# jolibrain/joliGEN

Hardware: AMD Instinct MI355X
Metric: train images/sec at 256x256 (DDPM UNet step) (higher is better)
Workload: dtype bf16; 1 GPU; palette_model DDPM, efficient UNet unet_mha ngf64 mults[1,2,4,8] res_blocks[2,2,2,2] mid-attn 16x32, 256x256, batch 32/GPU, inpainting synthetic masks, AdamW+EMA, iter_size 1 (example_ddpm_noglasses2glasses.json + SURVEY Appendix C overrides); global_batch=32, per_gpu_batch=32, image_size=256, efficient=True, parallelism=dp1, n_ranks_seen=1

## Files before the change

joligen_amd/_lib.py:

```python
from __future__ import annotations

import ctypes as C
import os
import re
import subprocess

_HERE = os.path.dirname(os.path.abspath(__file__))
CSRC = os.path.join(_HERE, "csrc")
LIB_PATH = os.path.join(CSRC, "libjg355.so")
HEADER = os.path.join(os.path.dirname(_HERE), "include", "jg355.h")
SOURCES = ["attention.hip", "gemm_nt.hip", "conv_halo.hip", "conv_kxk.hip", "reflect_border.hip", "conv_p64.hip", "conv1x1.hip", "gemm_tn.hip", "wgrad_halo.hip", "wgrad_sw.hip", "wgrad_kxk.hip", "nce.hip", "segformer.hip", "vit.hip", "projected_d.hip", "effnet.hip", "norm.hip", "gn_fused.hip", "elementwise.hip", "d_aug.hip", "context.hip", "d_diffusion.hip", "dropout.hip", "sem_cls.hip", "resize_aa.hip", "optim.hip", "capi.hip"]
HIPCC_FLAGS = ["--offload-arch=gfx950", "-O3", "-std=c++17", "-fPIC", "-shared", "-munsafe-fp-atomics", "-fno-slp-vectorize"]

FILE_FLAGS = {}

c_i32, c_i64, c_f32, c_p = C.c_int32, C.c_int64, C.c_float, C.c_void_p

_SCALARS = {"int": c_i32, "int32_t": c_i32, "int64_t": c_i64, "uint32_t": C.c_uint32, "uint64_t": C.c_uint64, "float": c_f32, "jg_stream_t": c_p}


def _ctype(decl: str, structs: dict, where: str):
    tok = re.findall(r"\w+|\*", decl)
    if len(tok) > 1 and tok[-1] != "*":
        tok = tok[:-1]
    if not tok or re.sub(r"[\w\s*]", "", decl):
        raise TypeError(f"jg355.h: cannot parse `{decl.strip()}` in `{where}`")
    if "*" not in tok:
        if len(tok) == 1 and tok[0] in _SCALARS:
            return _SCALARS[tok[0]]
        raise TypeError(f"jg355.h: type `{' '.join(tok)}` of `{decl.strip()}` in `{where}` is outside the ABI's type map")
    if tok == ["const", "char", "*"]:
        return C.c_char_p
    if len(tok) == 3 and tok[0] == "const" and tok[1] in structs and tok[2] == "*":
        return C.POINTER(structs[tok[1]])
    return c_p


def parse_header(text: str):
    text = re.sub(r"/\*.*?\*/", " ", text, flags=re.S)
    consts, structs, sigs, restypes = {}, {}, {}, {}
    for name, val in re.findall(r"^[ \t]*#[ \t]*define[ \t]+(JG_\w+)[ \t]+(-?\d+)[ \t]*$", text, flags=re.M):
        consts[name] = int(val)
    text = re.sub(r"^[ \t]*#.*$", " ", text, flags=re.M)
    text = re.sub(r'extern\s+"C"\s*\{(.*)\}', r"\1", text, flags=re.S)
    text = re.sub(r"typedef\s+void\s*\*\s*jg_stream_t\s*;", " ", text)

    def enum(m):
        for item in m.group(1).split(","):
            im = re.fullmatch(r"\s*(JG_\w+)\s*=\s*(-?\d+)\s*", item)
            if not im:
                raise TypeError(f"jg355.h: enumerator `{item.strip()}` needs the form JG_X = n")
            consts[im.group(1)] = int(im.group(2))
        return " "

    def struct(m):
        fields = []
        for decl in filter(str.strip, m.group(1).split(";")):
            first, *more = decl.split(",")
            ct = _ctype(first, structs, m.group(2))
            if ct not in _SCALARS.values() and more:
                raise TypeError(f"jg355.h: one pointer per declaration, `{decl.strip()}` in `{m.group(2)}`")
            fields += [(re.findall(r"\w+", d)[-1], ct) for d in [first] + more]
        structs[m.group(2)] = type(m.group(2), (C.Structure,), {"_fields_": fields})
        return " "

    def proto(m):
        ret, name, params = m.group(1), m.group(2), m.group(3)
        restypes[name] = _ctype(ret + " " + name, structs, name)
        sigs[name] = [] if params.strip() == "void" else [_ctype(p, structs, name) for p in params.split(",")]
        return " "

    text = re.sub(r"enum\s*\{([^}]*)\}\s*;", enum, text)
    text = re.sub(r"typedef\s+struct\s*\w*\s*\{([^}]*)\}\s*(\w+)\s*;", struct, text)
    text = re.sub(r"([\w\s*]+?)\b(jg_\w+)\s*\(([^()]*)\)\s*;", proto, text)
    if text.strip():
        raise TypeError(f"jg355.h: not understood: `{' '.join(text.split())[:200]}`")
    return consts, structs, sigs, restypes


with open(HEADER) as _f:
    CONSTANTS, STRUCTS, SIGNATURES, RESTYPES = parse_header(_f.read())
globals().update(CONSTANTS)
ConvArgs, WgradArgs = STRUCTS["jg_conv_args"], STRUCTS["jg_wgrad_args"]


def build(force: bool = False, verbose: bool = False, jobs: int = 0) -> str:
    import json
    import time
    from concurrent.futures import ThreadPoolExecutor

    hdrs = [os.path.join(CSRC, h) for h in sorted(os.listdir(CSRC)) if h.endswith(".h")] + [HEADER]
    hdr_time = max(os.path.getmtime(h) for h in hdrs)
    bdir = os.path.join(CSRC, "build")
    os.makedirs(bdir, exist_ok=True)
    hipcc = os.environ.get("HIPCC", "/opt/rocm/bin/hipcc")
    if not os.path.exists(hipcc):
        hipcc = "hipcc"
    cflags = [f for f in HIPCC_FLAGS if f != "-shared"]
    todo, objs = [], []
    for src in SOURCES:
        sp, op = os.path.join(CSRC, src), os.path.join(bdir, src.replace(".hip", ".o"))
        objs.append(op)
        if force or not os.path.exists(op) or os.path.getmtime(op) < max(os.path.getmtime(sp), hdr_time):
            todo.append((sp, op))

    def cc(job):
        sp, op = job
        cmd = [hipcc] + cflags + FILE_FLAGS.get(os.path.basename(sp), []) + ["-c", sp, "-o", op]
        if verbose:
            print(" ".join(cmd), flush=True)
        subprocess.run(cmd, check=True, cwd=CSRC)

    t0 = time.time()
    if todo:
        with ThreadPoolExecutor(max_workers=jobs or min(len(todo), os.cpu_count() or 4)) as ex:
            list(ex.map(cc, todo))
    relink = bool(todo) or not os.path.exists(LIB_PATH) or os.path.getmtime(LIB_PATH) < max(os.path.getmtime(o) for o in objs)
    if relink:
        cmd = [hipcc, "--offload-arch=gfx950", "-shared", "-fPIC", "-o", LIB_PATH] + objs
        if verbose:
            print(" ".join(cmd), flush=True)
        subprocess.run(cmd, check=True, cwd=CSRC)
    if todo or relink:
        with open(os.path.join(bdir, "BUILD_INFO.json"), "w") as f:
            json.dump({"compiled": [os.path.basename(s) for s, _ in todo], "linked": relink, "seconds": round(time.time() - t0, 1),
                       "flags": cflags, "hipcc": hipcc}, f)
    return LIB_PATH


_lib = None


def lib():
    global _lib
    if _lib is not None:
        return _lib
    if not os.path.exists(LIB_PATH):
        raise RuntimeError(
            f"{LIB_PATH} is missing: run `python -c 'import __graft_entry__ as g; g.build()'` "
            "(hipcc --offload-arch=gfx950).  joligen_amd has no CPU / eager fallback."
        )
    L = C.CDLL(LIB_PATH)
    for name, argtypes in SIGNATURES.items():
        fn = getattr(L, name)
        fn.argtypes = argtypes
        fn.restype = RESTYPES[name]
    _lib = L
    return L


def set_tuning(name: str, value: int):
    L = lib()
    prev = L.jg_get_tuning(name.encode())
    check(L.jg_set_tuning(name.encode(), int(value)), f"jg_set_tuning({name})")
    return prev


def check(code: int, what: str = ""):
    if code != 0:
        msg = lib().jg_strerror(code).decode()
        raise RuntimeError(f"libjg355 {what} failed: {msg} ({code})")
```

joligen_amd/csrc/common.h:

```cpp
#pragma once
#include <hip/hip_runtime.h>
#include <stdint.h>

#include "../../include/jg355.h"

typedef _Float16 f16_t;
typedef __bf16 bf16_t;
typedef _Float16 f16x8 __attribute__((ext_vector_type(8)));
typedef __bf16 bf16x8 __attribute__((ext_vector_type(8)));
typedef float f32x4 __attribute__((ext_vector_type(4)));
typedef short s16x4_t __attribute__((ext_vector_type(4)));
typedef __attribute__((address_space(3))) s16x4_t* lds_v4;

#define JG_WAVE 64

#define JG_TUNE_LIST(X) \
  X(HALO_CFG, 0) X(WGRAD_HALO_CFG, 0) X(CONV_VARIANT, 6) X(WGRAD_VARIANT, 4) X(SINKHORN_GENERIC, 0) X(CONV1X1, 1) X(GN_REVERSE, 1) \
  X(HALO_DBG, 0) X(PERSIST64, 1) X(HALO_PIPE, 1) X(WGRAD_PIPE, 1) X(CONV_SPLITK, 1) X(CONV_SMALL_TILE, 1) X(GN_FUSED, 1)           \
  X(GN_FUSED_CAP, 256) X(GN_FUSED_DBG, 0) X(GN_FUSED_SLEEP, 4) X(WGRAD_LDS_PAD, 0) X(LN_BWD_CAP, 256) X(DW_BWD_CAP, 512)           \
  X(DW_BWD_PPT, 8) X(CONV_KXK, 1) X(CONV_RING, 1) X(WGRAD_DEEP, 1) X(WGRAD_SW, 0) X(DETERMINISTIC, 0) X(WGRAD_GROUP_BLOCKS, 1024)  \
  X(SGEMM_SPLIT, 0) X(WGRAD_BIG, 1) X(DW_RUN, 1) X(SUBPIXEL_DGRAD_CFG, 0)
#define JG_TUNE_ENUM(name, dflt) JG_TUNE_##name,
enum JgTune { JG_TUNE_LIST(JG_TUNE_ENUM) JG_TUNE_COUNT };
#undef JG_TUNE_ENUM
int jg_tune(int which);
void jg_note_kernel(const char* name);

#define JG_CHECK_LAUNCH()                          \
  do {                                             \
    if (hipGetLastError() != hipSuccess) return JG_ERR_LAUNCH; \
  } while (0)

template <typename T> __device__ __forceinline__ float to_f32(T v) { return (float)v; }
template <typename T> __device__ __forceinline__ T from_f32(float v) { return (T)v; }

template <typename T> __device__ __forceinline__ T bits_to(uint16_t b) { return __builtin_bit_cast(T, b); }
template <typename T> __device__ __forceinline__ uint16_t to_bits(T v) { return __builtin_bit_cast(uint16_t, v); }

template <typename T> __device__ __forceinline__ void unpack8(const uint4& v, float* f) {
  const uint32_t w[4] = {v.x, v.y, v.z, v.w};
#pragma unroll
  for (int i = 0; i < 4; ++i) {
    f[2 * i] = to_f32(bits_to<T>((uint16_t)(w[i] & 0xffffu)));
    f[2 * i + 1] = to_f32(bits_to<T>((uint16_t)(w[i] >> 16)));
  }
}
template <typename T> __device__ __forceinline__ uint4 pack8(const float* f) {
  uint32_t w[4];
#pragma unroll
  for (int i = 0; i < 4; ++i) {
    w[i] = (uint32_t)to_bits<T>(from_f32<T>(f[2 * i])) | ((uint32_t)to_bits<T>(from_f32<T>(f[2 * i + 1])) << 16);
  }
  return make_uint4(w[0], w[1], w[2], w[3]);
}
template <typename T> __device__ __forceinline__ uint2 pack4(float a, float b, float c, float d) {
  uint2 r;
  r.x = (uint32_t)to_bits<T>(from_f32<T>(a)) | ((uint32_t)to_bits<T>(from_f32<T>(b)) << 16);
  r.y = (uint32_t)to_bits<T>(from_f32<T>(c)) | ((uint32_t)to_bits<T>(from_f32<T>(d)) << 16);
  return r;
}
template <typename T> __device__ __forceinline__ void unpack4(const uint2& v, float* f) {
  f[0] = to_f32(bits_to<T>((uint16_t)(v.x & 0xffffu)));
  f[1] = to_f32(bits_to<T>((uint16_t)(v.x >> 16)));
  f[2] = to_f32(bits_to<T>((uint16_t)(v.y & 0xffffu)));
  f[3] = to_f32(bits_to<T>((uint16_t)(v.y >> 16)));
}

template <typename T> struct Mfma;
template <> struct Mfma<f16_t> {
  static __device__ __forceinline__ f32x4 run(const uint4& a, const uint4& b, f32x4 c) {
    return __builtin_amdgcn_mfma_f32_16x16x32_f16(__builtin_bit_cast(f16x8, a), __builtin_bit_cast(f16x8, b), c, 0, 0, 0);
  }
};
template <> struct Mfma<bf16_t> {
  static __device__ __forceinline__ f32x4 run(const uint4& a, const uint4& b, f32x4 c) {
    return __builtin_amdgcn_mfma_f32_16x16x32_bf16(__builtin_bit_cast(bf16x8, a), __builtin_bit_cast(bf16x8, b), c, 0, 0, 0);
  }
};

template <typename T> __device__ __forceinline__ uint4 ldg16(const T* ptr, bool ok) {
  uint4 v = *reinterpret_cast<const uint4*>(ptr);
  v.x = ok ? v.x : 0u;
  v.y = ok ? v.y : 0u;
  v.z = ok ? v.z : 0u;
  v.w = ok ? v.w : 0u;
  return v;
}

__device__ __forceinline__ float sigmoid_fast(float u) { return __builtin_amdgcn_rcpf(1.0f + __expf(-u)); }
__device__ __forceinline__ float silu_f(float u) { return u * sigmoid_fast(u); }
__device__ __forceinline__ float silu_grad_f(float u) {
  const float s = sigmoid_fast(u);
  return s * (1.0f + u * (1.0f - s));
}

template <int ACT> __device__ __forceinline__ float act_f(float u) {
  if (ACT == JG_ACT_SILU) return silu_f(u);
  if (ACT == JG_ACT_RELU) return fmaxf(u, 0.f);
  if (ACT == JG_ACT_LRELU) return u > 0.f ? u : 0.2f * u;
  return u;
}
template <int ACT> __device__ __forceinline__ float act_grad_f(float u) {
  if (ACT == JG_ACT_SILU) return silu_grad_f(u);
  if (ACT == JG_ACT_RELU) return u > 0.f ? 1.f : 0.f;
  if (ACT == JG_ACT_LRELU) return u > 0.f ? 1.f : 0.2f;
  return 1.f;
}
__device__ __forceinline__ float act_grad_rt(float u, int act) {
  return act == JG_ACT_SILU ? silu_grad_f(u) : act == JG_ACT_RELU ? (u > 0.f ? 1.f : 0.f) : act == JG_ACT_LRELU ? (u > 0.f ? 1.f : 0.2f) : 1.f;
}

#define JG_DISPATCH_ACT(act, ...)                          \
  do {                                                     \
    if ((act) == JG_ACT_SILU) { constexpr int ACT = JG_ACT_SILU; __VA_ARGS__ }        \
    else if ((act) == JG_ACT_RELU) { constexpr int ACT = JG_ACT_RELU; __VA_ARGS__ }   \
    else if ((act) == JG_ACT_LRELU) { constexpr int ACT = JG_ACT_LRELU; __VA_ARGS__ } \
    else { constexpr int ACT = JG_ACT_NONE; __VA_ARGS__ }                              \
  } while (0)

__device__ __forceinline__ float wave_sum(float v) {
#pragma unroll
  for (int o = 32; o > 0; o >>= 1) v += __shfl_xor(v, o);
  return v;
}
__device__ __forceinline__ float wave_max(float v) {
#pragma unroll
  for (int o = 32; o > 0; o >>= 1) v = fmaxf(v, __shfl_xor(v, o));
  return v;
}

#define JG_DISPATCH_DTYPE(dtype, ...)                 \
  do {                                                \
    if ((dtype) == JG_F16) {                          \
      typedef f16_t T;                                \
      __VA_ARGS__                                     \
    } else if ((dtype) == JG_BF16) {                  \
      typedef bf16_t T;                               \
      __VA_ARGS__                                     \
    } else {                                          \
      return JG_ERR_BAD_ARG;                          \
    }                                                 \
  } while (0)
```

joligen_amd/csrc/gemm_tn.hip:

```cpp
#include "common.h"
#include "wgrad_params.h"
#include "lds_dma.h"
#include <vector>
#include <cstdlib>

namespace {


__device__ __forceinline__ int swz128(int row) { return (row >> 1) & 7; }

__device__ __forceinline__ void transpose4x8(const uint4* ra, uint2* out) {
  const uint32_t w[4][4] = {{ra[0].x, ra[0].y, ra[0].z, ra[0].w},
                            {ra[1].x, ra[1].y, ra[1].z, ra[1].w},
                            {ra[2].x, ra[2].y, ra[2].z, ra[2].w},
                            {ra[3].x, ra[3].y, ra[3].z, ra[3].w}};
#pragma unroll
  for (int d = 0; d < 4; ++d) {
    out[2 * d].x = (w[0][d] & 0xffffu) | (w[1][d] << 16);
    out[2 * d].y = (w[2][d] & 0xffffu) | (w[3][d] << 16);
    out[2 * d + 1].x = (w[0][d] >> 16) | (w[1][d] & 0xffff0000u);
    out[2 * d + 1].y = (w[2][d] >> 16) | (w[3][d] & 0xffff0000u);
  }
}

template <typename T>
__global__ __launch_bounds__(256) void wgrad_tn_kernel(WgP p) {
  constexpr int BM = 128, BN = 128, BK = 64;
  __shared__ uint4 sm[2][(BM + BN) * 8];

  const int tid = threadIdx.x;
  const int lane = tid & 63;
  const int wave = tid >> 6;
  const int wm = wave >> 1, wn = wave & 1;

  const int tilesN = (p.Ktot + BN - 1) / BN;
  const int n0 = (blockIdx.x % tilesN) * BN;
  const int m0 = (blockIdx.x / tilesN) * BM;

  const int z = blockIdx.z;
  const int batch = z / p.splitk, split = z % p.splitk;
  const int zb = batch / p.nh, zh = batch % p.nh;
  const T* __restrict__ dy = (const T*)p.dy + zb * p.sdyb + zh * p.sdyh;
  const T* __restrict__ x = (const T*)p.x + zb * p.sxb + zh * p.sxh;

  int per = (p.Mpix + p.splitk - 1) / p.splitk;
  per = (per + BK - 1) / BK * BK;
  const int kbeg = split * per;
  const int kend = min(p.Mpix, kbeg + per);
  if (kbeg >= kend) return;
  const int nk = (kend - kbeg + BK - 1) / BK;

  const int pq = tid & 15, co = tid >> 4;
  const int cm = m0 + co * 8;
  const bool a_ok = cm < p.Cout;
  const int nn = n0 + co * 8;
  const bool b_ok = nn < p.Ktot;
  const int rs = nn / p.Cin, ci = nn % p.Cin;
  const int fr = rs / p.S, fs = rs % p.S;
  const bool quad_row = (p.Wo & 3) == 0;

  uint4 ra[4], rb[4];
  float bsum[8];
#pragma unroll
  for (int q = 0; q < 8; ++q) bsum[q] = 0.f;
  const bool do_bias = p.dbias != nullptr && (blockIdx.x % tilesN) == 0;

  auto load_tiles = [&](int kbase) {
    const int p0 = kbase + pq * 4;
#pragma unroll
    for (int i = 0; i < 4; ++i) {
      const int pp = p0 + i;
      const bool ok = a_ok && pp < kend;
      ra[i] = ldg16(dy + (ok ? (long)pp * p.lddy + cm : 0), ok);
    }
    if (quad_row) {
      const int ow0 = p0 % p.Wo;
      const int t = p0 / p.Wo;
      const int oh = t % p.Ho;
      const int b = t / p.Ho;
      const int ih = oh * p.stride + fr - p.pad;
      const bool row_ok = b_ok && (unsigned)ih < (unsigned)p.H;
      const long rowoff = ((long)(b * p.H + ih) * p.W) * p.ldx + ci;
#pragma unroll
      for (int i = 0; i < 4; ++i) {
        const int iw = (ow0 + i) * p.stride + fs - p.pad;
        const bool ok = row_ok && (p0 + i) < kend && (unsigned)iw < (unsigned)p.W;
        rb[i] = ldg16(x + (ok ? rowoff + (long)iw * p.ldx : 0), ok);
      }
    } else {
#pragma unroll
      for (int i = 0; i < 4; ++i) {
        const int pp = p0 + i;
        const int ow = pp % p.Wo;
        const int t = pp / p.Wo;
        const int oh = t % p.Ho;
        const int b = t / p.Ho;
        const int ih = oh * p.stride + fr - p.pad;
        const int iw = ow * p.stride + fs - p.pad;
        const bool ok = b_ok && pp < kend && (unsigned)ih < (unsigned)p.H && (unsigned)iw < (unsigned)p.W;
        rb[i] = ldg16(x + (ok ? ((long)(b * p.H + ih) * p.W + iw) * p.ldx + ci : 0), ok);
      }
    }
  };
  auto store_lds = [&](int buf) {
    uint2 ta[8], tb[8];
    transpose4x8(ra, ta);
    transpose4x8(rb, tb);
    uint2* s2 = reinterpret_cast<uint2*>(&sm[buf][0]);
#pragma unroll
    for (int j = 0; j < 8; ++j) {
      const int row = co * 8 + j;
      const int slot = row * 16 + (((pq >> 1) ^ swz128(row)) << 1) + (pq & 1);
      s2[slot] = ta[j];
      s2[BM * 16 + slot] = tb[j];
    }
    if (do_bias) {
#pragma unroll
      for (int i = 0; i < 4; ++i) {
        float f[8];
        unpack8<T>(ra[i], f);
#pragma unroll
        for (int q = 0; q < 8; ++q) bsum[q] += f[q];
      }
    }
  };

  f32x4 acc[4][4];
#pragma unroll
  for (int i = 0; i < 4; ++i)
#pragma unroll
    for (int j = 0; j < 4; ++j) acc[i][j] = (f32x4){0.f, 0.f, 0.f, 0.f};

  const int frow = lane & 15, fk = lane >> 4;
  auto compute = [&](int buf) {
#pragma unroll
    for (int sub = 0; sub < 2; ++sub) {
      uint4 fa[4], fb[4];
      const int kc = fk + 4 * sub;
#pragma unroll
      for (int i = 0; i < 4; ++i) {
        const int row = wm * 64 + i * 16 + frow;
        fa[i] = sm[buf][row * 8 + (kc ^ swz128(row))];
      }
#pragma unroll
      for (int j = 0; j < 4; ++j) {
        const int row = wn * 64 + j * 16 + frow;
        fb[j] = sm[buf][BM * 8 + row * 8 + (kc ^ swz128(row))];
      }
#pragma unroll
      for (int i = 0; i < 4; ++i)
#pragma unroll
        for (int j = 0; j < 4; ++j) acc[i][j] = Mfma<T>::run(fa[i], fb[j], acc[i][j]);
    }
  };

// ... 419 lines not shown
        const int m = m0 + wm * 128 + i * 16 + (lane >> 4) * 4 + q;
        if (m >= p.Cout_out) continue;
        atomicAdd((float*)p.dw + zoff + (long)m * p.lddw + ocol, p.alpha * acc[i][j][q]);
      }
    }
  }
  if (do_bias) {
    float* s_b = reinterpret_cast<float*>(&sm[0][0]);
#pragma unroll
    for (int q = 0; q < 8; ++q) {
      float v = bsum[q];
      v += __shfl_xor(v, 32);
      if (lane < 32) s_b[wave * 256 + cidx * 8 + q] = v;
    }
    __syncthreads();
    if (tid < BM && (m0 + tid) < p.Cout_out) {
      float v = 0.f;
#pragma unroll
      for (int w8 = 0; w8 < 8; ++w8) v += s_b[w8 * 256 + tid];
      atomicAdd(p.dbias + m0 + tid, p.dbias_scale * v);
    }
  }
}

template <typename T, bool SPREAD = false, int ABL = 0>
__device__ __forceinline__ void wgrad_tn_dma_body(const WgP& p, const int bx, const int bz, uint4 (*sm)[2 * BIG_TILE]) {
  constexpr int BM = 256, BN = 256, BK = 64;
  const int tid = threadIdx.x;
  const int lane = tid & 63;
  const int wave = __builtin_amdgcn_readfirstlane(tid >> 6);
  const int wm = wave >> 2, wn = wave & 3;

  const int tilesN = (p.Ktot + BN - 1) / BN;
  const int n0 = (bx % tilesN) * BN;
  const int m0 = (bx / tilesN) * BM;
  const int batch = bz / p.splitk, split = bz % p.splitk;
  const int zb = batch / p.nh, zh = batch % p.nh;
  const T* __restrict__ dy = (const T*)p.dy + zb * p.sdyb + zh * p.sdyh;
  const T* __restrict__ x = (const T*)p.x + zb * p.sxb + zh * p.sxh;
  const T* zp = reinterpret_cast<const T*>(&jg_zero_page);

  int per = (p.Mpix + p.splitk - 1) / p.splitk;
  per = (per + BK - 1) / BK * BK;
  const int kbeg = split * per;
  const int kend = min(p.Mpix, kbeg + per);
  if (kbeg >= kend) return;
  const int nk = (kend - kbeg + BK - 1) / BK;

  typedef __attribute__((address_space(3))) char* lds_cptr;
  const unsigned lds0 = (unsigned)(size_t)(lds_cptr)(char*)&sm[0][0];

  int a_col[4], b_ci[4], b_fr[4], b_fs[4];
  bool a_ok[4], b_ok[4];
#pragma unroll
  for (int rd = 0; rd < 4; ++rd) {
    const int q = rd * 512 + tid;
    const int row = q >> 5, ps = q & 31;
    const int c = (((ps >> 1) ^ swz_tr(row)) << 1) | (ps & 1);
    a_col[rd] = m0 + c * 8;
    a_ok[rd] = a_col[rd] < p.Cout;
    const int nn = n0 + c * 8;
    b_ok[rd] = nn < p.Ktot;
    const int rs = nn / p.Cin;
    b_ci[rd] = nn % p.Cin;
    b_fr[rd] = rs / p.S;
    b_fs[rd] = rs % p.S;
  }
  auto issue_one = [&](int kbase, int buf, int idx) {
    const unsigned l0 = lds0 + (unsigned)((buf * 2 * BIG_TILE + wave * 64) * 16);
    const int rd = idx & 3;
    const int pp = kbase + ((rd * 512 + tid) >> 5);
    if (idx < 4) {
      const bool ok = a_ok[rd] && pp < kend;
      glds16(ok ? dy + (long)pp * p.lddy + a_col[rd] : zp, l0 + rd * 512 * 16);
    } else {
      const int ow = pp % p.Wo;
      const int t = pp / p.Wo;
      const int oh = t % p.Ho;
      const int b = t / p.Ho;
      const int ih = oh * p.stride + b_fr[rd] - p.pad;
      const int iw = ow * p.stride + b_fs[rd] - p.pad;
      const bool ok = b_ok[rd] && pp < kend && (unsigned)ih < (unsigned)p.H && (unsigned)iw < (unsigned)p.W;
      glds16(ok ? x + ((long)(b * p.H + ih) * p.W + iw) * p.ldx + b_ci[rd] : zp, l0 + (BIG_TILE + rd * 512) * 16);
    }
  };
  auto issue = [&](int kbase, int buf) {
#pragma unroll
    for (int idx = 0; idx < 8; ++idx) issue_one(kbase, buf, idx);
  };

  f32x4 acc[8][4], accb[8];
#pragma unroll
  for (int i = 0; i < 8; ++i) {
    accb[i] = (f32x4){0.f, 0.f, 0.f, 0.f};
#pragma unroll
    for (int j = 0; j < 4; ++j) acc[i][j] = (f32x4){0.f, 0.f, 0.f, 0.f};
  }
  const bool do_bias = p.dbias != nullptr && (bx % tilesN) == 0 && wn == 0;
  const uint32_t one1 = to_bits<T>(from_f32<T>(1.0f));
  const uint32_t one2 = one1 | (one1 << 16);
  const uint4 ones = make_uint4(one2, one2, one2, one2);

  const int i16 = lane & 15, g = lane >> 4;
  auto frag = [&](int buf, int tile, int cb, int sub) -> uint4 {
    if constexpr (ABL == 2) return make_uint4((unsigned)(buf + tile), (unsigned)cb, (unsigned)sub, (unsigned)lane);
    const char* base = reinterpret_cast<const char*>(&sm[buf][tile]);
    uint32_t w[4];
#pragma unroll
    for (int rd = 0; rd < 2; ++rd) {
      const int row = sub * 32 + g * 8 + rd * 4 + (i16 >> 2);
      const int off = (row * BIG_CH + ((cb ^ swz_tr(row)) << 1)) * 16 + (i16 & 3) * 8;
      const s16x4_t v = __builtin_amdgcn_ds_read_tr16_b64_v4i16((lds_v4)(base + off));
      const uint2 u = __builtin_bit_cast(uint2, v);
      w[2 * rd] = u.x;
      w[2 * rd + 1] = u.y;
    }
    return make_uint4(w[0], w[1], w[2], w[3]);
  };

  if constexpr (ABL != 3) issue(kbeg, 0);
  for (int ks = 0; ks < nk; ++ks) {
    const int cur = ks & 1;
    wait_vmcnt<0>();
    __builtin_amdgcn_s_barrier();
    const bool more = ks + 1 < nk;
    if (more && !SPREAD && ABL != 3) issue(kbeg + (ks + 1) * BK, cur ^ 1);
    uint4 fa_n = frag(cur, 0, wm * 8, 0);
#pragma unroll
    for (int sub = 0; sub < 2; ++sub) {
      uint4 fb[4];
#pragma unroll
      for (int j = 0; j < 4; ++j) fb[j] = frag(cur, BIG_TILE, wn * 4 + j, sub);
#pragma unroll
      for (int i = 0; i < 8; ++i) {
        const uint4 fa = fa_n;
        if (i < 7) fa_n = frag(cur, 0, wm * 8 + i + 1, sub);
        else if (sub == 0) fa_n = frag(cur, 0, wm * 8, 1);
        if (SPREAD && more && (i & 1) == 0) {
          __builtin_amdgcn_sched_barrier(0);
          issue_one(kbeg + (ks + 1) * BK, cur ^ 1, sub * 4 + (i >> 1));
          __builtin_amdgcn_sched_barrier(0);
        }
        if (do_bias) accb[i] = Mfma<T>::run(fa, ones, accb[i]);
#pragma unroll
        for (int j = 0; j < 4; ++j) {
          if constexpr (ABL == 1) { acc[i][j][0] += __builtin_bit_cast(float, fa.x ^ fb[j].y); acc[i][j][1] += __builtin_bit_cast(float, fa.z ^ fb[j].w); }
          else acc[i][j] = Mfma<T>::run(fa, fb[j], acc[i][j]);
        }
      }
    }
  }

  const long zoff = zb * p.sdwb + zh * p.sdwh;
#pragma unroll
  for (int j = 0; j < 4; ++j) {
    const int n = n0 + wn * 64 + j * 16 + (lane & 15);
    if (n >= p.Ktot) continue;
    const int ors = n / p.Cin, oci = n % p.Cin;
    if (oci >= p.Cin_out) continue;
    const long ocol = (long)ors * p.Cin_out + oci;
#pragma unroll
    for (int i = 0; i < 8; ++i) {
#pragma unroll
      for (int q = 0; q < 4; ++q) {
        const int m = m0 + wm * 128 + i * 16 + (lane >> 4) * 4 + q;
        if (m >= p.Cout_out) continue;
        atomicAdd((float*)p.dw + zoff + (long)m * p.lddw + ocol, p.alpha * acc[i][j][q]);
      }
    }
  }
  if (do_bias && (lane & 15) == 0) {
#pragma unroll
    for (int i = 0; i < 8; ++i)
#pragma unroll
      for (int q = 0; q < 4; ++q) {
        const int m = m0 + wm * 128 + i * 16 + (lane >> 4) * 4 + q;
        if (m < p.Cout_out) atomicAdd(p.dbias + m, p.dbias_scale * accb[i][q]);
      }
  }
}

template <typename T, bool DMA = true, int ABL = 0>
__global__ __launch_bounds__(512, 1) void wgrad_tn_big_kernel(WgP p) {
  __shared__ uint4 sm[2][2 * BIG_TILE];
  int bx, bz;
  wgrad_xcd_order(bx, bz);
  if constexpr (DMA) wgrad_tn_dma_body<T, ABL == 4, ABL == 4 ? 0 : ABL>(p, bx, bz, sm);
  else wgrad_tn_big_body<T>(p, bx, bz, sm);
}

constexpr int GROUP_MAX = 16;
struct WgGroup {
  WgP p[GROUP_MAX];
  int start[GROUP_MAX + 1];
  int tiles[GROUP_MAX];
  int n;
};
template <typename T, int WAVES_M, bool DEEP = false>
__global__ __launch_bounds__(256, 2) void wgrad_tn_tr_group_kernel(const WgGroup g) {
  __shared__ uint4 sm[2][2 * TR_TILE];
  const int b = blockIdx.x;
  int i = 0;
#pragma unroll
  for (int k = 1; k < GROUP_MAX; ++k) i += (k < g.n && b >= g.start[k]) ? 1 : 0;
  i = __builtin_amdgcn_readfirstlane(i);
  const int local = b - g.start[i];
  wgrad_tn_tr_body<T, WAVES_M, DEEP>(g.p[i], local % g.tiles[i], local / g.tiles[i], sm);
}

template <typename T, bool DMA = true>
__global__ __launch_bounds__(512, 1) void wgrad_tn_big_group_kernel(const WgGroup g) {
  __shared__ uint4 sm[2][2 * BIG_TILE];
  const int b = blockIdx.x;
  int i = 0;
#pragma unroll
  for (int k = 1; k < GROUP_MAX; ++k) i += (k < g.n && b >= g.start[k]) ? 1 : 0;
  i = __builtin_amdgcn_readfirstlane(i);
  const int local = b - g.start[i];
  if constexpr (DMA) wgrad_tn_dma_body<T>(g.p[i], local % g.tiles[i], local / g.tiles[i], sm);
  else wgrad_tn_big_body<T>(g.p[i], local % g.tiles[i], local / g.tiles[i], sm);
}

static inline bool wg_big_ok(const WgP& p) {
  return jg_tune(JG_TUNE_WGRAD_BIG) != 0 && p.out_mode == JG_OUT_ATOMIC_F32 && p.Cout >= 256 && p.Ktot >= 256 && p.Mpix >= 8192;
}

}

static int make_wgp(const jg_wgrad_args* a, WgP& p) {
  if (!a || !a->dy || !a->x || !a->dw) return JG_ERR_BAD_ARG;
  if (a->Cin % 8 || a->Cout % 8 || a->ldx % 8 || a->lddy % 8) return JG_ERR_BAD_ARG;
  if (a->nbatch < 1 || a->nh < 1 || a->splitk < 1) return JG_ERR_BAD_ARG;
  if ((long)a->nbatch * a->splitk > 65535) return JG_ERR_BAD_ARG;
  if (a->out_mode != JG_OUT_ATOMIC_F32 && a->splitk != 1) return JG_ERR_BAD_ARG;
  if (a->dbias && a->out_mode != JG_OUT_ATOMIC_F32) return JG_ERR_BAD_ARG;
  const long Mpix = (long)a->B * a->Ho * a->Wo;
  if (Mpix <= 0 || Mpix > (1L << 30)) return JG_ERR_BAD_ARG;
  p.dy = (const char*)a->dy; p.x = (const char*)a->x; p.dw = (char*)a->dw; p.dbias = a->dbias;
  p.Mpix = (int)Mpix; p.Cout = a->Cout; p.Ktot = a->R * a->S * a->Cin;
  p.H = a->H; p.W = a->W; p.Cin = a->Cin; p.R = a->R; p.S = a->S; p.pad = a->pad; p.stride = a->stride;
  p.Ho = a->Ho; p.Wo = a->Wo;
  p.Cin_out = a->Cin_out > 0 ? a->Cin_out : a->Cin;
  p.Cout_out = a->Cout_out > 0 ? a->Cout_out : a->Cout;
  p.lddy = a->lddy; p.ldx = a->ldx; p.lddw = a->lddw;
  p.nh = a->nh; p.splitk = a->splitk;
  if (jg_tune(JG_TUNE_DETERMINISTIC) != 0 && a->out_mode == JG_OUT_ATOMIC_F32) p.splitk = 1;
  p.sdyb = a->sdyb; p.sdyh = a->sdyh; p.sxb = a->sxb; p.sxh = a->sxh; p.sdwb = a->sdwb; p.sdwh = a->sdwh;
  p.alpha = a->alpha; p.out_mode = a->out_mode; p.B = a->B;
  p.dbias_scale = a->dbias_scale != 0.f ? a->dbias_scale : 1.f;
  if (a->pad_mode != 0 && a->pad_mode != 1) return JG_ERR_BAD_ARG;
  p.reflect = a->pad_mode == 1;
  if (a->x_mode < 0 || a->x_mode > 2) return JG_ERR_BAD_ARG;
  p.x_up = a->x_mode;
  if (p.x_up && (p.reflect || (a->H & 1) || (a->W & 1) || a->nbatch != 1)) return JG_ERR_BAD_ARG;
  return JG_OK;
}

extern "C" int jg_conv2d_wgrad_tn_group(int dtype, const jg_wgrad_args* a, int n, jg_stream_t stream) {
  if (!a || n < 1 || n > 4096) return JG_ERR_BAD_ARG;
  const int variant = jg_tune(JG_TUNE_WGRAD_VARIANT);
  if (variant < 2) return JG_ERR_UNSUPPORTED;
  std::vector<WgP> ps((size_t)n);
  std::vector<char> special((size_t)n, 0);
  for (int i = 0; i < n; ++i) {
    const int rc = make_wgp(a + i, ps[i]);
    if (rc != JG_OK) return rc;
    if (a[i].nbatch != 1 || a[i].out_mode != JG_OUT_ATOMIC_F32 || ps[i].reflect || ps[i].x_up) return JG_ERR_UNSUPPORTED;
    special[i] = variant >= 4 && (a[i].R > 1 || a[i].S > 1) &&
                 (jg_wgrad_halo_try(dtype, ps[i], 1, (hipStream_t)stream, true) || jg_wgrad_kxk_try(dtype, ps[i], 1, (hipStream_t)stream, true));
  }
  for (int i = 0; i < n; ++i)
    if (special[i] && !jg_wgrad_halo_try(dtype, ps[i], 1, (hipStream_t)stream)) jg_wgrad_kxk_try(dtype, ps[i], 1, (hipStream_t)stream);
  const int group_blocks = jg_tune(JG_TUNE_WGRAD_GROUP_BLOCKS);
  const size_t gpad = (size_t)jg_tune(JG_TUNE_WGRAD_LDS_PAD);
  for (int wavesm = 1; wavesm <= 3; ++wavesm) {
    WgGroup g;
    g.n = 0;
    g.start[0] = 0;
    auto flush = [&]() -> int {
      if (!g.n) return JG_OK;
      if (group_blocks > 0) {
        long total = 0;
        for (int i = 0; i < g.n; ++i) total += (long)g.tiles[i] * ((g.p[i].Mpix + 63) / 64);
        const long len = std::max<long>(4, (total + group_blocks - 1) / group_blocks);
        for (int i = 0; i < g.n; ++i) {
          const long ks = (g.p[i].Mpix + 63) / 64;
          g.p[i].splitk = (int)std::max<long>(1, std::min<long>(g.p[i].splitk, (ks + len - 1) / len));
          g.start[i + 1] = g.start[i] + g.tiles[i] * g.p[i].splitk;
        }
      }
      const dim3 grid(g.start[g.n]);
      const int deep = jg_tune(JG_TUNE_WGRAD_DEEP);
      if (wavesm == 3) {
        if (jg_tune(JG_TUNE_WGRAD_BIG) == 2) { JG_DISPATCH_DTYPE(dtype, hipLaunchKernelGGL((wgrad_tn_big_group_kernel<T, false>), grid, dim3(512), 0, (hipStream_t)stream, g);); }
        else { JG_DISPATCH_DTYPE(dtype, hipLaunchKernelGGL((wgrad_tn_big_group_kernel<T, true>), grid, dim3(512), 0, (hipStream_t)stream, g);); }
      } else if (wavesm == 1) {
        if (deep & 1) { JG_DISPATCH_DTYPE(dtype, hipLaunchKernelGGL((wgrad_tn_tr_group_kernel<T, 1, true>), grid, dim3(256), gpad, (hipStream_t)stream, g);); }
        else { JG_DISPATCH_DTYPE(dtype, hipLaunchKernelGGL((wgrad_tn_tr_group_kernel<T, 1>), grid, dim3(256), gpad, (hipStream_t)stream, g);); }
      } else {
        if (deep & 2) { JG_DISPATCH_DTYPE(dtype, hipLaunchKernelGGL((wgrad_tn_tr_group_kernel<T, 2, true>), grid, dim3(256), gpad, (hipStream_t)stream, g);); }
        else { JG_DISPATCH_DTYPE(dtype, hipLaunchKernelGGL((wgrad_tn_tr_group_kernel<T, 2>), grid, dim3(256), gpad, (hipStream_t)stream, g);); }
      }
      g.n = 0;
      return JG_OK;
    };
    for (int i = 0; i < n; ++i) {
      const WgP& p = ps[i];
      if (special[i] || (wg_big_ok(p) ? 3 : p.Cout <= 64 ? 1 : 2) != wavesm) continue;
      const int tiles = wavesm == 3 ? ((p.Cout + 255) / 256) * ((p.Ktot + 255) / 256) : ((p.Cout + 64 * wavesm - 1) / (64 * wavesm)) * ((p.Ktot + 127) / 128);
      g.p[g.n] = p;
      g.tiles[g.n] = tiles;
      g.start[g.n + 1] = g.start[g.n] + tiles * p.splitk;
      if (++g.n == GROUP_MAX) {
        const int rc2 = flush();
        if (rc2 != JG_OK) return rc2;
      }
    }
    const int rc3 = flush();
    if (rc3 != JG_OK) return rc3;
  }
  JG_CHECK_LAUNCH();
  return JG_OK;
}

extern "C" int jg_conv2d_wgrad_tn(int dtype, const jg_wgrad_args* a, jg_stream_t stream) {
  jg_note_kernel("");
  WgP p;
  {
    const int rc = make_wgp(a, p);
    if (rc != JG_OK) return rc;
  }
  const int variant = jg_tune(JG_TUNE_WGRAD_VARIANT);
  if (p.x_up == 2) {
    if (variant < 4 || !jg_wgrad_halo_try(dtype, p, a->nbatch, (hipStream_t)stream)) return JG_ERR_UNSUPPORTED;
    JG_CHECK_LAUNCH();
    return JG_OK;
  }
  if (variant >= 4 && (jg_wgrad_halo_try(dtype, p, a->nbatch, (hipStream_t)stream) || jg_wgrad_kxk_try(dtype, p, a->nbatch, (hipStream_t)stream))) {
    JG_CHECK_LAUNCH();
    return JG_OK;
  }
  if (p.reflect || p.x_up) return JG_ERR_UNSUPPORTED;
  if (variant >= 2 && wg_big_ok(p)) {
    const int tiles = ((p.Cout + 255) / 256) * ((p.Ktot + 255) / 256);
    dim3 grid(tiles, 1, a->nbatch * p.splitk);
    jg_note_kernel("wgrad_tn_big_kernel");
    const int bigmode = jg_tune(JG_TUNE_WGRAD_BIG);
    if (bigmode == 11) { JG_DISPATCH_DTYPE(dtype, hipLaunchKernelGGL((wgrad_tn_big_kernel<T, true, 1>), grid, dim3(512), 0, (hipStream_t)stream, p);); }
    else if (bigmode == 12) { JG_DISPATCH_DTYPE(dtype, hipLaunchKernelGGL((wgrad_tn_big_kernel<T, true, 2>), grid, dim3(512), 0, (hipStream_t)stream, p);); }
    else if (bigmode == 14) { JG_DISPATCH_DTYPE(dtype, hipLaunchKernelGGL((wgrad_tn_big_kernel<T, true, 4>), grid, dim3(512), 0, (hipStream_t)stream, p);); }
    else if (bigmode == 13) { JG_DISPATCH_DTYPE(dtype, hipLaunchKernelGGL((wgrad_tn_big_kernel<T, true, 3>), grid, dim3(512), 0, (hipStream_t)stream, p);); }
    else if (bigmode == 2) { JG_DISPATCH_DTYPE(dtype, hipLaunchKernelGGL((wgrad_tn_big_kernel<T, false>), grid, dim3(512), 0, (hipStream_t)stream, p);); }
    else { JG_DISPATCH_DTYPE(dtype, hipLaunchKernelGGL((wgrad_tn_big_kernel<T, true>), grid, dim3(512), 0, (hipStream_t)stream, p);); }
    JG_CHECK_LAUNCH();
    return JG_OK;
  }
  const int tilesN = (p.Ktot + 127) / 128;
  if (variant == 1) {
    dim3 grid(((p.Cout + 127) / 128) * tilesN, 1, a->nbatch * p.splitk);
    JG_DISPATCH_DTYPE(dtype, hipLaunchKernelGGL((wgrad_tn_kernel<T>), grid, dim3(256), 0, (hipStream_t)stream, p););
  } else if (p.Cout <= 64 && variant != 3) {
    dim3 grid(tilesN, 1, a->nbatch * p.splitk);
    jg_note_kernel("wgrad_tn_tr_kernel<1>");
    if (jg_tune(JG_TUNE_WGRAD_DEEP) & 1) { JG_DISPATCH_DTYPE(dtype, hipLaunchKernelGGL((wgrad_tn_tr_kernel<T, 1, true>), grid, dim3(256), 0, (hipStream_t)stream, p);); }
    else { JG_DISPATCH_DTYPE(dtype, hipLaunchKernelGGL((wgrad_tn_tr_kernel<T, 1>), grid, dim3(256), 0, (hipStream_t)stream, p);); }
  } else {
    dim3 grid(((p.Cout + 127) / 128) * tilesN, 1, a->nbatch * p.splitk);
    jg_note_kernel("wgrad_tn_tr_kernel<2>");
    if (jg_tune(JG_TUNE_WGRAD_DEEP) & 2) { JG_DISPATCH_DTYPE(dtype, hipLaunchKernelGGL((wgrad_tn_tr_kernel<T, 2, true>), grid, dim3(256), 0, (hipStream_t)stream, p);); }
    else { JG_DISPATCH_DTYPE(dtype, hipLaunchKernelGGL((wgrad_tn_tr_kernel<T, 2>), grid, dim3(256), 0, (hipStream_t)stream, p);); }
  }
  JG_CHECK_LAUNCH();
  return JG_OK;
}
```

joligen_amd/modules/projected_d.py:

```python
from __future__ import annotations

import os

import torch
import torch.nn as nn

from .._autograd import JGFunction
from .. import _lib, launch, ops
from .._lib import check
from ..ops import JG_ACT_LRELU, _dt, _p, _st, conv_nt, wgrad_tn
from .layers import JGConv2d, JGConvNd

TF_EFFICIENTNET_LITE0_WIDTHS = (24, 40, 112, 320)


class _Bilinear2Fn(JGFunction):

    @staticmethod
    def forward(ctx, x, Ho, Wo, align):
        ctx.geo = (x.shape[1], x.shape[2], align)
        return launch.bilinear2_fwd(x.contiguous(), Ho, Wo, align)

    @staticmethod
    @torch.autograd.function.once_differentiable
# ... 47 lines not shown
        dev = mods[0].weight_orig.device
        ws = snap = w16 = dw = 0
        rec = []
        for mod in mods:
            m = mod.meta
            K, RS = m.R * m.S * m.Cin_real, m.R * m.S
            rec.append(dict(ws=ws, snap=0, w16=w16, dw=dw, Cout=m.Cout_real, RS=RS, Cin=m.Cin_real, CoutP=m.Cout, CinP=m.Cin, K=K))
            ws += K + m.Cout_real + 2
            w16 += 2 * m.Cout * RS * m.Cin
            dw += m.Cout_real * K
        self.zero_floats = ws
        for r in rec:
            r["snap"] = ws + snap
            snap += 1 + r["Cout"] + r["K"]
        self.fbuf_floats, self.hbuf_elems, self.dbuf_floats = ws + snap, w16, dw + self.L
        self.dots_off = dw
        self.rec = rec
        self.max_K = max(r["K"] for r in rec)
        self.max_Cout = max(r["Cout"] for r in rec)
        self.max_w = max(r["CoutP"] * r["RS"] * r["CinP"] for r in rec)
        self.max_n = max(r["Cout"] * r["K"] for r in rec)
        tab = np.zeros((self.L, 11), dtype=np.int64)
        ints = tab.view(np.int32).reshape(self.L, 22)
        self.ptrs = []
        for i, (mod, r) in enumerate(zip(mods, rec)):
            g = mod.weight_orig.grad
            if g is None:
                raise RuntimeError("spectral conv weight has no arena-backed .grad")
            p = (mod.weight_orig.data_ptr(), mod.weight_u.data_ptr(), mod.weight_v.data_ptr(), g.data_ptr())
            self.ptrs.append(p)
            tab[i, 0:4] = p
            tab[i, 4:8] = (r["ws"], r["snap"], r["w16"], r["dw"])
            ints[i, 16:22] = (r["Cout"], r["RS"], r["Cin"], r["CoutP"], r["CinP"], 0)
        self.table = torch.from_numpy(tab).to(dev)

    def still_valid(self):
        return all(p == (m.weight_orig.data_ptr(), m.weight_u.data_ptr(), m.weight_v.data_ptr(), m.weight_orig.grad.data_ptr())
                   for p, m in zip(self.ptrs, self.mods))


class _SnPass:

    def __init__(self, group):
        L = _lib.lib()
        self.g = g = group
        dev = g.table.device
        self.fbuf = torch.empty(g.fbuf_floats, device=dev, dtype=torch.float32)
        self.hbuf = torch.empty(g.hbuf_elems, device=dev, dtype=g.dtype)
        check(L.jg_spectral_group_forward(_lib.JG_F16 if g.dtype == torch.float16 else _lib.JG_BF16, g.table.data_ptr(), g.L, self.fbuf.data_ptr(),
                                          g.zero_floats, self.hbuf.data_ptr(), g.max_K, g.max_Cout, g.max_w, 1e-12, _st()), "jg_spectral_group_forward")
        self.dbuf, self.mask, self.flushed = None, 0, False

    def views(self, i):
        r = self.g.rec[i]
        n = r["CoutP"] * r["RS"] * r["CinP"]
        w16 = self.hbuf[r["w16"]:r["w16"] + n].view(r["CoutP"], -1, r["CinP"])
        w16T = self.hbuf[r["w16"] + n:r["w16"] + 2 * n].view(r["CinP"], -1, r["CoutP"])
        return w16, w16T

    def dwsn(self, i):
        if self.dbuf is None:
            self.dbuf = torch.zeros(self.g.dbuf_floats, device=self.fbuf.device, dtype=torch.float32)
        r = self.g.rec[i]
        return self.dbuf[r["dw"]:r["dw"] + r["Cout"] * r["K"]].view(r["Cout"], r["K"])

    def delivered(self, i):
        self.mask |= 1 << i
        if self.mask == (1 << self.g.L) - 1:
            self.flush()

    def flush(self):
        if self.flushed or not self.mask:
            return
        g = self.g
        if ops.WGRAD_DEFER:
            ops.flush_deferred_wgrads()
        check(_lib.lib().jg_spectral_group_wgrad_fix(g.table.data_ptr(), g.L, self.fbuf.data_ptr(), self.dbuf.data_ptr(),
                                                     self.dbuf.data_ptr() + 4 * g.dots_off, self.mask, g.max_n, _st()), "jg_spectral_group_wgrad_fix")
        self.flushed = True


class _SpectralConvFn(JGFunction):

    @staticmethod
    def forward(ctx, x, weight_orig, bias, mod):
        L = _lib.lib()
        m = mod.meta
        x = x.contiguous()
        B, H, W_, Cin = x.shape
        assert Cin == m.Cin, (Cin, m.Cin)
        dev = x.device
        prepared = getattr(mod, "_sn_pass", None)
        if prepared is not None:
            mod._sn_pass = None
            sn, idx = prepared
            w16, w16T = sn.views(idx)
            Ho, Wo = m.out_hw(H, W_)
            y = torch.empty((B, Ho, Wo, m.Cout), device=dev, dtype=x.dtype)
            conv_nt(x, w16, y, B=B, H=H, W=W_, Cin=Cin, Cout=m.Cout, R=m.R, S=m.S, pad=m.pad, stride=m.stride, Ho=Ho, Wo=Wo, ldx=Cin,
                    ldw=m.R * m.S * Cin, ldy=m.Cout, bias=m.bias_pad if m.bias_pad is not None else bias)
            ctx.save_for_backward(x, w16T)
            ctx.mod, ctx.sn = mod, (sn, idx)
            return y
        ctx.sn = None
        sigma = torch.empty(1, device=dev, dtype=torch.float32)
        Wp = weight_orig.data_ptr()
        if mod.training:
            launch.spectral_power_iter(weight_orig, mod.weight_u, mod.weight_v, sigma, m.Cout_real, m.R * m.S, m.Cin_real)
        else:
            Wl = weight_orig.detach().reshape(m.Cout_real, -1)
            sigma.copy_(torch.dot(mod.weight_u, Wl @ mod.weight_v).reshape(1))
        w16 = torch.empty((m.Cout, m.R, m.S, m.Cin), device=dev, dtype=x.dtype)
        w16T = torch.empty((m.Cin, m.R, m.S, m.Cout), device=dev, dtype=x.dtype) if ctx.needs_input_grad[0] else None
        check(L.jg_spectral_weights(_dt(x), Wp, sigma.data_ptr(), w16.data_ptr(), _p(w16T), m.Cout_real, m.R * m.S, m.Cin_real, m.Cout, m.Cin,
                                    _st()), "jg_spectral_weights")
        Ho, Wo = m.out_hw(H, W_)
        y = torch.empty((B, Ho, Wo, m.Cout), device=dev, dtype=x.dtype)
        conv_nt(x, w16, y, B=B, H=H, W=W_, Cin=Cin, Cout=m.Cout, R=m.R, S=m.S, pad=m.pad, stride=m.stride, Ho=Ho, Wo=Wo, ldx=Cin,
                ldw=m.R * m.S * Cin, ldy=m.Cout, bias=m.bias_pad if m.bias_pad is not None else bias)
        ctx.save_for_backward(x, w16T, sigma, mod.weight_u.clone(), mod.weight_v.clone())
        ctx.mod = mod
        return y

    @staticmethod
    @torch.autograd.function.once_differentiable
    def backward(ctx, dy):
        if ctx.sn is not None:
            x, w16T = ctx.saved_tensors
            sigma = u = v = None
        else:
            x, w16T, sigma, u, v = ctx.saved_tensors
        mod = ctx.mod
        m = mod.meta
        dy = dy.contiguous()
        B, H, W_, Cin = x.shape
        _, Ho, Wo, Cout = dy.shape
        dx = None
        if ctx.needs_input_grad[0]:
            dx = torch.empty_like(x)
            if m.stride != 1:
                Hd, Wd = H + 2 * m.pad - m.R + 1, W_ + 2 * m.pad - m.S + 1
                dyd = ops.dilate2d(dy, Hd, Wd, m.stride)
                conv_nt(dyd, w16T, dx, B=B, H=Hd, W=Wd, Cin=Cout, Cout=Cin, R=m.R, S=m.S, pad=m.R - 1 - m.pad, stride=1, Ho=H, Wo=W_,
                        ldx=Cout, ldw=m.R * m.S * Cout, ldy=Cin)
            else:
                conv_nt(dy, w16T, dx, B=B, H=Ho, W=Wo, Cin=Cout, Cout=Cin, R=m.R, S=m.S, pad=m.R - 1 - m.pad, stride=1, Ho=H, Wo=W_,
                        ldx=Cout, ldw=m.R * m.S * Cout, ldy=Cin)
        if ctx.needs_input_grad[1]:
            wg = mod.weight_orig.grad
            if wg is None:
                raise RuntimeError("spectral conv weight has no arena-backed .grad")
            K = m.R * m.S * m.Cin_real
            dwsn = ctx.sn[0].dwsn(ctx.sn[1]) if ctx.sn is not None else torch.zeros((m.Cout_real, K), device=dy.device, dtype=torch.float32)
            ktot = m.R * m.S * Cin
            splitk = ops._wgrad_splitk(((Cout + 127) // 128) * ((ktot + 127) // 128), B * Ho * Wo)
            wgrad_tn(dy, x, dwsn, B=B, H=H, W=W_, Cin=Cin, Cout=Cout, R=m.R, S=m.S, pad=m.pad, stride=m.stride, Ho=Ho, Wo=Wo, lddy=Cout, ldx=Cin,
                     lddw=K, dbias=mod.bias.grad if mod.bias is not None else None, Cin_out=m.Cin_real, Cout_out=m.Cout_real, splitk=splitk,
                     defer=ctx.sn is not None)
            if ctx.sn is not None:
                ctx.sn[0].delivered(ctx.sn[1])
                return dx, None, None, None
            launch.spectral_wgrad_fix(dwsn, mod.weight_orig, u, v, sigma, wg, m.Cout_real, m.R * m.S, m.Cin_real)
        return dx, None, None, None


class SpectralConv2d(nn.Module, JGConvNd):

    jg_wname = "weight_orig"

    def __init__(self, cin, cout, k, stride, padding, bias=True):
        super().__init__()
        ref = nn.Conv2d(cin, cout, k, stride, padding, bias=bias)
        if bias:
            self.bias = nn.Parameter(ref.bias.detach().clone())
        else:
            self.register_parameter("bias", None)
        self.weight_orig = nn.Parameter(ref.weight.detach().clone())
        u = nn.functional.normalize(torch.randn(cout), dim=0, eps=1e-12)
        v = nn.functional.normalize(torch.randn(cin * k * k), dim=0, eps=1e-12)
        self.register_buffer("weight_u", u)
        self.register_buffer("weight_v", v)
        self.needs_dgrad = True
        self.jg_padding, self.jg_stride = padding, stride

    def forward(self, x):
        if self.meta is None:
            raise RuntimeError("SpectralConv2d used before ParamArena finalisation")
        return _SpectralConvFn.apply(x, self.weight_orig, self.bias, self)


class DownBlock(nn.Module):

    def __init__(self, cin, cout):
        super().__init__()
        self.main = nn.Sequential(SpectralConv2d(cin, cout, 4, 2, 1), nn.GroupNorm(cout // 2, cout), nn.LeakyReLU(0.2, inplace=True))

    def forward(self, x):
        conv, gn = self.main[0], self.main[1]
        return ops.group_norm(conv(x), gn.num_groups, gn.weight, gn.bias, None, JG_ACT_LRELU, gn.eps)


CHANNEL_DICT = {4: 512, 8: 512, 16: 256, 32: 128, 64: 64, 128: 64, 256: 32, 512: 16, 1024: 8}


class SingleDisc(nn.Module):

    def __init__(self, nc, start_sz=256, end_sz=8):
        super().__init__()
        nfc = dict(CHANNEL_DICT)
        if start_sz not in nfc:
            start_sz = min(nfc, key=lambda s: abs(s - start_sz))
        self.start_sz = start_sz
        nfc[start_sz] = nc
        layers = []
        while start_sz > end_sz:
            layers.append(DownBlock(nfc[start_sz], nfc[start_sz // 2]))
            start_sz //= 2
        layers.append(SpectralConv2d(nfc[end_sz], 1, 4, 1, 0, bias=False))
        self.main = nn.Sequential(*layers)

    def forward(self, x):
        for layer in self.main:
            x = layer(x)
        return x


class MultiScaleD(nn.Module):

    def __init__(self, channels, resolutions, num_discs=4):
        super().__init__()
        self.mini_discs = nn.ModuleDict({str(i): SingleDisc(nc=c, start_sz=r, end_sz=8)
                                         for i, (c, r) in enumerate(zip(channels[:num_discs], resolutions[:num_discs]))})

    def forward(self, features):
        outs = []
        for k, disc in self.mini_discs.items():
            lg = disc(features[k])
            outs.append(lg[..., 0].reshape(lg.shape[0], -1))
        return torch.cat(outs, dim=1)


class StandInEfficientNet(nn.Module):

    def __init__(self):
        super().__init__()
        w = TF_EFFICIENTNET_LITE0_WIDTHS

        def stage(cin, cout):
            return nn.Sequential(nn.Conv2d(cin, cout, 4, 2, 1), nn.LeakyReLU(0.2))

        self.conv_stem = nn.Conv2d(3, 16, 4, 2, 1)
        self.bn1 = nn.LeakyReLU(0.2)
        self.blocks = nn.Sequential(nn.Identity(), stage(16, w[0]), stage(w[0], w[1]), nn.Identity(), stage(w[1], w[2]), nn.Identity(),
                                    nn.Identity(), nn.Identity(), stage(w[2], w[3]))


class _Stage(nn.Module):

    def __init__(self, items):
        super().__init__()
        for i, it in enumerate(items):
            self.add_module(str(i), it)

    def forward(self, x):
        for mod in self.children():
            x = _run_plain(mod, x)
        return x


def _run_plain(mod, x):
    if isinstance(mod, JGConv2d):
        return mod(x)
    if isinstance(mod, nn.LeakyReLU):
        return ops.activation(x, JG_ACT_LRELU)
    if isinstance(mod, nn.Identity):
        return x
    if isinstance(mod, (nn.Sequential, _Stage)):
        for sub in mod.children():
            x = _run_plain(sub, x)
        return x
    raise NotImplementedError(type(mod))


def _hip_stage(cin, cout):
    return nn.Sequential(JGConv2d(cin, cout, 4, padding=1, stride=2), nn.LeakyReLU(0.2))


LITE0_STEM = 32
LITE0_ARCH = (("ds", 1, 3, 1, 1, 16), ("ir", 2, 3, 2, 6, 24), ("ir", 2, 5, 2, 6, 40), ("ir", 3, 3, 2, 6, 80), ("ir", 3, 5, 1, 6, 112),
              ("ir", 4, 5, 2, 6, 192), ("ir", 1, 3, 1, 6, 320))
LITE0_BN_EPS = 1e-3


def tf_same_pad(size, k, stride):
    out = -(-size // stride)
    total = max((out - 1) * stride + k - size, 0)
    return total // 2, total - total // 2


class _FrozenBN(nn.Module):

    def __init__(self, c, eps=LITE0_BN_EPS):
        super().__init__()
        self.weight, self.bias = nn.Parameter(torch.ones(c)), nn.Parameter(torch.zeros(c))
        self.register_buffer("running_mean", torch.zeros(c))
        self.register_buffer("running_var", torch.ones(c))
        self.register_buffer("num_batches_tracked", torch.tensor(0, dtype=torch.long))
        self.eps = eps
        self._key, self._affine = None, None

# ... 430 lines not shown
```

joligen_amd/modules/unet_exec.py:

```python
from __future__ import annotations

import contextlib
import math
import os
import weakref
from typing import Tuple

import torch
import torch.nn as nn

from .._autograd import JGFunction
from .. import _lib, launch, ops, parallel
from .._lib import JG_ACT_NONE, JG_ACT_SILU, check
from ..ops import _dt, _p, _st, attn_core_bwd, attn_core_fwd, conv_nt, wgrad_tn


class Act:

    __slots__ = ("t", "st", "hw", "pid", "hs_j")

    def __init__(self, t, st, hw, pid, hs_j=None):
        self.t, self.st, self.hw, self.pid, self.hs_j = t, st, hw, pid, hs_j


# ... 9 lines not shown
NSLOT = 16
NORM_BEFORE_UP = os.environ.get("JG_NORM_BEFORE_UP", "1") != "0"
FUSE_DOWN_POOL = os.environ.get("JG_FUSE_DOWN_POOL", "1") != "0"
SUBPIXEL_CONV = os.environ.get("JG_SUBPIXEL_CONV", "1") != "0"
POOL_IN_DGRAD = os.environ.get("JG_POOL_IN_DGRAD", "1") != "0"
SUBPIXEL_DGRAD = os.environ.get("JG_SUBPIXEL_DGRAD", "1") != "0"
SUBPIXEL_WGRAD = os.environ.get("JG_SUBPIXEL_WGRAD", "1") != "0"
X_UP_ON_READ = os.environ.get("JG_X_UP_ON_READ", "1") != "0"
RES_UP_ON_READ = os.environ.get("JG_RES_UP_ON_READ", "1") != "0"
FUSE_GN_REDUCE = os.environ.get("JG_FUSE_GN_REDUCE", "0") != "0"
WGRAD_STREAM = os.environ.get("JG_WGRAD_STREAM", "1") != "0"
WGRAD_CU_MASK = os.environ.get("JG_WGRAD_CU_MASK", "")


def cu_masked_stream(device, first, count, total=256):
    import ctypes as C

    hip = C.CDLL("libamdhip64.so")
    words = (total + 31) // 32
    mask = (C.c_uint32 * words)()
    for i in range(first, min(total, first + count)):
        mask[i // 32] |= 1 << (i % 32)
    st = C.c_void_p()
    with torch.cuda.device(device):
        rc = hip.hipExtStreamCreateWithCUMask(C.byref(st), C.c_uint32(words), mask)
    if rc != 0:
        raise RuntimeError(f"hipExtStreamCreateWithCUMask failed with {rc}")
    return torch.cuda.ExternalStream(st.value, device=device)


def _side_stream(device):
    if WGRAD_CU_MASK:
        first, count = (int(v) for v in WGRAD_CU_MASK.split(":"))
        return cu_masked_stream(device, first, count)
    return torch.cuda.Stream(device=device)
WGRAD_FIRST = os.environ.get("JG_WGRAD_FIRST", "1") != "0"
FUSE_GN_COEF = os.environ.get("JG_FUSE_GN_COEF", "0") != "0"
GN_FUSED = os.environ.get("JG_GN_FUSED", "0") != "0"
FUSE_SKIP_APPLY = os.environ.get("JG_FUSE_SKIP_APPLY", "1") != "0"
FUSE_SKIP_BWD = os.environ.get("JG_FUSE_SKIP_BWD", "1") != "0"


class _Pool:

    def __init__(self, n, device):
        self.buf = torch.zeros(n, device=device, dtype=torch.float32)
        self.off = 0

    def take(self, B, C):
        n = B * NSLOT * C * 2
        if self.off + n > self.buf.numel():
            raise RuntimeError("statistics pool exhausted")
        v = self.buf[self.off:self.off + n].view(B, NSLOT, C, 2)
        self.off += n
        return v

    def take_rows(self, B, C):
        n = B * C * 2
        if self.off + n > self.buf.numel():
            return None
        v = self.buf[self.off:self.off + n].view(B, C, 2)
        self.off += n
        return v


def halo_ok(m, H, W):
    return m.R == 3 and m.S == 3 and m.pad == 1 and m.stride == 1 and m.Cin % 64 == 0 and m.Cout % 64 == 0 and H % 16 == 0 and W % 16 == 0


def subpixel_ok(m, H, W):
    return halo_ok(m, H, W) and H % 32 == 0 and W % 32 == 0 and m.Cin_real == m.Cin and m.Cout_real == m.Cout


def subpixel_fold(m, dtype):
    out = torch.empty((4, m.Cout, 2, 2, m.Cin), device=m.weight.device, dtype=dtype)
    check(_lib.lib().jg_subpixel_fold(_lib.JG_F16 if dtype == torch.float16 else _lib.JG_BF16, m.weight.data_ptr(), out.data_ptr(), m.Cout,
                                      m.Cin, _st()), "jg_subpixel_fold")
    return out


def subpixel_fold_pair(m, dtype):
    out = torch.empty((4, m.Cout, 2, 2, m.Cin), device=m.weight.device, dtype=dtype)
    outT = torch.empty((4, m.Cin, 2, 2, m.Cout), device=m.weight.device, dtype=dtype)
    check(_lib.lib().jg_subpixel_fold_pair(_lib.JG_F16 if dtype == torch.float16 else _lib.JG_BF16, m.weight.data_ptr(), out.data_ptr(),
                                           outT.data_ptr(), m.Cout, m.Cin, _st()), "jg_subpixel_fold_pair")
    return out, outT


def conv_fwd(x, m, out=None, res=None, res_scale=1.0, alpha=1.0, stats=None, res_up=False, x_up=False, wfold=None):
    B, H, W, Cin = x.shape
    if x_up:
        H, W = 2 * H, 2 * W
    Ho, Wo = m.out_hw(H, W)
    if out is None:
        out = torch.empty((B, Ho, Wo, m.Cout), device=x.device, dtype=x.dtype)
    fuse = stats is not None and _stats_fusable(B, Ho, Wo, m.Cout)
    conv_nt(x, m.w16 if wfold is None else wfold, out, B=B, H=H, W=W, Cin=Cin, Cout=m.Cout, R=m.R, S=m.S, pad=m.pad, stride=m.stride,
            Ho=Ho, Wo=Wo, ldx=_ld(x), ldw=m.R * m.S * Cin if wfold is None else 4 * Cin, ldy=_ld(out),
            bias=m.bias_pad if m.bias_pad is not None else m.bias, res=res,
            ldres=_ld(res) if res is not None else 0, alpha=alpha, res_scale=res_scale,
            stats=stats if fuse else None, ldstats=stats.stride(1) // 2 if fuse else 0, stats_slots=NSLOT,
            res_mode=1 if res_up else 0, x_mode=(2 if wfold is not None else 1) if x_up else 0)
    if stats is not None and not fuse:
        check(_lib.lib().jg_gn_stats_ld(_dt(out), out.data_ptr(), _ld(out), stats.data_ptr(), stats.stride(0) // 2, B, Ho * Wo,
                                        m.Cout, _st()), "jg_gn_stats_ld")
    return out


def conv1x1_gn_apply(x, m, ab, act):
    B, H, W, Cin = x.shape
    if m.R != 1 or m.S != 1 or m.stride != 1 or m.pad != 0:
        return None
    y = torch.empty((B, H, W, m.Cout), device=x.device, dtype=x.dtype)
    yn = torch.empty((B, H, W, Cin), device=x.device, dtype=x.dtype)
    ok = conv_nt(x, m.w16, y, B=B, H=H, W=W, Cin=Cin, Cout=m.Cout, R=1, S=1, pad=0, stride=1, Ho=H, Wo=W, ldx=_ld(x), ldw=Cin, ldy=m.Cout,
                 bias=m.bias_pad if m.bias_pad is not None else m.bias, apply=(ab, yn, Cin, act))
    return (yn, y) if ok is not False else None


def conv_dgrad(dy, m, x_shape, out=None, res=None, alpha=1.0, gn=None, pool=None, pool_out=False, wfoldT=None):
    if m.stride != 1:
        raise NotImplementedError("input-gradient of strided convolutions is not implemented")
    B, H, W, Cin = x_shape
    _, Ho, Wo, Cout = dy.shape
    if pool_out:
        assert out is None and res is None and gn is None
        out = torch.empty((B, H // 2, W // 2, Cin), device=dy.device, dtype=dy.dtype)
        if wfoldT is not None:
            conv_nt(dy, wfoldT, out, B=B, H=Ho, W=Wo, Cin=Cout, Cout=Cin, R=3, S=3, pad=1, stride=1, Ho=H, Wo=W, ldx=_ld(dy), ldw=4 * Cout,
                    ldy=_ld(out), alpha=alpha, y_mode=2)
            return out
    if out is None:
        out = torch.empty(x_shape, device=dy.device, dtype=dy.dtype)
    red = None
    kw = {}
    if gn is not None and pool is not None and res is None and _stats_fusable(B, H, W, Cin) and FUSE_GN_REDUCE:
        gx, gab, gact = gn
        red = pool.take(B, Cin)
        kw = dict(stats=red, ldstats=Cin, stats_slots=NSLOT, gn_reduce=(gx, _ld(gx), gab, gact))
    conv_nt(dy, m.w16T, out, B=B, H=Ho, W=Wo, Cin=Cout, Cout=Cin, R=m.R, S=m.S, pad=m.R - 1 - m.pad, stride=1, Ho=H, Wo=W,
            ldx=_ld(dy), ldw=m.R * m.S * Cout, ldy=_ld(out), alpha=alpha, res=res, ldres=_ld(res) if res is not None else 0,
            res_scale=1.0, y_mode=1 if pool_out else 0, **kw)
    return (out, red) if gn is not None else out


def conv_wgrad(dy, x, m, alpha=1.0, dbias_scale=0.0, x_up=False, subpixel=False):
    B, H, W, Cin = x.shape
    if x_up:
        H, W = 2 * H, 2 * W
    _, Ho, Wo, Cout = dy.shape
    wg = m.weight.grad
    if wg is None:
        raise RuntimeError("conv weight has no arena-backed .grad")
    ktot = m.R * m.S * Cin
    tiles = ((Cout + 127) // 128) * ((ktot + 127) // 128)
    splitk = ops._wgrad_splitk(tiles, B * Ho * Wo)
    wgrad_tn(dy, x, wg, B=B, H=H, W=W, Cin=Cin, Cout=Cout, R=m.R, S=m.S, pad=m.pad, stride=m.stride, Ho=Ho, Wo=Wo,
             lddy=_ld(dy), ldx=_ld(x), lddw=m.R * m.S * m.Cin_real, dbias=m.bias.grad if m.bias is not None else None,
             Cin_out=m.Cin_real, Cout_out=m.Cout_real, splitk=splitk, alpha=alpha, dbias_scale=dbias_scale, x_mode=(2 if subpixel else 1) if x_up else 0)


def gn_coef(st, hw, gamma, beta, film, G, eps):
    B, ns, C, _ = st.shape
    ab = torch.empty((B, C, 2), device=st.device, dtype=torch.float32)
    mr = torch.empty((B, G, 2), device=st.device, dtype=torch.float32)
    check(_lib.lib().jg_gn_coef_ld(st.data_ptr(), st.stride(1) // 2, ns, _p(gamma), _p(beta), _p(film),
                                   film.stride(0) if film is not None else 0, ab.data_ptr(), mr.data_ptr(), B, hw, C, G, eps,
                                   _st()), "jg_gn_coef_ld")
    return ab, mr


def gn_apply(x, ab, act):
    B, H, W, C = x.shape
    y = torch.empty((B, H, W, C), device=x.device, dtype=x.dtype)
    check(_lib.lib().jg_gn_apply_ld(_dt(x), x.data_ptr(), _ld(x), ab.data_ptr(), y.data_ptr(), C, B, H * W, C, act, _st()),
          "jg_gn_apply_ld")
    return y


def gn_bwd_coef(red, nslots, gamma, beta, film, mr, dgamma, dbeta, dfilm, B, HW, C, G):
    pqr = torch.empty((B, C, 3), device=red.device, dtype=torch.float32)
    check(_lib.lib().jg_gn_bwd_coef_slots(red.data_ptr(), nslots, _p(gamma), _p(beta), _p(film),
                                          film.stride(0) if film is not None else 0, mr.data_ptr(), pqr.data_ptr(), _p(dgamma),
                                          _p(dbeta), _p(dfilm), dfilm.stride(0) if dfilm is not None else 0, B, HW, C, G, _st()),
          "jg_gn_bwd_coef_slots")
    return pqr


def gn_bwd(x, dy, ab, mr, gamma, beta, film, G, act, dfilm=None, out=None, adds=(), red=None, pooled=None, pool=None, skip=None):
    L = _lib.lib()
    B, H, W, C = x.shape
    HW = H * W
    dev, dt = x.device, _dt(x)
    nslots = NSLOT
    if red is None and GN_FUSED and skip is None and pool is not None and G <= 2048 and C <= 2048:
        rows, cnt = pool.take_rows(B, C), pool.take_rows(B, 1)
        if rows is not None and cnt is not None:
            dgamma = gamma.grad if gamma is not None else None
            dbeta = beta.grad if beta is not None else None
            if gamma is not None and dgamma is None:
                raise RuntimeError("norm weight has no arena-backed .grad")
            if out is None:
                out = torch.empty((B, H, W, C), device=dev, dtype=x.dtype)
            adds = list(adds)
            if pooled is not None:
                if len(adds) > 1:
                    raise RuntimeError("at most one full-resolution addend next to the pooled one")
                a1, s1 = pooled[1] if pooled[1] is not None else (None, 0.0)
                a2, s2 = adds[0] if adds else (None, 0.0)
            else:
                if len(adds) > 2:
                    raise RuntimeError("at most two fused gradient addends")
                a1, s1 = adds[0] if len(adds) > 0 else (None, 0.0)
                a2, s2 = adds[1] if len(adds) > 1 else (None, 0.0)
            check(L.jg_gn_bwd_fused(dt, int(pooled is not None), x.data_ptr(), _ld(x), dy.data_ptr(), _ld(dy),
                                    pooled[0] if pooled is not None else 1.0, ab.data_ptr(), rows.data_ptr(), cnt.data_ptr(),
                                    ops.gn_status(dev).data_ptr(), _p(gamma), _p(beta), _p(film), film.stride(0) if film is not None else 0,
                                    mr.data_ptr(), _p(dgamma), _p(dbeta), _p(dfilm), dfilm.stride(0) if dfilm is not None else 0, G,
                                    out.data_ptr(), _ld(out), _p(a1), _ld(a1) if a1 is not None else 0, s1, _p(a2),
                                    _ld(a2) if a2 is not None else 0, s2, B, H, W, C, act, _st()), "jg_gn_bwd_fused")
            return out
    if red is None:
        nslots = 1
        red = pool.take_rows(B, C) if pool is not None else None
        up, ld = (L.jg_gn_bwd_reduce_up_acc, L.jg_gn_bwd_reduce_ld_acc) if red is not None else (L.jg_gn_bwd_reduce_up, L.jg_gn_bwd_reduce_ld)
        if red is None:
            red = torch.empty((B, C, 2), device=dev, dtype=torch.float32)
        if pooled is not None:
            check(up(dt, x.data_ptr(), _ld(x), dy.data_ptr(), _ld(dy), pooled[0], ab.data_ptr(), red.data_ptr(), B, H, W, C, act, _st()),
                  "jg_gn_bwd_reduce_up")
        else:
            check(ld(dt, x.data_ptr(), _ld(x), dy.data_ptr(), _ld(dy), ab.data_ptr(), red.data_ptr(), B, HW, C, act, _st()),
                  "jg_gn_bwd_reduce_ld")
    dgamma = gamma.grad if gamma is not None else None
    dbeta = beta.grad if beta is not None else None
    if gamma is not None and dgamma is None:
        raise RuntimeError("norm weight has no arena-backed .grad")
    if FUSE_GN_COEF and skip is None and nslots == 1 and G <= 256:
        if out is None:
            out = torch.empty((B, H, W, C), device=dev, dtype=x.dtype)
        adds = list(adds)
        if pooled is not None:
            if len(adds) > 1:
                raise RuntimeError("at most one full-resolution addend next to the pooled one")
            a1, s1 = pooled[1] if pooled[1] is not None else (None, 0.0)
            a2, s2 = adds[0] if adds else (None, 0.0)
        else:
            if len(adds) > 2:
                raise RuntimeError("at most two fused gradient addends")
            a1, s1 = adds[0] if len(adds) > 0 else (None, 0.0)
            a2, s2 = adds[1] if len(adds) > 1 else (None, 0.0)
        check(L.jg_gn_bwd_apply_fc(dt, int(pooled is not None), x.data_ptr(), _ld(x), dy.data_ptr(), _ld(dy),
                                   pooled[0] if pooled is not None else 1.0, ab.data_ptr(), red.data_ptr(), _p(gamma), _p(beta), _p(film),
                                   film.stride(0) if film is not None else 0, mr.data_ptr(), _p(dgamma), _p(dbeta), _p(dfilm),
                                   dfilm.stride(0) if dfilm is not None else 0, G, out.data_ptr(), _ld(out), _p(a1),
                                   _ld(a1) if a1 is not None else 0, s1, _p(a2), _ld(a2) if a2 is not None else 0, s2, B, H, W, C, act, _st()),
              "jg_gn_bwd_apply_fc")
        return out
    pqr = gn_bwd_coef(red, nslots, gamma, beta, film, mr, dgamma, dbeta, dfilm, B, HW, C, G)
    if out is None:
        out = torch.empty((B, H, W, C), device=dev, dtype=x.dtype)
    adds = list(adds)
    if pooled is not None:
        if len(adds) > 1:
            raise RuntimeError("at most one full-resolution addend next to the pooled one")
        a1, s1 = pooled[1] if pooled[1] is not None else (None, 0.0)
        a2, s2 = adds[0] if adds else (None, 0.0)
        check(L.jg_gn_bwd_apply_up(dt, x.data_ptr(), _ld(x), dy.data_ptr(), _ld(dy), pooled[0], ab.data_ptr(), pqr.data_ptr(),
                                   out.data_ptr(), _ld(out), _p(a1), _ld(a1) if a1 is not None else 0, s1, _p(a2),
                                   _ld(a2) if a2 is not None else 0, s2, B, H, W, C, act, _st()), "jg_gn_bwd_apply_up")
        return out
    if len(adds) > 2:
        raise RuntimeError("at most two fused gradient addends")
    a1, s1 = adds[0] if len(adds) > 0 else (None, 0.0)
    a2, s2 = adds[1] if len(adds) > 1 else (None, 0.0)
    if skip is not None:
        dO, m, alpha = skip
        if FUSE_SKIP_BWD and m.R == 1 and m.S == 1 and m.stride == 1 and m.pad == 0:
            ok = conv_nt(dO, m.w16T, out, B=B, H=H, W=W, Cin=m.Cout, Cout=C, R=1, S=1, pad=0, stride=1, Ho=H, Wo=W, ldx=_ld(dO), ldw=m.Cout,
                         ldy=_ld(out), alpha=alpha, gn_bwd_apply=(x, dy, ab, pqr, a1, s1, a2, s2, act))
            if ok is not False:
                return out
    check(L.jg_gn_bwd_apply_ld(dt, x.data_ptr(), _ld(x), dy.data_ptr(), _ld(dy), ab.data_ptr(), pqr.data_ptr(), out.data_ptr(),
                               _ld(out), _p(a1), _ld(a1) if a1 is not None else 0, s1, _p(a2),
                               _ld(a2) if a2 is not None else 0, s2, B, HW, C, act, _st()), "jg_gn_bwd_apply_ld")
    if skip is not None:
        dO, m, alpha = skip
        return conv_dgrad(dO, m, x.shape, res=out, alpha=alpha)
    return out


def gn_bwd_drop(x, dy, ab, mr, gamma, beta, film, G, act, drop, dfilm=None, pool=None):
    B, H, W, C = x.shape
    red = pool.take_rows(B, C) if pool is not None else None
    if red is None:
        red = torch.zeros((B, C, 2), device=x.device, dtype=torch.float32)
    dgamma = gamma.grad if gamma is not None else None
    dbeta = beta.grad if beta is not None else None
    if gamma is not None and dgamma is None:
        raise RuntimeError("norm weight has no arena-backed .grad")
    launch.gn_bwd_reduce_drop(x, dy, ab, red, act, *drop)
    pqr = gn_bwd_coef(red, 1, gamma, beta, film, mr, dgamma, dbeta, dfilm, B, H * W, C, G)
    return launch.gn_bwd_apply_drop(x, dy, ab, pqr, act, *drop)


def gn_apply_pool(x, ab, act, scale):
    B, H, W, C = x.shape
    y = torch.empty((B, H // 2, W // 2, C), device=x.device, dtype=x.dtype)
    check(_lib.lib().jg_gn_apply_pool(_dt(x), x.data_ptr(), _ld(x), ab.data_ptr(), y.data_ptr(), C, B, H, W, C, act, scale, _st()),
          "jg_gn_apply_pool")
    return y

# ... 576 lines not shown
```

joligen_amd/ops.py:

```python
from __future__ import annotations

import ctypes as C
import math
import os

from typing import Optional, Tuple

import torch

from ._autograd import JGFunction
from . import _lib
from ._lib import (JG_ACT_LRELU, JG_ACT_NONE, JG_ACT_RELU, JG_ACT_SILU, JG_ACT_TANH, JG_OUT_ATOMIC_F32, JG_OUT_STORE_T, ConvArgs,
                   WgradArgs, check)
from . import launch
from .launch import SINKHORN_ITERS, _DT, _dt, _p, _raw_stream, _st, sgemm


def _require_cuda(*ts):
    for t in ts:
        if t is not None and not t.is_cuda:
            raise RuntimeError("joligen_amd ops run on the GPU only (no CPU fallback); got a CPU tensor")


KERNEL_TIMING = None
# ... 149 lines not shown
        return 0
    by_dt = {}
    for dt, a, keep in todo:
        by_dt.setdefault(dt, []).append(a)
    if os.environ.get("JG_WGRAD_DUMP"):
        with open(os.environ["JG_WGRAD_DUMP"], "a") as f:
            f.write("flush %d\n" % len(todo))
            for dt, a, keep in todo:
                f.write("%d %d %d %d %d %d %d %d %d %d %d %d %d\n" % (a.B, a.H, a.W, a.Cin, a.Cout, a.R, a.S, a.pad, a.stride, a.Ho, a.Wo, a.splitk, int(bool(a.dbias))))
    side = _WGRAD_SIDE[0] if _WGRAD_SIDE is not None else None
    if side is not None:
        side.wait_stream(torch.cuda.current_stream())
        for dt, a, keep in todo:
            for t in keep[:2]:
                t.record_stream(side)
        ctx = torch.cuda.stream(side)
    else:
        import contextlib

        ctx = contextlib.nullcontext()
    with ctx:
        for dt, args in by_dt.items():
            arr = (WgradArgs * len(args))(*args)
            check(_lib.lib().jg_conv2d_wgrad_tn_group(dt, arr, len(args), _st()), "jg_conv2d_wgrad_tn_group")
    return len(todo)


class deferred_wgrads:

    def __init__(self, stream=None, every=48):
        self.stream, self.every = stream, every

    def __enter__(self):
        global WGRAD_DEFER, _WGRAD_SIDE
        self.prev = WGRAD_DEFER
        if WGRAD_GROUP and WGRAD_DEFER is None:
            WGRAD_DEFER = []
            _WGRAD_SIDE = (self.stream, self.every) if self.stream is not None else None
        return self

    def __exit__(self, *exc):
        global WGRAD_DEFER, _WGRAD_SIDE
        if self.prev is None and WGRAD_DEFER is not None:
            try:
                if exc[0] is None:
                    flush_deferred_wgrads()
                    if _WGRAD_SIDE is not None:
                        torch.cuda.current_stream().wait_stream(_WGRAD_SIDE[0])
            finally:
                WGRAD_DEFER = None
                _WGRAD_SIDE = None


def axpby(a, alpha=1.0, b=None, beta=0.0, alpha_dev=None, out=None):
    y = torch.empty_like(a) if out is None else out
    check(_lib.lib().jg_axpby(_dt(a), a.data_ptr(), alpha, _p(alpha_dev), _p(b), beta, y.data_ptr(), a.numel(), _st()),
          "jg_axpby")
    return y


class ConvMeta:

    __slots__ = ("Cin", "Cout", "Cin_real", "Cout_real", "R", "S", "pad", "stride", "w16", "w16T", "weight", "bias",
                 "bias_pad")

    def out_hw(self, H, W):
        return ((H + 2 * self.pad - self.R) // self.stride + 1, (W + 2 * self.pad - self.S) // self.stride + 1)


WGRAD_TARGET_BLOCKS = int(os.environ.get("JG_WGRAD_TARGET_BLOCKS", "1536"))
WGRAD_MAX_SPLITK = 512
WGRAD_SPLIT_PIX = int(os.environ.get("JG_WGRAD_SPLIT_PIX", "256"))


def _wgrad_splitk(tiles, mpix, nbatch=1):
    want = max(1, (WGRAD_TARGET_BLOCKS + tiles - 1) // tiles)
    cap = max(1, mpix // WGRAD_SPLIT_PIX)
    return max(1, min(want, cap, WGRAD_MAX_SPLITK, 65535 // max(1, nbatch)))


def conv2d_forward(x, m: ConvMeta, res=None, res_scale=1.0, alpha=1.0, stats=None):
    _require_cuda(x)
    B, H, W, Cin = x.shape
    assert Cin == m.Cin, (Cin, m.Cin)
    Ho, Wo = m.out_hw(H, W)
    y = torch.empty((B, Ho, Wo, m.Cout), device=x.device, dtype=x.dtype)
    conv_nt(x, m.w16, y, B=B, H=H, W=W, Cin=Cin, Cout=m.Cout, R=m.R, S=m.S, pad=m.pad, stride=m.stride, Ho=Ho, Wo=Wo,
            ldx=Cin, ldw=m.R * m.S * Cin, ldy=m.Cout, bias=m.bias_pad if m.bias_pad is not None else m.bias, res=res,
            ldres=m.Cout, alpha=alpha, res_scale=res_scale, stats=stats)
    return y


def dilate2d(x, Ho, Wo, stride):
    B, H, W, Cc = x.shape
    y = torch.empty((B, Ho, Wo, Cc), device=x.device, dtype=x.dtype)
    check(_lib.lib().jg_dilate2d(_dt(x), x.contiguous().data_ptr(), y.data_ptr(), B, H, W, Cc, Ho, Wo, stride, _st()), "jg_dilate2d")
    return y


PHASE_TCONV = os.environ.get("JG_PHASE_TCONV", "1") != "0"
PATCH_DGRAD = os.environ.get("JG_PATCH_DGRAD", "1") != "0"


def phase_tconv_ok(m: ConvMeta, Hout, Wout, C, N):
    return (PHASE_TCONV and m.stride == 2 and m.R == m.S and m.R in (3, 4) and m.pad == 1 and C % 64 == 0 and N % 64 == 0 and Hout % 32 == 0
            and Wout % 32 == 0)


def phase_tconv(x, m: ConvMeta, y, bias=None, alpha=1.0):
    B, h, w, C = x.shape
    N = y.shape[-1]
    wf = torch.empty((4, N, 2, 2, C), device=x.device, dtype=x.dtype)
    check(_lib.lib().jg_transposed_fold(_dt(x), m.w16T.data_ptr(), wf.data_ptr(), N, C, m.R, m.S, m.pad, _st()), "jg_transposed_fold")
    conv_nt(x, wf, y, B=B, H=2 * h, W=2 * w, Cin=C, Cout=N, R=3, S=3, pad=1, stride=1, Ho=2 * h, Wo=2 * w, ldx=C, ldw=4 * C, ldy=N, bias=bias,
            alpha=alpha, x_mode=2)
    return y


def conv2d_dgrad(dy, m: ConvMeta, x_shape, alpha=1.0):
    B, H, W, Cin = x_shape
    _, Ho, Wo, Cout = dy.shape
    dx = torch.empty(x_shape, device=dy.device, dtype=dy.dtype)
    if m.stride != 1:
        if H == 2 * Ho and W == 2 * Wo and phase_tconv_ok(m, H, W, Cout, Cin):
            return phase_tconv(dy, m, dx, alpha=alpha)
        if (PATCH_DGRAD and Cin == 8 and m.Cin_real <= 4 and Cout % 8 == 0 and m.R * m.S * Cout * 16 <= 65536
                and Ho == (H + 2 * m.pad - m.R) // m.stride + 1 and Wo == (W + 2 * m.pad - m.S) // m.stride + 1):
            check(_lib.lib().jg_conv_dgrad_gather(_dt(dy), dy.contiguous().data_ptr(), m.w16.data_ptr(), dx.data_ptr(), B, H, W, Ho, Wo, Cout, m.R, m.S,
                                                  m.stride, m.pad, alpha, _st()), "jg_conv_dgrad_gather")
            return dx
        if PATCH_DGRAD and m.stride == m.R == m.S and m.pad == 0 and H == Ho * m.R and W == Wo * m.S:
            N = m.R * m.S * Cin
            wt = m.w16.view(Cout, N).t().contiguous()
            tmp = torch.empty((B, Ho, Wo, N), device=dy.device, dtype=dy.dtype)
            conv_nt(dy, wt, tmp, B=B, H=Ho, W=Wo, Cin=Cout, Cout=N, R=1, S=1, pad=0, stride=1, Ho=Ho, Wo=Wo, ldx=Cout, ldw=Cout, ldy=N, alpha=alpha)
            dx.view(B, Ho, m.R, Wo, m.S, Cin).copy_(tmp.view(B, Ho, Wo, m.R, m.S, Cin).permute(0, 1, 3, 2, 4, 5))
            return dx
        Hd, Wd = H + 2 * m.pad - m.R + 1, W + 2 * m.pad - m.S + 1
        dyd = dilate2d(dy, Hd, Wd, m.stride)
        conv_nt(dyd, m.w16T, dx, B=B, H=Hd, W=Wd, Cin=Cout, Cout=Cin, R=m.R, S=m.S, pad=m.R - 1 - m.pad, stride=1, Ho=H, Wo=W,
                ldx=Cout, ldw=m.R * m.S * Cout, ldy=Cin, alpha=alpha)
        return dx
    conv_nt(dy, m.w16T, dx, B=B, H=Ho, W=Wo, Cin=Cout, Cout=Cin, R=m.R, S=m.S, pad=m.R - 1 - m.pad, stride=1, Ho=H, Wo=W,
            ldx=Cout, ldw=m.R * m.S * Cout, ldy=Cin, alpha=alpha)
    return dx


def conv2d_wgrad(dy, x, m: ConvMeta, alpha=1.0, want_w=True, want_b=True):
    B, H, W, Cin = x.shape
    _, Ho, Wo, Cout = dy.shape
    wg = m.weight.grad
    if wg is None:
        raise RuntimeError("conv weight has no arena-backed .grad (module not finalised by ParamArena)")
    ktot = m.R * m.S * Cin
    tiles = ((Cout + 127) // 128) * ((ktot + 127) // 128)
    splitk = _wgrad_splitk(tiles, B * Ho * Wo)
    dbias = m.bias.grad if (want_b and m.bias is not None) else None
    wgrad_tn(dy, x, wg, B=B, H=H, W=W, Cin=Cin, Cout=Cout, R=m.R, S=m.S, pad=m.pad, stride=m.stride, Ho=Ho, Wo=Wo,
             lddy=Cout, ldx=Cin, lddw=m.R * m.S * m.Cin_real, dbias=dbias, Cin_out=m.Cin_real, Cout_out=m.Cout_real,
             splitk=splitk, alpha=alpha)


HEAD7_PACKED = os.environ.get("JG_HEAD7_PACKED", "1") != "0"
_HEAD7_BUFS = {}


def head7_ok(x_pad, m: ConvMeta):
    if not HEAD7_PACKED or TORCH_OPS_BOUNDARY or KERNEL_TIMING is not None or not x_pad.is_cuda:
        return False
    B, Hp, Wp, Cin = x_pad.shape
    return (m.R == 7 and m.S == 7 and m.stride == 1 and m.pad == 0 and Cin == m.Cin and Cin % 64 == 0 and m.Cout_real <= 4 and (Wp - 6) % 16 == 0
            and Hp > 6 and B * (Hp - 6) * (Wp - 6) >= 65536 and x_pad.dtype in (torch.float16, torch.bfloat16))


class _Head7x7Fn(JGFunction):

    @staticmethod
    def forward(ctx, x_pad, weight, bias, meta, act):
        m = meta
        x_pad = x_pad.contiguous()
        B, Hp, Wp, Cin = x_pad.shape
        H, W = Hp - 6, Wp - 6
        dev, dt = x_pad.device, x_pad.dtype
        key = (m.w16.data_ptr(), dt, Cin)
        bufs = _HEAD7_BUFS.get(key)
        if bufs is None:
            bufs = _HEAD7_BUFS[key] = (torch.zeros((8, 4, 7, Cin), device=dev, dtype=dt), torch.zeros((Cin, 7, 8, 4), device=dev, dtype=dt))
        wz, wzT = bufs
        wz[:7].copy_(m.w16[:4].permute(1, 0, 2, 3))
        wzT[:, :, :7].copy_(m.w16[:4].permute(3, 2, 1, 0).flip(1))
        z = torch.empty((B, Hp, W, 32), device=dev, dtype=dt)
        conv_nt(x_pad, wz, z, B=B, H=Hp, W=Wp, Cin=Cin, Cout=32, R=1, S=7, pad=0, stride=1, Ho=Hp, Wo=W, ldx=Cin, ldw=7 * Cin, ldy=32)
        out = torch.empty((B, H, W, 8), device=dev, dtype=dt)
        b4 = m.bias_pad
        if b4 is None and m.bias is not None:
            b4 = torch.zeros(4, device=dev, dtype=torch.float32)
            b4[:m.Cout_real].copy_(m.bias.detach()[:m.Cout_real])
        check(_lib.lib().jg_tapsum7(_dt(x_pad), z.data_ptr(), _p(b4), out.data_ptr(), B, H, W, act, _st()), "jg_tapsum7")
        ctx.save_for_backward(x_pad, out, wzT)
        ctx.cfg = (m, act)
        return out

    @staticmethod
    @torch.autograd.function.once_differentiable
    def backward(ctx, dout):
        x_pad, out, wzT = ctx.saved_tensors
        m, act = ctx.cfg
        dout = dout.contiguous()
        B, Hp, Wp, Cin = x_pad.shape
        H, W = Hp - 6, Wp - 6
        dev, dt = x_pad.device, x_pad.dtype
        Hz = (Hp + 7) // 8 * 8
        dz = torch.empty((B, Hz, W, 32), device=dev, dtype=dt)
        dzm = torch.empty((B, Hp, W + 12, 32), device=dev, dtype=dt)
        check(_lib.lib().jg_tapspread7(_dt(dout), dout.data_ptr(), out.data_ptr(), dz.data_ptr(), dzm.data_ptr(), B, H, W, Hz, act, _st()), "jg_tapspread7")
        dx = None
        if ctx.needs_input_grad[0]:
            dx = torch.empty_like(x_pad)
            conv_nt(dzm, wzT, dx, B=B, H=Hp, W=W + 12, Cin=32, Cout=Cin, R=1, S=7, pad=0, stride=1, Ho=Hp, Wo=Wp, ldx=32, ldw=7 * 32, ldy=Cin)
        if ctx.needs_input_grad[1] or ctx.needs_input_grad[2]:
            wg = m.weight.grad
            if wg is None:
                raise RuntimeError("conv weight has no arena-backed .grad (module not finalised by ParamArena)")
            acc = torch.zeros(32 * 7 * Cin + 32, device=dev, dtype=torch.float32)
            dwz, db = acc[:32 * 7 * Cin].view(8, 4, 7, Cin), acc[32 * 7 * Cin:]
            wgrad_tn(dz, x_pad, dwz, B=B, H=Hp, W=Wp, Cin=Cin, Cout=32, R=1, S=7, pad=0, stride=1, Ho=Hz, Wo=W, lddy=32, ldx=Cin, lddw=7 * Cin, dbias=db,
                     Cin_out=Cin, Cout_out=32, splitk=1, defer=False)
            cr = m.Cout_real
            wg.permute(0, 2, 3, 1)[:cr].add_(dwz[:7, :cr].permute(1, 0, 2, 3)[..., :m.Cin_real])
            if m.bias is not None and ctx.needs_input_grad[2]:
                m.bias.grad[:cr].add_(db[:cr])
        return dx, None, None, None, None


def head_conv7(x_pad, m: ConvMeta, act=0):
    return _Head7x7Fn.apply(x_pad, m.weight, m.bias, m, act)


class _Conv2dFn(JGFunction):
    @staticmethod
    def forward(ctx, x, weight, bias, res, meta, res_scale, alpha, stats=None):
        y = conv2d_forward(x, meta, res, res_scale, alpha, stats)
        ctx.save_for_backward(x)
        ctx.meta, ctx.res_scale, ctx.alpha, ctx.has_res = meta, res_scale, alpha, res is not None
        return y

    @staticmethod
    @torch.autograd.function.once_differentiable
    def backward(ctx, dy):
        (x,) = ctx.saved_tensors
        m = ctx.meta
        dy = dy.contiguous()
        dx = dres = None
        if ctx.needs_input_grad[0]:
            dx = conv2d_dgrad(dy, m, x.shape, ctx.alpha)
        if ctx.needs_input_grad[1] or ctx.needs_input_grad[2]:
            conv2d_wgrad(dy, x, m, ctx.alpha, ctx.needs_input_grad[1], ctx.needs_input_grad[2])
        if ctx.has_res and ctx.needs_input_grad[3]:
            dres = dy if ctx.res_scale == 1.0 else axpby(dy, ctx.res_scale)
        return dx, None, None, dres, None, None, None, None


TORCH_OPS_BOUNDARY = False


class torch_ops_boundary:
    def __enter__(self):
        global TORCH_OPS_BOUNDARY
        self.prev, TORCH_OPS_BOUNDARY = TORCH_OPS_BOUNDARY, True

    def __exit__(self, *a):
        global TORCH_OPS_BOUNDARY
        TORCH_OPS_BOUNDARY = self.prev


def _conv2d_via_torch_ops(x, m: ConvMeta, res, res_scale, alpha):
    import torch.nn.functional as F

    w = m.weight.reshape(m.Cout_real, m.Cin_real, m.R, m.S).permute(0, 2, 3, 1)
    b = m.bias
    if m.Cin != m.Cin_real or m.Cout != m.Cout_real:
        w = F.pad(w, (0, m.Cin - m.Cin_real, 0, 0, 0, 0, 0, m.Cout - m.Cout_real))
        if b is not None:
            b = F.pad(b, (0, m.Cout - m.Cout_real))
    return torch.ops.jg355.conv2d_nt(x, w, b, res, m.pad, m.stride, alpha, res_scale if res is not None else 0.0)


CONV_STATS = os.environ.get("JG_CONV_STATS", "0") != "0"


def conv2d_stats(x, meta: ConvMeta):
    B, H, W, _ = x.shape
    Ho, Wo = meta.out_hw(H, W)
    if (not CONV_STATS or TORCH_OPS_BOUNDARY or KERNEL_TIMING is not None or (Ho * Wo) % 256 or meta.Cout % 64 or meta.R != meta.S or meta.R not in (1, 3)
            or meta.stride != 1 or _lib.lib().jg_get_tuning(b"JG_DETERMINISTIC") != 0):
        return conv2d(x, meta), None
    sums = torch.zeros((B, meta.Cout, 2), device=x.device, dtype=torch.float32)
    return _Conv2dFn.apply(x, meta.weight, meta.bias, None, meta, 1.0, 1.0, sums), sums


def conv2d(x, meta: ConvMeta, res=None, res_scale=1.0, alpha=1.0):
    if TORCH_OPS_BOUNDARY:
        return _conv2d_via_torch_ops(x, meta, res, res_scale, alpha)
    return _Conv2dFn.apply(x, meta.weight, meta.bias, res, meta, res_scale, alpha)


REFLECT_DGRAD_HALO = os.environ.get("JG_REFLECT_DGRAD_HALO", "1") != "0"


def reflect_conv_ok(x, m: ConvMeta):
    B, H, W, Cin = x.shape
    return (m.R == 3 and m.S == 3 and m.stride == 1 and m.pad == 0 and Cin % 64 == 0 and m.Cout % 64 == 0 and H % 16 == 0
            and W % 16 == 0 and H >= 16 and W >= 16 and B * H * W * max(Cin, m.Cout) < (1 << 31))


class _ReflectConv2dFn(JGFunction):

    @staticmethod
    def forward(ctx, x, weight, bias, meta, with_identity=False):
        _require_cuda(x)
        x = x.contiguous()
        B, H, W, Cin = x.shape
        m = meta
        y = torch.empty((B, H, W, m.Cout), device=x.device, dtype=x.dtype)
        conv_nt(x, m.w16, y, B=B, H=H, W=W, Cin=Cin, Cout=m.Cout, R=3, S=3, pad=1, stride=1, Ho=H, Wo=W, ldx=Cin, ldw=9 * Cin,
                ldy=m.Cout, bias=m.bias_pad if m.bias_pad is not None else m.bias, pad_mode=1)
        ctx.save_for_backward(x)
        ctx.meta = m
        ctx.with_identity = with_identity
        if with_identity:
            return x.view_as(x), y
        return y

    @staticmethod
    @torch.autograd.function.once_differentiable
    def backward(ctx, *grads):
        (x,) = ctx.saved_tensors
        m = ctx.meta
        did, dy = grads if ctx.with_identity else (None, grads[0])
        if dy is None:
            return did, None, None, None, None
        dy = dy.contiguous()
        B, H, W, Cin = x.shape
        dx = None
        if ctx.needs_input_grad[0]:
            if REFLECT_DGRAD_HALO and m.Cout % 64 == 0 and Cin % 64 == 0:
                dx = torch.empty_like(x)
                res = did.contiguous() if did is not None else None
                did = None
                conv_nt(dy, m.w16T, dx, B=B, H=H, W=W, Cin=m.Cout, Cout=Cin, R=3, S=3, pad=1, stride=1, Ho=H, Wo=W, ldx=m.Cout, ldw=9 * m.Cout,
                        ldy=Cin, res=res, ldres=Cin)
                ws = torch.empty(_lib.lib().jg_reflect_dgrad_border_ws_floats(B, H, W, Cin), device=x.device, dtype=torch.float32)
                check(_lib.lib().jg_reflect_dgrad_border(_dt(dy), dy.data_ptr(), m.Cout, m.w16T.data_ptr(), dx.data_ptr(), Cin, ws.data_ptr(), B, H, W,
                                                         m.Cout, Cin, 1.0, _st()), "jg_reflect_dgrad_border")
            else:
                dx = launch.reflect_pad2d_bwd(conv2d_dgrad(dy, m, (B, H + 2, W + 2, Cin)), 1)
        if ctx.needs_input_grad[1] or ctx.needs_input_grad[2]:
            wg = m.weight.grad
            if wg is None:
                raise RuntimeError("conv weight has no arena-backed .grad (module not finalised by ParamArena)")
            dbias = m.bias.grad if (ctx.needs_input_grad[2] and m.bias is not None) else None
            wgrad_tn(dy, x, wg, B=B, H=H, W=W, Cin=Cin, Cout=m.Cout, R=3, S=3, pad=1, stride=1, Ho=H, Wo=W, lddy=m.Cout, ldx=Cin,
                     lddw=9 * m.Cin_real, dbias=dbias, Cin_out=m.Cin_real, Cout_out=m.Cout_real,
                     splitk=_wgrad_splitk(((m.Cout + 127) // 128) * ((9 * Cin + 127) // 128), B * H * W), pad_mode=1)
        if did is not None and dx is not None:
            dx = axpby(dx, 1.0, did.contiguous(), 1.0)
        elif did is not None:
            dx = did
        return dx, None, None, None, None


def reflect_conv2d_id(x, meta: ConvMeta):
    return _ReflectConv2dFn.apply(x, meta.weight, meta.bias, meta, True)


def reflect_conv2d(x, meta: ConvMeta):
    if TORCH_OPS_BOUNDARY:
        return torch.ops.jg355.reflect_conv2d(x, meta.weight.permute(0, 2, 3, 1), meta.bias)
    return _ReflectConv2dFn.apply(x, meta.weight, meta.bias, meta)


ZERO_POOL = os.environ.get("JG_ZERO_POOL", "1") != "0"
_ZERO_CHUNK = {}


def zero_pool_reset(device=None, allocate=False):
    for k in [k for k in _ZERO_CHUNK if device is None or k[0] == device]:
        del _ZERO_CHUNK[k]
    if allocate and ZERO_POOL and device is not None:
        _ZERO_CHUNK[(device, torch.cuda.current_stream(device).cuda_stream)] = [torch.zeros(1 << 20, device=device, dtype=torch.float32), 0,
                                                                               torch.cuda.is_current_stream_capturing()]


def zeros_f32(n, device):
    n = (int(n) + 63) // 64 * 64
    if not ZERO_POOL or n > (1 << 18) or device.type != "cuda":
        return torch.zeros(n, device=device, dtype=torch.float32)
    cap = torch.cuda.is_current_stream_capturing()
    key = (device, torch.cuda.current_stream(device).cuda_stream)
    st = _ZERO_CHUNK.get(key)
    if st is not None and st[2] != cap:
        st = None
    if st is None and cap and not any(v[2] for v in _ZERO_CHUNK.values()):
        return torch.zeros(n, device=device, dtype=torch.float32)
    if st is None or st[1] + n > st[0].numel():
        st = _ZERO_CHUNK[key] = [torch.zeros(1 << 20, device=device, dtype=torch.float32), 0, cap]
    out = st[0][st[1]:st[1] + n]
    st[1] += n
    return out


def _drop_args(x, keep, u, key, stream, call, shape=None):
    keep, stream, call = float(keep), int(stream), int(call)
    if x.dim() != 4 or not 0.0 < keep <= 1.0 or not 0 <= stream < 65536 or not 0 <= call < 2 ** 32:
        raise ValueError(f"dropout: x [B, H, W, C], keep in (0, 1], stream < 65536 (got {tuple(x.shape)}, keep={keep}, stream={stream}, call={call})")
    B, H, W, C = x.shape if shape is None else shape
    if u is not None:
        if u.dtype != torch.float32 or tuple(u.shape) != (B, C, H, W):
            raise ValueError(f"dropout: u must be fp32 [B, C, H, W] = {(B, C, H, W)}, got {u.dtype} {tuple(u.shape)}")
        u, key = u.contiguous(), None
    elif key is None or key.numel() != 2 or key.element_size() != 4:
        raise ValueError("dropout: a draw needs the two-word Philox key (ops.d_aug_key)")
    _require_cuda(x, u, key)
    return keep, u, key, stream, call


def _group_norm_launch(x, gamma, beta, film, G, act, eps, sums=None, add=None, drop=None):
    _require_cuda(x)
    L = _lib.lib()
    B, C = x.shape[0], x.shape[-1]
    HW = x.numel() // (B * C)
    dev, st, dt = x.device, _st(), _dt(x)
    ab = torch.empty((B, C, 2), device=dev, dtype=torch.float32)
    mr = torch.empty((B, G, 2), device=dev, dtype=torch.float32)
    ldfilm = film.stride(0) if film is not None else 0
    if sums is None:
        sums = zeros_f32(B * C * 2, dev)[:B * C * 2].view(B, C, 2)
        check(L.jg_gn_stats_ld(dt, x.data_ptr(), C, sums.data_ptr(), C, B, HW, C, st), "jg_gn_stats_ld")
    check(L.jg_gn_coef(sums.data_ptr(), _p(gamma), _p(beta), _p(film), ldfilm, ab.data_ptr(), mr.data_ptr(), B, HW, C,
                       G, eps, st), "jg_gn_coef")
    if drop is not None:
        return launch.gn_apply_drop(x, ab, act, *drop), ab, mr
    y = torch.empty_like(x)
    if add is not None:
        add = add.contiguous()
        check(L.jg_gn_apply_add(dt, x.data_ptr(), C, ab.data_ptr(), add.data_ptr(), C, y.data_ptr(), C, B, HW, C, act, st), "jg_gn_apply_add")
    else:
        check(L.jg_gn_apply(dt, x.data_ptr(), ab.data_ptr(), y.data_ptr(), B, HW, C, act, st), "jg_gn_apply")
    return y, ab, mr


class _GroupNormFn(JGFunction):
    @staticmethod
    def forward(ctx, x, gamma, beta, film, G, act, eps, sums=None, add=None):
        y, ab, mr = _group_norm_launch(x, gamma, beta, film, G, act, eps, sums, add)
        ctx.save_for_backward(x, ab, mr, gamma, beta, film)
        ctx.G, ctx.act = G, act
        return y

    @staticmethod
    @torch.autograd.function.once_differentiable
    def backward(ctx, dy):
        x, ab, mr, gamma, beta, film = ctx.saved_tensors
        L = _lib.lib()
        dy = dy.contiguous()
        B, C = x.shape[0], x.shape[-1]
        HW = x.numel() // (B * C)
        dev, st, dt = x.device, _st(), _dt(x)
        red = zeros_f32(B * C * 2, dev)[:B * C * 2].view(B, C, 2)
        pqr = torch.empty((B, C, 3), device=dev, dtype=torch.float32)
        want_film = film is not None and ctx.needs_input_grad[3]
        dfilm = torch.empty((B, 2 * C), device=dev, dtype=torch.float32) if want_film else None
        dgamma = gamma.grad if (gamma is not None and ctx.needs_input_grad[1]) else None
        dbeta = beta.grad if (beta is not None and ctx.needs_input_grad[2]) else None
        if (gamma is not None and ctx.needs_input_grad[1] and dgamma is None):
            raise RuntimeError("norm weight has no arena-backed .grad")
        ldfilm = film.stride(0) if film is not None else 0
        check(L.jg_gn_bwd_reduce_ld_acc(dt, x.data_ptr(), C, dy.data_ptr(), C, ab.data_ptr(), red.data_ptr(), B, HW, C, ctx.act, st),
              "jg_gn_bwd_reduce_ld_acc")
        check(L.jg_gn_bwd_coef(red.data_ptr(), _p(gamma), _p(beta), _p(film), ldfilm, mr.data_ptr(), pqr.data_ptr(),
                               _p(dgamma), _p(dbeta), _p(dfilm), 2 * C, B, HW, C, ctx.G, st), "jg_gn_bwd_coef")
        dx = None
        if ctx.needs_input_grad[0]:
            dx = torch.empty_like(x)
            check(L.jg_gn_bwd_apply(dt, x.data_ptr(), dy.data_ptr(), ab.data_ptr(), pqr.data_ptr(), dx.data_ptr(), B, HW,
                                    C, ctx.act, st), "jg_gn_bwd_apply")
        return dx, None, None, dfilm, None, None, None, None, (dy if ctx.needs_input_grad[8] else None)


def _gn_drop_bwd_launch(x, dy, ab, mr, gamma, beta, film, G, act, drop, red, dgamma, dbeta, dfilm, want_dx=True):
    B, C = x.shape[0], x.shape[-1]
    HW = x.numel() // (B * C)
    pqr = torch.empty((B, C, 3), device=x.device, dtype=torch.float32)
    ldfilm = film.stride(0) if film is not None else 0
    launch.gn_bwd_reduce_drop(x, dy, ab, red, act, *drop)
    check(_lib.lib().jg_gn_bwd_coef(red.data_ptr(), _p(gamma), _p(beta), _p(film), ldfilm, mr.data_ptr(), pqr.data_ptr(), _p(dgamma), _p(dbeta),
                                    _p(dfilm), 2 * C, B, HW, C, G, _st()), "jg_gn_bwd_coef")
    return launch.gn_bwd_apply_drop(x, dy, ab, pqr, act, *drop) if want_dx else None


class _GroupNormDropFn(JGFunction):

    @staticmethod
    def forward(ctx, x, gamma, beta, film, G, act, eps, sums, keep, u, key, stream, call):
        x = x.contiguous()
        drop = _drop_args(x, keep, u, key, stream, call)
        y, ab, mr = _group_norm_launch(x, gamma, beta, film, G, act, eps, sums, None, drop)
        ctx.save_for_backward(x, ab, mr, gamma, beta, film, drop[1], drop[2])
        ctx.G, ctx.act, ctx.drop = G, act, (drop[0], drop[3], drop[4])
        return y

    @staticmethod
    @torch.autograd.function.once_differentiable
    def backward(ctx, dy):
        x, ab, mr, gamma, beta, film, u, key = ctx.saved_tensors
        keep, stream, call = ctx.drop
        B, C = x.shape[0], x.shape[-1]
        red = zeros_f32(B * C * 2, x.device)[:B * C * 2].view(B, C, 2)
        want_film = film is not None and ctx.needs_input_grad[3]
        dfilm = torch.empty((B, 2 * C), device=x.device, dtype=torch.float32) if want_film else None
        dgamma = gamma.grad if (gamma is not None and ctx.needs_input_grad[1]) else None
        dbeta = beta.grad if (beta is not None and ctx.needs_input_grad[2]) else None
        if (gamma is not None and ctx.needs_input_grad[1] and dgamma is None):
            raise RuntimeError("norm weight has no arena-backed .grad")
        dx = _gn_drop_bwd_launch(x, dy.contiguous(), ab, mr, gamma, beta, film, ctx.G, ctx.act, (keep, u, key, stream, call), red, dgamma, dbeta,
                                 dfilm, ctx.needs_input_grad[0])
        return (dx, None, None, dfilm) + (None,) * 9


class _ActDropFn(JGFunction):

    @staticmethod
    def forward(ctx, x, act, keep, u, key, stream, call):
        x = x.contiguous()
        drop = _drop_args(x, keep, u, key, stream, call)
        ctx.save_for_backward(x, drop[1], drop[2])
        ctx.act, ctx.drop = act, (drop[0], drop[3], drop[4])
        return launch.gn_apply_drop(x, None, act, *drop)

    @staticmethod
    @torch.autograd.function.once_differentiable
    def backward(ctx, dy):
        x, u, key = ctx.saved_tensors
        keep, stream, call = ctx.drop
        return (launch.gn_bwd_apply_drop(x, dy.contiguous(), None, None, ctx.act, keep, u, key, stream, call),) + (None,) * 6


def activation_dropout(x, act, keep, u=None, key=None, stream=0, call=0):
    if TORCH_OPS_BOUNDARY:
        return torch.ops.jg355.act_drop(x, act, float(keep), u, key, int(stream), int(call))
    return _ActDropFn.apply(x, act, keep, u, key, stream, call)


_GN_STATUS = {}


def gn_status(device):
    key = torch.device(device).index or 0
    t = _GN_STATUS.get(key)
    if t is None:
        t = _GN_STATUS[key] = torch.zeros(4, device=device, dtype=torch.int32)
    return t


def check_gn_status():
    for k, t in _GN_STATUS.items():
        if int(t[0]) != 0:
            raise RuntimeError(f"jg_gn_bwd_fused: an inter-workgroup wait expired on cuda:{k} (results of that launch are invalid)")


def group_norm(x, G, gamma=None, beta=None, film=None, act=JG_ACT_NONE, eps=1e-5, sums=None, add=None, keep=None, u=None, key=None, stream=0,
               call=0):
    if keep is not None:
        if add is not None:
            raise ValueError("group_norm: dropout and a residual addend do not occur behind one normalisation")
        if TORCH_OPS_BOUNDARY:
            return torch.ops.jg355.group_norm_act_drop(x, gamma, beta, film, G, act, eps, float(keep), u, key, int(stream), int(call))
        return _GroupNormDropFn.apply(x, gamma, beta, film, G, act, eps, sums, keep, u, key, stream, call)
    if TORCH_OPS_BOUNDARY:
        y = torch.ops.jg355.group_norm_act(x, gamma, beta, film, G, act, eps)
        return y if add is None else y + add
    return _GroupNormFn.apply(x, gamma, beta, film, G, act, eps, sums, add)


def conv_transpose2d_forward(x, m: ConvMeta, output_padding=0):
    B, H, W, Cin_t = x.shape
    assert Cin_t == m.Cout, (Cin_t, m.Cout)
    Ho = (H - 1) * m.stride - 2 * m.pad + m.R + output_padding
    Wo = (W - 1) * m.stride - 2 * m.pad + m.S + output_padding
    y = torch.empty((B, Ho, Wo, m.Cin), device=x.device, dtype=x.dtype)
    if Ho == 2 * H and Wo == 2 * W and phase_tconv_ok(m, Ho, Wo, Cin_t, m.Cin):
        return phase_tconv(x.contiguous(), m, y, bias=m.bias)
    Hd, Wd = Ho + 2 * m.pad - m.R + 1, Wo + 2 * m.pad - m.S + 1
    xd = dilate2d(x, Hd, Wd, m.stride)
    conv_nt(xd, m.w16T, y, B=B, H=Hd, W=Wd, Cin=Cin_t, Cout=m.Cin, R=m.R, S=m.S, pad=m.R - 1 - m.pad, stride=1, Ho=Ho, Wo=Wo,
            ldx=Cin_t, ldw=m.R * m.S * Cin_t, ldy=m.Cin, bias=m.bias)
    return y


class _ConvTranspose2dFn(JGFunction):
    @staticmethod
    def forward(ctx, x, weight, bias, meta, output_padding):
        _require_cuda(x)
        y = conv_transpose2d_forward(x, meta, output_padding)
        ctx.save_for_backward(x)
        ctx.meta = meta
        return y

    @staticmethod
    @torch.autograd.function.once_differentiable
    def backward(ctx, dy):
        (x,) = ctx.saved_tensors
        m = ctx.meta
        dy = dy.contiguous()
        B, H, W, Cin_t = x.shape
        _, Ho, Wo, Cout_t = dy.shape
        dx = None
        if ctx.needs_input_grad[0]:
            dx = torch.empty_like(x)
            conv_nt(dy, m.w16, dx, B=B, H=Ho, W=Wo, Cin=Cout_t, Cout=Cin_t, R=m.R, S=m.S, pad=m.pad, stride=m.stride, Ho=H, Wo=W,
                    ldx=Cout_t, ldw=m.R * m.S * Cout_t, ldy=Cin_t)
        if ctx.needs_input_grad[1]:
            wg = m.weight.grad
            if wg is None:
                raise RuntimeError("conv-transpose weight has no arena-backed .grad")
            ktot = m.R * m.S * Cout_t
            tiles = ((Cin_t + 127) // 128) * ((ktot + 127) // 128)
            wgrad_tn(x, dy, wg, B=B, H=Ho, W=Wo, Cin=Cout_t, Cout=Cin_t, R=m.R, S=m.S, pad=m.pad, stride=m.stride, Ho=H, Wo=W,
                     lddy=Cin_t, ldx=Cout_t, lddw=ktot, splitk=_wgrad_splitk(tiles, B * H * W))
        if ctx.needs_input_grad[2] and m.bias is not None:
            check(_lib.lib().jg_channel_sum(_dt(dy), dy.data_ptr(), Cout_t, m.bias.grad.data_ptr(), B * Ho * Wo, Cout_t, 1.0, _st()),
                  "jg_channel_sum")
        return dx, None, None, None, None


def conv_transpose2d(x, meta: ConvMeta, output_padding=0):
    if TORCH_OPS_BOUNDARY:
        from .ops_library_cut import conv_transpose2d_via_ops

        return conv_transpose2d_via_ops(x, meta, output_padding)
    return _ConvTranspose2dFn.apply(x, meta.weight, meta.bias, meta, output_padding)


class _ReflectPadFn(JGFunction):
    @staticmethod
    def forward(ctx, x, pad):
        _require_cuda(x)
        ctx.pad = pad
        return launch.reflect_pad2d(x.contiguous(), pad)

    @staticmethod
    @torch.autograd.function.once_differentiable
    def backward(ctx, dy):
        return launch.reflect_pad2d_bwd(dy.contiguous(), ctx.pad), None


def reflect_pad2d(x, pad):
    if TORCH_OPS_BOUNDARY:
        return torch.ops.jg355.reflect_pad2d(x, pad)
    return _ReflectPadFn.apply(x, pad)


def _crop_window(x, top, left, Ho, Wo):
    B, H, W, Cc = x.shape
    y = torch.empty(B, Ho, Wo, Cc, device=x.device, dtype=x.dtype)
    check(_lib.lib().jg_crop2d(_dt(x), x.data_ptr(), y.data_ptr(), B, H, W, Cc, top, left, Ho, Wo, 0, _st()), "jg_crop2d")
    return y


class _CropFn(JGFunction):
    @staticmethod
    def forward(ctx, x, top, left, Ho, Wo):
        _require_cuda(x)
        x = x.contiguous()
        ctx.cfg = (x.shape[1], x.shape[2], top, left)
        return _crop_window(x, top, left, Ho, Wo)

    @staticmethod
    @torch.autograd.function.once_differentiable
    def backward(ctx, dy):
        H, W, top, left = ctx.cfg
        dy = dy.contiguous()
        B, Ho, Wo, Cc = dy.shape
        dx = torch.empty(B, H, W, Cc, device=dy.device, dtype=dy.dtype)
        check(_lib.lib().jg_crop2d(_dt(dy), dy.data_ptr(), dx.data_ptr(), B, H, W, Cc, top, left, Ho, Wo, 1, _st()), "jg_crop2d")
        return dx, None, None, None, None


def crop2d(x, top, left, Ho, Wo):
    return _CropFn.apply(x, top, left, Ho, Wo)


class _ActFn(JGFunction):
    @staticmethod
    def forward(ctx, x, act):
        _require_cuda(x)
        y = launch.act_fwd(x.contiguous(), act)
        ctx.save_for_backward(y)
        ctx.act = act
        return y

    @staticmethod
    @torch.autograd.function.once_differentiable
    def backward(ctx, dy):
        (y,) = ctx.saved_tensors
        return launch.act_bwd(y, dy.contiguous(), ctx.act), None


def activation(x, act):
    if TORCH_OPS_BOUNDARY:
        return torch.ops.jg355.act(x, act)
    return _ActFn.apply(x, act)


def _pool(x, scale):
    B, H, W, Cc = x.shape
    y = torch.empty((B, H // 2, W // 2, Cc), device=x.device, dtype=x.dtype)
    check(_lib.lib().jg_pool2x2(_dt(x), x.data_ptr(), y.data_ptr(), B, H, W, Cc, scale, _st()), "jg_pool2x2")
    return y


def _up(x, scale):
    B, H, W, Cc = x.shape
    y = torch.empty((B, H * 2, W * 2, Cc), device=x.device, dtype=x.dtype)
    check(_lib.lib().jg_upsample2x(_dt(x), x.data_ptr(), y.data_ptr(), B, H, W, Cc, scale, _st()), "jg_upsample2x")
    return y


class _AvgPool2Fn(JGFunction):
    @staticmethod
    def forward(ctx, x):
        return _pool(x, 0.25)

    @staticmethod
    @torch.autograd.function.once_differentiable
    def backward(ctx, dy):
        return _up(dy.contiguous(), 0.25)


class _Upsample2Fn(JGFunction):
    @staticmethod
    def forward(ctx, x):
        return _up(x, 1.0)

    @staticmethod
    @torch.autograd.function.once_differentiable
    def backward(ctx, dy):
        return _pool(dy.contiguous(), 1.0)


def avg_pool2(x):
    return torch.ops.jg355.resample2(x, False, 0.25)


def upsample_nearest2(x):
    return torch.ops.jg355.resample2(x, True, 1.0)


def copy_channels(src, soff, dst, doff, n):
    P = src.numel() // src.shape[-1]
    check(_lib.lib().jg_copy_channels(_dt(src), src.data_ptr(), src.shape[-1], soff, dst.data_ptr(), dst.shape[-1], doff, P,
                                      n, _st()), "jg_copy_channels")


class _CatFn(JGFunction):
    @staticmethod
    def forward(ctx, a, b):
        Ca, Cb = a.shape[-1], b.shape[-1]
        y = torch.empty(a.shape[:-1] + (Ca + Cb,), device=a.device, dtype=a.dtype)
        copy_channels(a, 0, y, 0, Ca)
        copy_channels(b, 0, y, Ca, Cb)
        ctx.Ca, ctx.Cb = Ca, Cb
        return y

    @staticmethod
    @torch.autograd.function.once_differentiable
    def backward(ctx, dy):
        dy = dy.contiguous()
        da = db = None
        if ctx.needs_input_grad[0]:
            da = torch.empty(dy.shape[:-1] + (ctx.Ca,), device=dy.device, dtype=dy.dtype)
            copy_channels(dy, 0, da, 0, ctx.Ca)
# ... 964 lines not shown
        return out, noisy
    return _ContextFrameFn.apply(inner, ctx, c, C, sigma, z, key, int(noise_stream), int(call), None if outs is None else tuple(outs), want_noisy)


def _d_diffusion_launch(xs, a, b, t_epl, noise_std, key, call, ts, zs, outs, t_outs):
    n, B = _dd_check_maps(xs, "d_diffusion")
    for grp, what in ((ts, "ts"), (zs, "zs")):
        if grp is not None and len(grp) != n:
            raise ValueError(f"d_diffusion: {what} needs one entry per map (None: drawn)")
    for l, x in enumerate(xs):
        C = x.shape[3]
        t = None if ts is None else ts[l]
        z = None if zs is None else zs[l]
        if t is not None and (t.dtype != torch.int32 or tuple(t.shape) != (B, C) or not t.is_contiguous()):
            raise TypeError(f"d_diffusion: t of level {l} must be contiguous int32 {(B, C)}, got {tuple(t.shape)} {t.dtype}")
        if z is not None and (z.dtype != torch.float32 or tuple(z.shape) != (B, C, x.shape[1], x.shape[2]) or not z.is_contiguous()):
            raise TypeError(f"d_diffusion: z of level {l} must be contiguous fp32 {(B, C, x.shape[1], x.shape[2])}, got {tuple(z.shape)} {z.dtype}")
        _require_cuda(t, z)
    if key is not None and (key.dtype != torch.int32 or key.numel() != 2):
        raise TypeError("d_diffusion: key must hold two int32 words")
    _require_cuda(key)
    H, W, C = _dd_arrays(xs)
    check(_lib.lib().jg_d_diffusion(_dt(xs[0]), n, _dd_ptrs(xs, n), _dd_ptrs(outs, n), _dd_ptrs(t_outs, n), _dd_ptrs(ts, n), _dd_ptrs(zs, n), H, W, C, B,
                                    a.data_ptr(), b.data_ptr(), t_epl.data_ptr(), float(noise_std), _p(key), int(call), _st()), "jg_d_diffusion")


def _d_diffusion_bwd_launch(dys, t_saved, a):
    n, B = _dd_check_maps(dys, "d_diffusion_bwd")
    dxs = [torch.empty_like(d) for d in dys]
    H, W, C = _dd_arrays(dys)
    check(_lib.lib().jg_d_diffusion_bwd(_dt(dys[0]), n, _dd_ptrs(dys, n), _dd_ptrs(dxs, n), _dd_ptrs(t_saved, n), H, W, C, B, a.data_ptr(), _st()),
          "jg_d_diffusion_bwd")
    return dxs


class _DDiffusionFn(JGFunction):

    @staticmethod
    def forward(ctx, state, noise_std, key, call, ts, zs, *xs):
        xs = [x.contiguous() for x in xs]
        outs = [torch.empty_like(x) for x in xs]
        t_outs = [torch.empty((x.shape[0], x.shape[3]), device=x.device, dtype=torch.int32) for x in xs]
        _d_diffusion_launch(xs, state.a, state.b, state.t_epl, noise_std, key, call, ts, zs, outs, t_outs)
        ctx.a = state.a
        ctx.save_for_backward(*t_outs)
        ctx.mark_non_differentiable(*t_outs)
        return (*outs, *t_outs)

    @staticmethod
    @torch.autograd.function.once_differentiable
    def backward(ctx, *g):
        n = len(ctx.saved_tensors)
        dxs = _d_diffusion_bwd_launch([d.contiguous() for d in g[:n]], list(ctx.saved_tensors), ctx.a)
        return (None,) * 6 + tuple(dxs)


def d_diffusion(xs, state, noise_std, key=None, ts=None, zs=None, call=0):
    xs = list(xs)
    state.check()
    n = len(xs)
    if TORCH_OPS_BOUNDARY:
        if (ts is not None and any(t is None for t in ts)) or (zs is not None and any(z is None for z in zs)):
            raise ValueError("d_diffusion through torch.ops: ts / zs are given for every level or not at all")
        res = torch.ops.jg355.d_diffusion(xs, state.a, state.b, state.t_epl, float(noise_std), key, list(ts or ()), list(zs or ()), int(call))
        return list(res[:n]), list(res[n:])
    res = _DDiffusionFn.apply(state, float(noise_std), key, int(call), None if ts is None else list(ts), None if zs is None else list(zs), *xs)
    return list(res[:n]), list(res[n:])


def _d_diffusion_update_launch(p, Tn, a, b, t_epl, loss, num, den, u, key, call):
    _require_cuda(loss, u, key)
    if loss.dtype != torch.float32 or loss.numel() != 1:
        raise TypeError(f"d_diffusion_update: loss_real must be an fp32 scalar on the device, got {tuple(loss.shape)} {loss.dtype}")
    if u is not None and (u.dtype != torch.float32 or u.numel() != D_DIFFUSION_EPL or not u.is_contiguous()):
        raise TypeError(f"d_diffusion_update: u must be contiguous fp32 [{D_DIFFUSION_EPL}]")
    if key is not None and (key.dtype != torch.int32 or key.numel() != 2):
        raise TypeError("d_diffusion_update: key must hold two int32 words")
    check(_lib.lib().jg_d_diffusion_update(p.data_ptr(), Tn.data_ptr(), a.data_ptr(), b.data_ptr(), t_epl.data_ptr(), loss.data_ptr(), float(num),
                                           float(den), _p(u), _p(key), int(call), _st()), "jg_d_diffusion_update")


def d_diffusion_update(state, loss_real, batch_times_every, u=None, key=None, call=0):
    state.check()
    loss = loss_real.detach().reshape(1)
    if u is None and key is None:
        key = d_aug_key(loss.device)
    if TORCH_OPS_BOUNDARY:
        torch.ops.jg355.d_diffusion_update(*state.tensors(), loss, float(batch_times_every), 100.0 * 1000.0, u, key, int(call))
    else:
        _d_diffusion_update_launch(*state.tensors(), loss, float(batch_times_every), 100.0 * 1000.0, u, key, int(call))
    return state


class _ToNCHWFn(JGFunction):
    @staticmethod
    def forward(ctx, x, Cc):
        B, H, W, cpad = x.shape
        y = torch.empty((B, Cc, H, W), device=x.device, dtype=torch.float32)
        check(_lib.lib().jg_nhwc_to_nchw_f32(_dt(x), x.data_ptr(), y.data_ptr(), B, Cc, H, W, cpad, _st()), "nhwc_to_nchw")
        ctx.cpad, ctx.dtype = cpad, x.dtype
        return y

    @staticmethod
    @torch.autograd.function.once_differentiable
    def backward(ctx, dy):
        return to_nhwc(dy.contiguous().float(), ctx.dtype, ctx.cpad), None


def to_nchw_f32(x, Cc):
    return _ToNCHWFn.apply(x, Cc)


def to_nhwc(x, act_dtype, cpad=None):
    B, Cc, H, W = x.shape
    cpad = cpad or (Cc + 7) // 8 * 8
    y = torch.empty((B, H, W, cpad), device=x.device, dtype=act_dtype)
    check(_lib.lib().jg_nchw_f32_to_nhwc(_DT[act_dtype], x.contiguous().data_ptr(), y.data_ptr(), B, Cc, H, W, cpad, _st()),
          "nchw_to_nhwc")
    return y


def _conv_out_hw(H, W, R, S, pad, stride):
    return (H + 2 * pad - R) // stride + 1, (W + 2 * pad - S) // stride + 1


@torch.library.custom_op("jg355::conv2d_nt", mutates_args=())
def _op_conv2d_nt(x: torch.Tensor, w: torch.Tensor, bias: Optional[torch.Tensor], res: Optional[torch.Tensor], pad: int, stride: int,
                  alpha: float, res_scale: float) -> torch.Tensor:
    B, H, W, Cin = x.shape
    Cout, R, S, _ = w.shape
    Ho, Wo = _conv_out_hw(H, W, R, S, pad, stride)
    y = torch.empty((B, Ho, Wo, Cout), device=x.device, dtype=x.dtype)
    x, w = x.contiguous(), w.to(x.dtype).contiguous()
    conv_nt(x, w, y, B=B, H=H, W=W, Cin=Cin, Cout=Cout, R=R, S=S, pad=pad, stride=stride, Ho=Ho, Wo=Wo, ldx=Cin,
            ldw=R * S * Cin, ldy=Cout, bias=bias, res=None if res is None else res.contiguous(), ldres=Cout, alpha=alpha, res_scale=res_scale)
    return y


@_op_conv2d_nt.register_fake
def _(x, w, bias, res, pad, stride, alpha, res_scale):
    B, H, W, _ = x.shape
    Cout, R, S, _ = w.shape
    Ho, Wo = _conv_out_hw(H, W, R, S, pad, stride)
    return x.new_empty((B, Ho, Wo, Cout))


@torch.library.custom_op("jg355::conv2d_wgrad", mutates_args=())
def _op_conv2d_wgrad(dy: torch.Tensor, x: torch.Tensor, R: int, S: int, pad: int, stride: int, alpha: float) -> Tuple[torch.Tensor, torch.Tensor]:
    B, H, W, Cin = x.shape
    _, Ho, Wo, Cout = dy.shape
    dw = torch.zeros((Cout, R, S, Cin), device=x.device, dtype=torch.float32)
    db = torch.zeros((Cout,), device=x.device, dtype=torch.float32)
    ktot = R * S * Cin
    splitk = _wgrad_splitk(((Cout + 127) // 128) * ((ktot + 127) // 128), B * Ho * Wo)
    wgrad_tn(dy.contiguous(), x.contiguous(), dw, B=B, H=H, W=W, Cin=Cin, Cout=Cout, R=R, S=S, pad=pad, stride=stride, Ho=Ho, Wo=Wo,
             lddy=Cout, ldx=Cin, lddw=ktot, dbias=db, splitk=splitk, alpha=alpha)
    return dw, db


@_op_conv2d_wgrad.register_fake
def _(dy, x, R, S, pad, stride, alpha):
    return x.new_empty((dy.shape[-1], R, S, x.shape[-1]), dtype=torch.float32), x.new_empty((dy.shape[-1],), dtype=torch.float32)


def _conv2d_nt_setup(ctx, inputs, output):
    x, w, bias, res, pad, stride, alpha, res_scale = inputs
    ctx.save_for_backward(x, w)
    ctx.geo = (pad, stride, alpha, res_scale, bias is not None, res is not None)


def _conv2d_nt_backward(ctx, dy):
    x, w = ctx.saved_tensors
    pad, stride, alpha, res_scale, has_bias, has_res = ctx.geo
    Cout, R, S, Cin = w.shape
    dy = dy.contiguous()
    dx = dw = db = dres = None
    if ctx.needs_input_grad[0]:
        wT = w.to(dy.dtype).permute(3, 1, 2, 0).flip(1, 2).contiguous()
        dyd = dy
        if stride != 1:
            H, W_ = x.shape[1], x.shape[2]
            dyd = torch.ops.jg355.dilate2d(dy, H + 2 * pad - R + 1, W_ + 2 * pad - S + 1, stride)
        dx = torch.ops.jg355.conv2d_nt(dyd, wT, None, None, R - 1 - pad, 1, alpha, 0.0)
    if ctx.needs_input_grad[1] or (has_bias and ctx.needs_input_grad[2]):
        dwf, dbf = torch.ops.jg355.conv2d_wgrad(dy, x, R, S, pad, stride, alpha)
        dw = dwf.to(w.dtype) if ctx.needs_input_grad[1] else None
        db = dbf if (has_bias and ctx.needs_input_grad[2]) else None
    if has_res and ctx.needs_input_grad[3]:
        dres = dy if res_scale == 1.0 else (dy.float() * res_scale).to(dy.dtype)
    return dx, dw, db, dres, None, None, None, None


_op_conv2d_nt.register_autograd(_conv2d_nt_backward, setup_context=_conv2d_nt_setup)


@torch.library.custom_op("jg355::group_norm_act", mutates_args=())
def _op_group_norm_act(x: torch.Tensor, gamma: Optional[torch.Tensor], beta: Optional[torch.Tensor], film: Optional[torch.Tensor],
                       groups: int, act: int, eps: float) -> torch.Tensor:
    return _group_norm_launch(x.contiguous(), gamma, beta, None if film is None else film.contiguous(), groups, act, eps)[0]


@_op_group_norm_act.register_fake
def _(x, gamma, beta, film, groups, act, eps):
    return torch.empty_like(x)


@torch.library.custom_op("jg355::group_norm_act_bwd", mutates_args=())
def _op_group_norm_act_bwd(x: torch.Tensor, dy: torch.Tensor, gamma: Optional[torch.Tensor], beta: Optional[torch.Tensor],
                           film: Optional[torch.Tensor], groups: int, act: int, eps: float) -> Tuple[torch.Tensor, torch.Tensor, torch.Tensor, torch.Tensor]:
    L = _lib.lib()
    x, dy = x.contiguous(), dy.contiguous()
    B, C = x.shape[0], x.shape[-1]
    HW = x.numel() // (B * C)
    dev, st, dt = x.device, _st(), _dt(x)
    f32 = dict(device=dev, dtype=torch.float32)
    sums, ab, mr = torch.empty((B, C, 2), **f32), torch.empty((B, C, 2), **f32), torch.empty((B, groups, 2), **f32)
    film = None if film is None else film.contiguous()
    ldfilm = film.stride(0) if film is not None else 0
    check(L.jg_gn_stats(dt, x.data_ptr(), sums.data_ptr(), B, HW, C, st), "jg_gn_stats")
    check(L.jg_gn_coef(sums.data_ptr(), _p(gamma), _p(beta), _p(film), ldfilm, ab.data_ptr(), mr.data_ptr(), B, HW, C, groups, eps, st), "jg_gn_coef")
    red, pqr = torch.empty((B, C, 2), **f32), torch.empty((B, C, 3), **f32)
    dgamma, dbeta, dfilm = torch.zeros((C,), **f32), torch.zeros((C,), **f32), torch.zeros((B, 2 * C), **f32)
    check(L.jg_gn_bwd_reduce(dt, x.data_ptr(), dy.data_ptr(), ab.data_ptr(), red.data_ptr(), B, HW, C, act, st), "jg_gn_bwd_reduce")
    check(L.jg_gn_bwd_coef(red.data_ptr(), _p(gamma), _p(beta), _p(film), ldfilm, mr.data_ptr(), pqr.data_ptr(),
                           dgamma.data_ptr() if gamma is not None else None, dbeta.data_ptr() if beta is not None else None,
                           dfilm.data_ptr() if film is not None else None, 2 * C, B, HW, C, groups, st), "jg_gn_bwd_coef")
    dx = torch.empty_like(x)
    check(L.jg_gn_bwd_apply(dt, x.data_ptr(), dy.data_ptr(), ab.data_ptr(), pqr.data_ptr(), dx.data_ptr(), B, HW, C, act, st), "jg_gn_bwd_apply")
    return dx, dgamma, dbeta, dfilm


@_op_group_norm_act_bwd.register_fake
def _(x, dy, gamma, beta, film, groups, act, eps):
    B, C = x.shape[0], x.shape[-1]
    f = lambda *sh: x.new_empty(sh, dtype=torch.float32)
    return torch.empty_like(x), f(C), f(C), f(B, 2 * C)


def _gn_setup(ctx, inputs, output):
    x, gamma, beta, film, groups, act, eps = inputs
    ctx.save_for_backward(x, gamma, beta, film)
    ctx.cfg = (groups, act, eps)


def _gn_backward(ctx, dy):
    x, gamma, beta, film = ctx.saved_tensors
    groups, act, eps = ctx.cfg
    dx, dgamma, dbeta, dfilm = torch.ops.jg355.group_norm_act_bwd(x, dy, gamma, beta, film, groups, act, eps)
    return (dx if ctx.needs_input_grad[0] else None, dgamma if (gamma is not None and ctx.needs_input_grad[1]) else None,
            dbeta if (beta is not None and ctx.needs_input_grad[2]) else None,
            dfilm if (film is not None and ctx.needs_input_grad[3]) else None, None, None, None)


_op_group_norm_act.register_autograd(_gn_backward, setup_context=_gn_setup)


@torch.library.custom_op("jg355::group_norm_act_drop", mutates_args=())
def _op_group_norm_act_drop(x: torch.Tensor, gamma: Optional[torch.Tensor], beta: Optional[torch.Tensor], film: Optional[torch.Tensor],
                            groups: int, act: int, eps: float, keep: float, u: Optional[torch.Tensor], key: Optional[torch.Tensor], stream: int,
                            call: int) -> torch.Tensor:
    x = x.contiguous()
    return _group_norm_launch(x, gamma, beta, None if film is None else film.contiguous(), groups, act, eps, None, None,
                              _drop_args(x, keep, u, key, stream, call))[0]


@_op_group_norm_act_drop.register_fake
def _(x, gamma, beta, film, groups, act, eps, keep, u, key, stream, call):
    return torch.empty_like(x, memory_format=torch.contiguous_format)


@torch.library.custom_op("jg355::group_norm_act_drop_bwd", mutates_args=())
def _op_group_norm_act_drop_bwd(x: torch.Tensor, dy: torch.Tensor, gamma: Optional[torch.Tensor], beta: Optional[torch.Tensor],
                                film: Optional[torch.Tensor], groups: int, act: int, eps: float, keep: float, u: Optional[torch.Tensor],
                                key: Optional[torch.Tensor], stream: int, call: int) -> Tuple[torch.Tensor, torch.Tensor, torch.Tensor, torch.Tensor]:
    L = _lib.lib()
    x, dy = x.contiguous(), dy.contiguous()
    drop = _drop_args(x, keep, u, key, stream, call)
    B, C = x.shape[0], x.shape[-1]
    HW = x.numel() // (B * C)
    f32 = dict(device=x.device, dtype=torch.float32)
    sums, ab, mr = torch.empty((B, C, 2), **f32), torch.empty((B, C, 2), **f32), torch.empty((B, groups, 2), **f32)
    film = None if film is None else film.contiguous()
    ldfilm = film.stride(0) if film is not None else 0
    check(L.jg_gn_stats(_dt(x), x.data_ptr(), sums.data_ptr(), B, HW, C, _st()), "jg_gn_stats")
    check(L.jg_gn_coef(sums.data_ptr(), _p(gamma), _p(beta), _p(film), ldfilm, ab.data_ptr(), mr.data_ptr(), B, HW, C, groups, eps, _st()), "jg_gn_coef")
    dgamma, dbeta, dfilm = torch.zeros((C,), **f32), torch.zeros((C,), **f32), torch.zeros((B, 2 * C), **f32)
    dx = _gn_drop_bwd_launch(x, dy, ab, mr, gamma, beta, film, groups, act, drop, torch.zeros((B, C, 2), **f32), dgamma if gamma is not None else None,
                             dbeta if beta is not None else None, dfilm if film is not None else None)
    return dx, dgamma, dbeta, dfilm


@_op_group_norm_act_drop_bwd.register_fake
def _(x, dy, gamma, beta, film, groups, act, eps, keep, u, key, stream, call):
    B, C = x.shape[0], x.shape[-1]
    f = lambda *sh: x.new_empty(sh, dtype=torch.float32)
    return torch.empty_like(x, memory_format=torch.contiguous_format), f(C), f(C), f(B, 2 * C)


def _gnd_setup(ctx, inputs, output):
    x, gamma, beta, film, groups, act, eps, keep, u, key, stream, call = inputs
    ctx.save_for_backward(x, gamma, beta, film, u, key)
    ctx.cfg = (groups, act, eps, keep, stream, call)


def _gnd_backward(ctx, dy):
    x, gamma, beta, film, u, key = ctx.saved_tensors
    groups, act, eps, keep, stream, call = ctx.cfg
    dx, dgamma, dbeta, dfilm = torch.ops.jg355.group_norm_act_drop_bwd(x, dy, gamma, beta, film, groups, act, eps, keep, u, key, stream, call)
    return (dx if ctx.needs_input_grad[0] else None, dgamma if (gamma is not None and ctx.needs_input_grad[1]) else None,
# ... 319 lines not shown
```

joligen_amd/ops_library_cut.py:

```python
from __future__ import annotations

from typing import List, Optional, Tuple

import torch

from . import _lib, launch, ops
from ._lib import check
from .launch import SINKHORN_ITERS, _DT, _dt, _st
from .ops import conv_nt, wgrad_tn

T = torch.Tensor
op = torch.library.custom_op


def _z(like, dtype=torch.float32):
    return torch.zeros(0, device=like.device, dtype=dtype)


@op("jg355::layer_norm", mutates_args=())
def layer_norm(x: T, weight: T, bias: T, eps: float) -> Tuple[T, T]:
    return launch.layernorm_fwd(x.contiguous(), weight, bias, eps)


@layer_norm.register_fake
# ... 113 lines not shown
    B, Tn, C3 = qkv.shape
    return qkv.new_empty((B, Tn, C3 // 3)), qkv.new_empty((B * heads, Tn), dtype=torch.float32)


@op("jg355::vit_attention_bwd", mutates_args=())
def vit_attention_bwd(qkv: T, a: T, lse: T, da: T, heads: int) -> T:
    return launch.vit_attention_bwd(qkv.contiguous(), a, lse, da.contiguous(), heads)


@vit_attention_bwd.register_fake
def _(qkv, a, lse, da, heads):
    return torch.empty_like(qkv)


def _va_setup(ctx, inputs, output):
    ctx.save_for_backward(inputs[0], output[0], output[1])
    ctx.heads = inputs[1]


def _va_backward(ctx, da, dl):
    qkv, a, lse = ctx.saved_tensors
    return torch.ops.jg355.vit_attention_bwd(qkv, a, lse, da, ctx.heads), None


vit_attention.register_autograd(_va_backward, setup_context=_va_setup)


@op("jg355::gelu", mutates_args=())
def gelu(x: T) -> T:
    return launch.gelu_fwd(x.contiguous())


@gelu.register_fake
def _(x):
    return torch.empty_like(x)


@op("jg355::gelu_bwd", mutates_args=())
def gelu_bwd(x: T, dy: T) -> T:
    return launch.gelu_bwd(x.contiguous(), dy.contiguous())


@gelu_bwd.register_fake
def _(x, dy):
    return torch.empty_like(x)


gelu.register_autograd(lambda ctx, dy: torch.ops.jg355.gelu_bwd(ctx.saved_tensors[0], dy),
                       setup_context=lambda ctx, inputs, output: ctx.save_for_backward(inputs[0]))


@op("jg355::reflect_pad2d", mutates_args=())
def reflect_pad2d(x: T, pad: int) -> T:
    return launch.reflect_pad2d(x.contiguous(), pad)


@reflect_pad2d.register_fake
def _(x, pad):
    B, H, W, C = x.shape
    return x.new_empty((B, H + 2 * pad, W + 2 * pad, C))


@op("jg355::reflect_pad2d_bwd", mutates_args=())
def reflect_pad2d_bwd(dy: T, pad: int) -> T:
    return launch.reflect_pad2d_bwd(dy.contiguous(), pad)


@reflect_pad2d_bwd.register_fake
def _(dy, pad):
    B, Hp, Wp, C = dy.shape
    return dy.new_empty((B, Hp - 2 * pad, Wp - 2 * pad, C))


reflect_pad2d.register_autograd(lambda ctx, dy: (torch.ops.jg355.reflect_pad2d_bwd(dy, ctx.pad), None),
                                setup_context=lambda ctx, inputs, output: setattr(ctx, "pad", inputs[1]))
reflect_pad2d_bwd.register_autograd(lambda ctx, g: (torch.ops.jg355.reflect_pad2d(g, ctx.pad), None),
                                    setup_context=lambda ctx, inputs, output: setattr(ctx, "pad", inputs[1]))


@op("jg355::dilate2d", mutates_args=())
def dilate2d(x: T, Ho: int, Wo: int, stride: int) -> T:
    return ops.dilate2d(x.contiguous(), Ho, Wo, stride)


@dilate2d.register_fake
def _(x, Ho, Wo, stride):
    return x.new_empty((x.shape[0], Ho, Wo, x.shape[-1]))


def _dil_setup(ctx, inputs, output):
    ctx.geo = (inputs[0].shape[1], inputs[0].shape[2], inputs[3])


def _dil_backward(ctx, dy):
    H, W, s = ctx.geo
    return dy[:, ::s, ::s][:, :H, :W].contiguous(), None, None, None


dilate2d.register_autograd(_dil_backward, setup_context=_dil_setup)


@op("jg355::act", mutates_args=())
def act(x: T, kind: int) -> T:
    return launch.act_fwd(x.contiguous(), kind)


@act.register_fake
def _(x, kind):
    return torch.empty_like(x)


@op("jg355::act_bwd", mutates_args=())
def act_bwd(y: T, dy: T, kind: int) -> T:
    return launch.act_bwd(y.contiguous(), dy.contiguous(), kind)


@act_bwd.register_fake
def _(y, dy, kind):
    return torch.empty_like(y)


def _act_setup(ctx, inputs, output):
    ctx.save_for_backward(output)
    ctx.kind = inputs[1]


act.register_autograd(lambda ctx, dy: (torch.ops.jg355.act_bwd(ctx.saved_tensors[0], dy, ctx.kind), None), setup_context=_act_setup)


@op("jg355::reflect_conv2d", mutates_args=())
def reflect_conv2d(x: T, w: T, bias: Optional[T]) -> T:
    x = x.contiguous()
    B, H, W, Cin = x.shape
    Cout = w.shape[0]
    y = torch.empty((B, H, W, Cout), device=x.device, dtype=x.dtype)
    conv_nt(x, w.to(x.dtype).contiguous(), y, B=B, H=H, W=W, Cin=Cin, Cout=Cout, R=3, S=3, pad=1, stride=1, Ho=H, Wo=W, ldx=Cin, ldw=9 * Cin,
            ldy=Cout, bias=bias, pad_mode=1)
    return y


@reflect_conv2d.register_fake
def _(x, w, bias):
    return x.new_empty((*x.shape[:3], w.shape[0]))


@op("jg355::reflect_conv2d_wgrad", mutates_args=())
def reflect_conv2d_wgrad(dy: T, x: T) -> Tuple[T, T]:
    dy, x = dy.contiguous(), x.contiguous()
    B, H, W, Cin = x.shape
    Cout = dy.shape[-1]
    dw = torch.zeros((Cout, 3, 3, Cin), device=x.device, dtype=torch.float32)
    db = torch.zeros((Cout,), device=x.device, dtype=torch.float32)
    wgrad_tn(dy, x, dw, B=B, H=H, W=W, Cin=Cin, Cout=Cout, R=3, S=3, pad=1, stride=1, Ho=H, Wo=W, lddy=Cout, ldx=Cin, lddw=9 * Cin, dbias=db,
             splitk=ops._wgrad_splitk(((Cout + 127) // 128) * ((9 * Cin + 127) // 128), B * H * W), pad_mode=1)
    return dw, db


@reflect_conv2d_wgrad.register_fake
def _(dy, x):
    return x.new_empty((dy.shape[-1], 3, 3, x.shape[-1]), dtype=torch.float32), x.new_empty((dy.shape[-1],), dtype=torch.float32)


def _rc_setup(ctx, inputs, output):
    x, w, bias = inputs
    ctx.save_for_backward(x, w)
    ctx.has_bias = bias is not None


def _rc_backward(ctx, dy):
    x, w = ctx.saved_tensors
    dy = dy.contiguous()
    dx = dw = db = None
    if ctx.needs_input_grad[0]:
        wT = w.to(dy.dtype).permute(3, 1, 2, 0).flip(1, 2).contiguous()
        dx = torch.ops.jg355.reflect_pad2d_bwd(torch.ops.jg355.conv2d_nt(dy, wT, None, None, 2, 1, 1.0, 0.0), 1)
    if ctx.needs_input_grad[1] or (ctx.has_bias and ctx.needs_input_grad[2]):
        dwf, dbf = torch.ops.jg355.reflect_conv2d_wgrad(dy, x)
        dw = dwf.to(w.dtype) if ctx.needs_input_grad[1] else None
        db = dbf if (ctx.has_bias and ctx.needs_input_grad[2]) else None
    return dx, dw, db


reflect_conv2d.register_autograd(_rc_backward, setup_context=_rc_setup)


@op("jg355::gather_patches", mutates_args=())
def gather_patches(feat: T, ids: T, C: int) -> T:
    feat, ids = feat.contiguous(), ids.contiguous()
    B, H, W, ld = feat.shape
    P = ids.numel()
    out = torch.empty((B * P, C), device=feat.device, dtype=torch.float32)
    check(_lib.lib().jg_gather_rows(_dt(feat), feat.data_ptr(), ld, ids.data_ptr(), out.data_ptr(), B, H * W, C, P, _st()), "jg_gather_rows")
    return out


@gather_patches.register_fake
def _(feat, ids, C):
    return feat.new_empty((feat.shape[0] * ids.numel(), C), dtype=torch.float32)


@op("jg355::scatter_patches", mutates_args=())
def scatter_patches(dout: T, ids: T, B: int, H: int, W: int, ld: int, fp16: bool) -> T:
    dout, ids = dout.contiguous(), ids.contiguous()
    dt = torch.float16 if fp16 else torch.bfloat16
    dfeat = torch.zeros((B, H, W, ld), device=dout.device, dtype=dt)
    check(_lib.lib().jg_scatter_rows(_DT[dt], dfeat.data_ptr(), ld, ids.data_ptr(), dout.data_ptr(), B, H * W, dout.shape[1], ids.numel(), _st()),
          "jg_scatter_rows")
    return dfeat


@scatter_patches.register_fake
def _(dout, ids, B, H, W, ld, fp16):
    return dout.new_empty((B, H, W, ld), dtype=torch.float16 if fp16 else torch.bfloat16)


def _gp_setup(ctx, inputs, output):
    feat, ids, C = inputs
    ctx.save_for_backward(ids)
    ctx.geo = (*feat.shape, feat.dtype == torch.float16)


def _gp_backward(ctx, dout):
    (ids,) = ctx.saved_tensors
    B, H, W, ld, fp16 = ctx.geo
    return torch.ops.jg355.scatter_patches(dout, ids, B, H, W, ld, fp16), None, None


gather_patches.register_autograd(_gp_backward, setup_context=_gp_setup)


@op("jg355::l2_normalize", mutates_args=())
def l2_normalize(x: T, eps: float) -> Tuple[T, T]:
    return launch.l2norm_fwd(x.contiguous(), eps)


@l2_normalize.register_fake
def _(x, eps):
    return torch.empty_like(x), x.new_empty((x.shape[0],))


@op("jg355::l2_normalize_bwd", mutates_args=())
def l2_normalize_bwd(y: T, nrm: T, dy: T, eps: float) -> T:
    return launch.l2norm_bwd(y, nrm, dy.contiguous(), eps)


@l2_normalize_bwd.register_fake
def _(y, nrm, dy, eps):
    return torch.empty_like(y)


def _l2_setup(ctx, inputs, output):
    ctx.save_for_backward(output[0], output[1])
    ctx.eps = inputs[1]


l2_normalize.register_autograd(lambda ctx, dy, dn: (torch.ops.jg355.l2_normalize_bwd(ctx.saved_tensors[0], ctx.saved_tensors[1], dy, ctx.eps), None),
                               setup_context=_l2_setup)


@op("jg355::patch_nce", mutates_args=())
def patch_nce(q: T, k: T, nimg: int, temp: float, pm1: float, monce: bool) -> Tuple[T, T, T, T, T]:
    loss, S, K, uh, vh = launch.nce_fwd(q.contiguous(), k.contiguous(), nimg, temp, pm1, monce)
    return (loss, S, K, uh, vh) if monce else (loss, S, _z(q), _z(q), _z(q))


@patch_nce.register_fake
def _(q, k, nimg, temp, pm1, monce):
    R = q.shape[0]
    P = R // nimg
    e = q.new_empty((0,))
    if monce:
        return q.new_empty((R,)), q.new_empty((nimg, P, P)), q.new_empty((nimg, P, P)), q.new_empty((nimg, SINKHORN_ITERS, P)), q.new_empty((nimg, SINKHORN_ITERS + 1, P))
    return q.new_empty((R,)), q.new_empty((nimg, P, P)), e, q.new_empty((0,)), q.new_empty((0,))


@op("jg355::patch_nce_bwd", mutates_args=())
def patch_nce_bwd(q: T, k: T, S: T, K: T, uh: T, vh: T, dloss: T, nimg: int, temp: float, pm1: float, monce: bool) -> Tuple[T, T]:
    return launch.nce_bwd(q, k, S, K, uh, vh, dloss.contiguous().float(), nimg, temp, pm1, monce)


@patch_nce_bwd.register_fake
def _(q, k, S, K, uh, vh, dloss, nimg, temp, pm1, monce):
    return torch.empty_like(q), torch.empty_like(k)


def _nce_setup(ctx, inputs, output):
    q, k, nimg, temp, pm1, monce = inputs
    ctx.save_for_backward(q, k, *output[1:])
    ctx.cfg = (nimg, temp, pm1, monce)


def _nce_backward(ctx, dloss, *unused):
    q, k, S, K, uh, vh = ctx.saved_tensors
    dq, dk = torch.ops.jg355.patch_nce_bwd(q, k, S, K, uh, vh, dloss, *ctx.cfg)
    return dq, dk, None, None, None, None


patch_nce.register_autograd(_nce_backward, setup_context=_nce_setup)


@op("jg355::patch_hdce", mutates_args=())
def patch_hdce(q: T, k: T, nimg: int, temp: float, gamma: float, wperiod: int, wcount: int) -> Tuple[T, T, T, T]:
    loss, S, G, stats = launch.hdce_fwd(q.contiguous(), k.contiguous(), nimg, temp, gamma, wperiod, wcount)
    return loss, S, (_z(q) if G is None else G), stats


def _hdce_ng(nimg, wperiod, wcount):
# ... 336 lines not shown
```

joligen_amd/ops_segformer.py:

```python
from __future__ import annotations

import os

import torch

from ._autograd import JGFunction
from . import _lib, launch
from ._lib import JG_ACT_NONE, JG_ACT_RELU, check
from .ops import _DT, _dt, _p, _require_cuda, _st, copy_channels

DW_TWO_PHASE = os.environ.get("JG_DW_TWO_PHASE", "1") != "0"
RESIZE_BWD_SEPARABLE = os.environ.get("JG_RESIZE_BWD_SEPARABLE", "1") != "0"


class _LayerNormFn(JGFunction):
    @staticmethod
    def forward(ctx, x, weight, bias, eps):
        _require_cuda(x)
        x = x.contiguous()
        y, mr = launch.layernorm_fwd(x, weight, bias, eps)
        ctx.save_for_backward(x, mr, weight)
        ctx.gw, ctx.gb = weight.grad, bias.grad
        return y

# ... 236 lines not shown
        ab = torch.empty((B, C, 2), device=dev, dtype=torch.float32)
        mr = torch.empty((C, 2), device=dev, dtype=torch.float32)
        sums = None
        sync = _sync_active(training)
        world = 1
        if training:
            sums = torch.empty((B, C, 2), device=dev, dtype=torch.float32)
            check(L.jg_gn_stats(dt, x.data_ptr(), sums.data_ptr(), B, HW, C, st), "jg_gn_stats")
        if sync:
            tot = sums.sum(0, keepdim=True).contiguous()
            world = _all_reduce_sum(tot)
            ab1 = torch.empty((1, C, 2), device=dev, dtype=torch.float32)
            check(L.jg_bn_coef(tot.data_ptr(), weight.data_ptr(), bias.data_ptr(), _p(running_mean), _p(running_var), ab1.data_ptr(), mr.data_ptr(), 1,
                               world * B * HW, C, eps, momentum, 1, st), "jg_bn_coef")
            ab.copy_(ab1.expand(B, C, 2))
        else:
            check(L.jg_bn_coef(_p(sums), weight.data_ptr(), bias.data_ptr(), _p(running_mean), _p(running_var), ab.data_ptr(), mr.data_ptr(), B, HW, C,
                               eps, momentum, int(training), st), "jg_bn_coef")
        y = torch.empty_like(x)
        check(L.jg_gn_apply(dt, x.data_ptr(), ab.data_ptr(), y.data_ptr(), B, HW, C, act, st), "jg_gn_apply")
        ctx.save_for_backward(x, ab, mr, weight)
        ctx.cfg = (training, act, weight.grad, bias.grad, sync, world)
        return y

    @staticmethod
    @torch.autograd.function.once_differentiable
    def backward(ctx, dy):
        x, ab, mr, weight = ctx.saved_tensors
        training, act, gw, gb, sync, world = ctx.cfg
        L = _lib.lib()
        dy = dy.contiguous()
        B, C = x.shape[0], x.shape[-1]
        HW = x.numel() // (B * C)
        dev, st, dt = x.device, _st(), _dt(x)
        red = torch.empty((B, C, 2), device=dev, dtype=torch.float32)
        pqr = torch.empty((B, C, 3), device=dev, dtype=torch.float32)
        want_p = ctx.needs_input_grad[1] or ctx.needs_input_grad[2]
        if want_p and (gw is None or gb is None):
            raise RuntimeError("BatchNorm parameters have no arena-backed .grad")
        check(L.jg_gn_bwd_reduce(dt, x.data_ptr(), dy.data_ptr(), ab.data_ptr(), red.data_ptr(), B, HW, C, act, st), "jg_gn_bwd_reduce")
        if sync:
            if want_p:
                scratch = torch.empty((B, C, 3), device=dev, dtype=torch.float32)
                check(L.jg_bn_bwd_coef(red.data_ptr(), weight.data_ptr(), mr.data_ptr(), scratch.data_ptr(), _p(gw), _p(gb), B, HW, C, 1, st),
                      "jg_bn_bwd_coef")
            tot = red.sum(0, keepdim=True).contiguous()
            _all_reduce_sum(tot)
            pqr1 = torch.empty((1, C, 3), device=dev, dtype=torch.float32)
            check(L.jg_bn_bwd_coef(tot.data_ptr(), weight.data_ptr(), mr.data_ptr(), pqr1.data_ptr(), None, None, 1, world * B * HW, C, 1, st),
                  "jg_bn_bwd_coef")
            pqr.copy_(pqr1.expand(B, C, 3))
        else:
            check(L.jg_bn_bwd_coef(red.data_ptr(), weight.data_ptr(), mr.data_ptr(), pqr.data_ptr(), _p(gw) if want_p else None,
                                   _p(gb) if want_p else None, B, HW, C, int(training), st), "jg_bn_bwd_coef")
        dx = None
        if ctx.needs_input_grad[0]:
            dx = torch.empty_like(x)
            check(L.jg_gn_bwd_apply(dt, x.data_ptr(), dy.data_ptr(), ab.data_ptr(), pqr.data_ptr(), dx.data_ptr(), B, HW, C, act, st), "jg_gn_bwd_apply")
        return (dx,) + (None,) * 8


def batch_norm(x, bn, act=JG_ACT_NONE):
    training = bn.training
    if training and bn.num_batches_tracked is not None:
        bn.num_batches_tracked += 1
    return _BatchNormFn.apply(x, bn.weight, bn.bias, bn.running_mean, bn.running_var, training, float(bn.momentum), float(bn.eps), act)


class _AttnComposeFn(JGFunction):
    @staticmethod
    def forward(ctx, img, logits, xin, na, ni, nc):
        _require_cuda(img, logits, xin)
        img, logits, xin = img.contiguous(), logits.contiguous(), xin.contiguous()
        B, S = img.shape[0], img.shape[1]
        f = S // logits.shape[1]
        out = torch.empty_like(xin)
        check(_lib.lib().jg_attn_compose_fwd(_dt(img), img.data_ptr(), logits.data_ptr(), xin.data_ptr(), out.data_ptr(), B, S, f, na, ni, nc,
                                             img.shape[-1], logits.shape[-1], xin.shape[-1], out.shape[-1], _st()), "jg_attn_compose_fwd")
        ctx.save_for_backward(img, logits, xin)
        ctx.cfg = (f, na, ni, nc)
        return out

    @staticmethod
    @torch.autograd.function.once_differentiable
    def backward(ctx, dout):
        img, logits, xin = ctx.saved_tensors
        f, na, ni, nc = ctx.cfg
        dout = dout.contiguous()
        B, S = img.shape[0], img.shape[1]
        dimg, dlog = torch.empty_like(img), torch.empty_like(logits)
        dxin = torch.empty_like(xin) if ctx.needs_input_grad[2] else None
        check(_lib.lib().jg_attn_compose_bwd(_dt(img), img.data_ptr(), logits.data_ptr(), xin.data_ptr(), dout.data_ptr(), dimg.data_ptr(),
                                             dlog.data_ptr(), _p(dxin), B, S, f, na, ni, nc, img.shape[-1], logits.shape[-1], xin.shape[-1],
                                             dout.shape[-1], _st()), "jg_attn_compose_bwd")
        return dimg, dlog, dxin, None, None, None


def attention_compose(img, logits, xin, na, ni, nc):
    return _AttnComposeFn.apply(img, logits, xin, na, ni, nc)


class _ScaleFn(JGFunction):
    @staticmethod
    def forward(ctx, x, s, res, per_channel):
        _require_cuda(x)
        x = x.contiguous()
        B, C = x.shape[0], x.shape[-1]
        HW = x.numel() // (B * C)
        y = torch.empty_like(x)
        r = None if res is None else res.contiguous()
        check(_lib.lib().jg_scale(_dt(x), x.data_ptr(), s.data_ptr(), _p(r), y.data_ptr(), B, HW, C, int(per_channel), _st()), "jg_scale")
        ctx.save_for_backward(s)
        ctx.per_channel, ctx.has_res = per_channel, res is not None
        return y

    @staticmethod
    @torch.autograd.function.once_differentiable
    def backward(ctx, dy):
        (s,) = ctx.saved_tensors
        dy = dy.contiguous()
        B, C = dy.shape[0], dy.shape[-1]
        HW = dy.numel() // (B * C)
        dx = None
        if ctx.needs_input_grad[0]:
            dx = torch.empty_like(dy)
            check(_lib.lib().jg_scale(_dt(dy), dy.data_ptr(), s.data_ptr(), None, dx.data_ptr(), B, HW, C, int(ctx.per_channel), _st()), "jg_scale")
        return dx, None, (dy if ctx.has_res and ctx.needs_input_grad[2] else None), None


def scale_add(x, s, res=None, per_channel=False):
    return _ScaleFn.apply(x, s.contiguous().float(), res, per_channel)


class _SlicedLinearFn(JGFunction):

    @staticmethod
    def forward(ctx, x, weight, bias, meta, row0, n):
        from .ops import conv_nt

        _require_cuda(x)
        x = x.contiguous()
        B, N, Cin = x.shape
        m = meta
        y = torch.empty((B, N, n), device=x.device, dtype=x.dtype)
        conv_nt(x, m.w16, y, B=B, H=1, W=N, Cin=Cin, Cout=n, R=1, S=1, pad=0, stride=1, Ho=1, Wo=N, ldx=Cin, ldw=Cin, ldy=n,
                bias=None if m.bias is None else m.bias[row0:row0 + n], w_off=row0 * Cin)
        ctx.save_for_backward(x)
        ctx.cfg = (m, row0, n)
        return y

    @staticmethod
    @torch.autograd.function.once_differentiable
    def backward(ctx, dy):
        from .ops import _wgrad_splitk, conv_nt, wgrad_tn

        (x,) = ctx.saved_tensors
        m, row0, n = ctx.cfg
        dy = dy.contiguous()
        B, N, Cin = x.shape
        rows = m.Cout
        dx = None
        if ctx.needs_input_grad[0]:
            dx = torch.empty_like(x)
            conv_nt(dy, m.w16T, dx, B=B, H=1, W=N, Cin=n, Cout=Cin, R=1, S=1, pad=0, stride=1, Ho=1, Wo=N, ldx=n, ldw=rows, ldy=Cin, w_off=row0)
        if ctx.needs_input_grad[1] or ctx.needs_input_grad[2]:
            wg = m.weight.grad
            if wg is None:
                raise RuntimeError("projection weight has no arena-backed .grad")
            dbias = m.bias.grad[row0:row0 + n] if (m.bias is not None and ctx.needs_input_grad[2]) else None
            tiles = ((n + 127) // 128) * ((Cin + 127) // 128)
            wgrad_tn(dy, x, wg, B=B, H=1, W=N, Cin=Cin, Cout=n, R=1, S=1, pad=0, stride=1, Ho=1, Wo=N, lddy=n, ldx=Cin, lddw=Cin, dbias=dbias,
                     Cin_out=Cin, Cout_out=n, splitk=_wgrad_splitk(tiles, B * N), dw_off=row0 * Cin)
        return dx, None, None, None, None, None


class _SlicedInConvFn(JGFunction):

    @staticmethod
    def forward(ctx, x, weight, bias, meta, col0, with_bias):
        from .ops import conv_nt

        _require_cuda(x)
        x = x.contiguous()
        B, H, W, k = x.shape
        m = meta
        y = torch.empty((B, H, W, m.Cout), device=x.device, dtype=x.dtype)
        conv_nt(x, m.w16, y, B=B, H=H, W=W, Cin=k, Cout=m.Cout, R=1, S=1, pad=0, stride=1, Ho=H, Wo=W, ldx=k, ldw=m.Cin, ldy=m.Cout,
                bias=(m.bias_pad if m.bias_pad is not None else m.bias) if with_bias else None, w_off=col0)
        ctx.save_for_backward(x)
        ctx.cfg = (m, col0, with_bias)
        return y

    @staticmethod
    @torch.autograd.function.once_differentiable
    def backward(ctx, dy):
        from .ops import _wgrad_splitk, conv_nt, wgrad_tn

        (x,) = ctx.saved_tensors
        m, col0, with_bias = ctx.cfg
        dy = dy.contiguous()
        B, H, W, k = x.shape
        dx = None
        if ctx.needs_input_grad[0]:
            dx = torch.empty_like(x)
            conv_nt(dy, m.w16T, dx, B=B, H=H, W=W, Cin=m.Cout, Cout=k, R=1, S=1, pad=0, stride=1, Ho=H, Wo=W, ldx=m.Cout, ldw=m.Cout, ldy=k,
                    w_off=col0 * m.Cout)
        if ctx.needs_input_grad[1] or ctx.needs_input_grad[2]:
            wg = m.weight.grad
            if wg is None:
                raise RuntimeError("convolution weight has no arena-backed .grad")
            dbias = m.bias.grad if (with_bias and m.bias is not None and ctx.needs_input_grad[2]) else None
            tiles = ((m.Cout + 127) // 128) * ((k + 127) // 128)
            wgrad_tn(dy, x, wg, B=B, H=H, W=W, Cin=k, Cout=m.Cout, R=1, S=1, pad=0, stride=1, Ho=H, Wo=W, lddy=m.Cout, ldx=k, lddw=m.Cin_real,
                     dbias=dbias, Cin_out=k, Cout_out=m.Cout_real, splitk=_wgrad_splitk(tiles, B * H * W), dw_off=col0)
        return dx, None, None, None, None, None


def sliced_in_conv(x, meta, col0, with_bias=False):
    if meta.R != 1 or meta.S != 1 or meta.Cin != meta.Cin_real or col0 % 8 or x.shape[-1] % 8:
        raise ValueError("sliced_in_conv: 1x1 convolution with unpadded input channels, slices on multiples of 8")
    return _SlicedInConvFn.apply(x, meta.weight, meta.bias, meta, col0, with_bias)


class _ResizeSumFn(JGFunction):

    @staticmethod
    def forward(ctx, act, chscale, x0, *xs):
        _require_cuda(x0, *xs)
        x0 = x0.contiguous()
        xs = [x.contiguous() for x in xs]
        if len(xs) > 3:
            raise ValueError("resize_sum: at most three resized terms")
        B, Ho, Wo, C = x0.shape
        y = torch.empty_like(x0)
        a = []
        for i in range(3):
            a += [xs[i].data_ptr(), xs[i].shape[1], xs[i].shape[2]] if i < len(xs) else [None, 1, 1]
        if chscale is not None:
            chscale = chscale.contiguous().float()
            assert tuple(chscale.shape) == (B, C), tuple(chscale.shape)
        check(_lib.lib().jg_resize_sum(_dt(x0), x0.data_ptr(), *a, y.data_ptr(), B, Ho, Wo, C, act, _p(chscale), _st()), "jg_resize_sum")
        ctx.save_for_backward(y, chscale)
        ctx.cfg = (act, [tuple(x.shape) for x in xs])
        return y

    @staticmethod
    @torch.autograd.function.once_differentiable
    def backward(ctx, dy):
        y, chscale = ctx.saved_tensors
        act, shapes = ctx.cfg
        dy = dy.contiguous()
        B, Ho, Wo, C = y.shape
        need0, needs = ctx.needs_input_grad[2], ctx.needs_input_grad[3:]
        if (RESIZE_BWD_SEPARABLE and Wo * C * dy.element_size() <= 65536 and any(needs)) or chscale is not None:
            if Wo * C * dy.element_size() > 65536:
                raise NotImplementedError("resize_sum with a channel scale: rows of more than 64 KB")
            plain = act == JG_ACT_NONE and chscale is None
            g = torch.empty_like(y) if (need0 and not plain) else None
            outs, a = [], []
            for i in range(3):
                dx = None
                if i < len(shapes) and needs[i]:
                    dx = torch.empty((B, shapes[i][1], shapes[i][2], C), device=dy.device, dtype=dy.dtype)
                if i < len(shapes):
                    outs.append(dx)
                a += [_p(dx), shapes[i][1] if dx is not None else 1, shapes[i][2] if dx is not None else 1]
            nws = int(_lib.lib().jg_resize_sum_bwd_ws_floats(B, Ho, C, *(a[3 * i + 2] if a[3 * i] else 0 for i in range(3))))
            ws = torch.empty(max(nws, 1), device=dy.device, dtype=torch.float32)
            check(_lib.lib().jg_resize_sum_bwd(_dt(y), y.data_ptr(), dy.data_ptr(), _p(g), *a, ws.data_ptr(), B, Ho, Wo, C, act, _p(chscale), _st()),
                  "jg_resize_sum_bwd")
            return (None, None, (dy if plain else g) if need0 else None) + tuple(outs)
        g = dy
        if act != JG_ACT_NONE:
            g = launch.act_bwd(y, dy, act)
        outs = []
        for i, (_, H, W, _c) in enumerate(shapes):
            dx = None
            if needs[i]:
                dx = torch.empty((B, H, W, C), device=dy.device, dtype=dy.dtype)
                check(_lib.lib().jg_bilinear_bwd(_dt(g), g.data_ptr(), dx.data_ptr(), B, H, W, C, Ho, Wo, C, _st()), "jg_bilinear_bwd")
            outs.append(dx)
        return (None, None, g if need0 else None) + tuple(outs)


def resize_sum(x0, xs, act=JG_ACT_NONE, chscale=None):
    return _ResizeSumFn.apply(act, chscale, x0, *xs)


def sliced_linear(x, meta, row0, n):
    return _SlicedLinearFn.apply(x, meta.weight, meta.bias, meta, row0, n)
```

Before: 674.9 images/sec.

## Pick wgrad kernel kind and split-K in C++ with a cost model

```diff
diff --git a/joligen_amd/_lib.py b/joligen_amd/_lib.py
--- a/joligen_amd/_lib.py
+++ b/joligen_amd/_lib.py
@@ -84,22 +84,32 @@
 ConvArgs, WgradArgs = STRUCTS["jg_conv_args"], STRUCTS["jg_wgrad_args"]
 
 
-def build(force: bool = False, verbose: bool = False, jobs: int = 0) -> str:
+def build(force: bool = False, verbose: bool = False, jobs: int = 0, defines=()) -> str:
     import json
     import time
     from concurrent.futures import ThreadPoolExecutor
 
     hdrs = [os.path.join(CSRC, h) for h in sorted(os.listdir(CSRC)) if h.endswith(".h")] + [HEADER]
     hdr_time = max(os.path.getmtime(h) for h in hdrs)
-    bdir = os.path.join(CSRC, "build")
+    main_bdir = bdir = os.path.join(CSRC, "build")
+    lib_path = LIB_PATH
+    defines = tuple(defines)
+    if defines:
+        build(force=force, verbose=verbose, jobs=jobs)
+        tag = "_".join(defines).lower()
+        bdir, lib_path = os.path.join(CSRC, "build", tag), os.path.join(CSRC, f"libjg355_{tag}.so")
+        force = False
     os.makedirs(bdir, exist_ok=True)
     hipcc = os.environ.get("HIPCC", "/opt/rocm/bin/hipcc")
     if not os.path.exists(hipcc):
         hipcc = "hipcc"
-    cflags = [f for f in HIPCC_FLAGS if f != "-shared"]
+    cflags = [f for f in HIPCC_FLAGS if f != "-shared"] + ["-D" + d for d in defines]
     todo, objs = [], []
     for src in SOURCES:
-        sp, op = os.path.join(CSRC, src), os.path.join(bdir, src.replace(".hip", ".o"))
+        sp = os.path.join(CSRC, src)
+        with open(sp) as f:
+            own = not defines or any(d in f.read() for d in defines)
+        op = os.path.join(bdir if own else main_bdir, src.replace(".hip", ".o"))
         objs.append(op)
         if force or not os.path.exists(op) or os.path.getmtime(op) < max(os.path.getmtime(sp), hdr_time):
             todo.append((sp, op))
@@ -115,9 +125,9 @@
     if todo:
         with ThreadPoolExecutor(max_workers=jobs or min(len(todo), os.cpu_count() or 4)) as ex:
             list(ex.map(cc, todo))
-    relink = bool(todo) or not os.path.exists(LIB_PATH) or os.path.getmtime(LIB_PATH) < max(os.path.getmtime(o) for o in objs)
+    relink = bool(todo) or not os.path.exists(lib_path) or os.path.getmtime(lib_path) < max(os.path.getmtime(o) for o in objs)
     if relink:
-        cmd = [hipcc, "--offload-arch=gfx950", "-shared", "-fPIC", "-o", LIB_PATH] + objs
+        cmd = [hipcc, "--offload-arch=gfx950", "-shared", "-fPIC", "-o", lib_path] + objs
         if verbose:
             print(" ".join(cmd), flush=True)
         subprocess.run(cmd, check=True, cwd=CSRC)
@@ -125,7 +135,7 @@
         with open(os.path.join(bdir, "BUILD_INFO.json"), "w") as f:
             json.dump({"compiled": [os.path.basename(s) for s, _ in todo], "linked": relink, "seconds": round(time.time() - t0, 1),
                        "flags": cflags, "hipcc": hipcc}, f)
-    return LIB_PATH
+    return lib_path
 
 
 _lib = None
diff --git a/joligen_amd/csrc/common.h b/joligen_amd/csrc/common.h
--- a/joligen_amd/csrc/common.h
+++ b/joligen_amd/csrc/common.h
@@ -19,7 +19,7 @@
   X(HALO_DBG, 0) X(PERSIST64, 1) X(HALO_PIPE, 1) X(WGRAD_PIPE, 1) X(CONV_SPLITK, 1) X(CONV_SMALL_TILE, 1) X(GN_FUSED, 1)           \
   X(GN_FUSED_CAP, 256) X(GN_FUSED_DBG, 0) X(GN_FUSED_SLEEP, 4) X(WGRAD_LDS_PAD, 0) X(LN_BWD_CAP, 256) X(DW_BWD_CAP, 512)           \
   X(DW_BWD_PPT, 8) X(CONV_KXK, 1) X(CONV_RING, 1) X(WGRAD_DEEP, 1) X(WGRAD_SW, 0) X(DETERMINISTIC, 0) X(WGRAD_GROUP_BLOCKS, 1024)  \
-  X(SGEMM_SPLIT, 0) X(WGRAD_BIG, 1) X(DW_RUN, 1) X(SUBPIXEL_DGRAD_CFG, 0)
+  X(SGEMM_SPLIT, 0) X(WGRAD_BIG, 1) X(DW_RUN, 1) X(SUBPIXEL_DGRAD_CFG, 0) X(WGRAD_PICK, 1)
 #define JG_TUNE_ENUM(name, dflt) JG_TUNE_##name,
 enum JgTune { JG_TUNE_LIST(JG_TUNE_ENUM) JG_TUNE_COUNT };
 #undef JG_TUNE_ENUM
diff --git a/joligen_amd/csrc/gemm_tn.hip b/joligen_amd/csrc/gemm_tn.hip
--- a/joligen_amd/csrc/gemm_tn.hip
+++ b/joligen_amd/csrc/gemm_tn.hip
@@ -1,6 +1,10 @@
 #include "common.h"
 #include "wgrad_params.h"
 #include "lds_dma.h"
+#include "wgrad_pick.h"
+#include <array>
+#include <map>
+#include <mutex>
 #include <vector>
 #include <cstdlib>
 
@@ -726,6 +730,29 @@
   }
 
   const long zoff = zb * p.sdwb + zh * p.sdwh;
+  if constexpr (ABL == 5) {
+    float v = 0.f;
+#pragma unroll
+    for (int i = 0; i < 8; ++i)
+#pragma unroll
+      for (int j = 0; j < 4; ++j) v += acc[i][j][0] + acc[i][j][1] + acc[i][j][2] + acc[i][j][3];
+    const int n = n0 + wn * 64 + (lane & 15), m = m0 + wm * 128 + (lane >> 4);
+    if (n < p.Cin_out && m < p.Cout_out) atomicAdd((float*)p.dw + zoff + (long)m * p.lddw + n, p.alpha * v);
+    return;
+  }
+  if constexpr (ABL == 6) {
+    const int n = n0 + wn * 64 + lane;
+#pragma unroll
+    for (int i = 0; i < 8; ++i)
+#pragma unroll
+      for (int j = 0; j < 4; ++j)
+#pragma unroll
+        for (int q = 0; q < 4; ++q) {
+          const int m = m0 + wm * 128 + i * 16 + j * 4 + q;
+          if (n < p.Cin_out && m < p.Cout_out) atomicAdd((float*)p.dw + zoff + (long)m * p.lddw + n, p.alpha * acc[i][j][q]);
+        }
+    return;
+  }
 #pragma unroll
   for (int j = 0; j < 4; ++j) {
     const int n = n0 + wn * 64 + j * 16 + (lane & 15);
@@ -799,14 +826,40 @@
   return jg_tune(JG_TUNE_WGRAD_BIG) != 0 && p.out_mode == JG_OUT_ATOMIC_F32 && p.Cout >= 256 && p.Ktot >= 256 && p.Mpix >= 8192;
 }
 
-}
-
-static int make_wgp(const jg_wgrad_args* a, WgP& p) {
+static int wg_cus() {
+  static std::mutex mu;
+  static std::map<int, int> cus;
+  int dev = 0;
+  if (hipGetDevice(&dev) != hipSuccess) dev = 0;
+  std::lock_guard<std::mutex> lk(mu);
+  auto it = cus.find(dev);
+  if (it != cus.end()) return it->second;
+  int n = 0;
+  if (hipDeviceGetAttribute(&n, hipDeviceAttributeMultiprocessorCount, dev) != hipSuccess || n < 1) n = 1;
+  cus[dev] = n;
+  return n;
+}
+
+static JgWgPick wg_pick_cached(int Cout, int Ktot, int Mpix, int nbatch, bool det, int mask, bool keep_kind) {
+  static std::mutex mu;
+  static std::map<std::array<int, 7>, JgWgPick> memo;
+  const std::array<int, 7> key = {Cout, Ktot, Mpix, nbatch, wg_cus(), det ? 1 : 0, mask | (keep_kind ? 8 : 0)};
+  std::lock_guard<std::mutex> lk(mu);
+  auto it = memo.find(key);
+  if (it != memo.end()) return it->second;
+  const JgWgPick c = jg_wgrad_pick(Cout, Ktot, Mpix, nbatch, key[4], key[5], mask, keep_kind ? 1 : 0);
+  if (memo.size() < 4096) memo[key] = c;
+  return c;
+}
+
+}
+
+static int make_wgp(const jg_wgrad_args* a, WgP& p, int& kind, bool grouped = false) {
   if (!a || !a->dy || !a->x || !a->dw) return JG_ERR_BAD_ARG;
   if (a->Cin % 8 || a->Cout % 8 || a->ldx % 8 || a->lddy % 8) return JG_ERR_BAD_ARG;
-  if (a->nbatch < 1 || a->nh < 1 || a->splitk < 1) return JG_ERR_BAD_ARG;
+  if (a->nbatch < 1 || a->nh < 1 || a->splitk < 0) return JG_ERR_BAD_ARG;
   if ((long)a->nbatch * a->splitk > 65535) return JG_ERR_BAD_ARG;
-  if (a->out_mode != JG_OUT_ATOMIC_F32 && a->splitk != 1) return JG_ERR_BAD_ARG;
+  if (a->out_mode != JG_OUT_ATOMIC_F32 && a->splitk > 1) return JG_ERR_BAD_ARG;
   if (a->dbias && a->out_mode != JG_OUT_ATOMIC_F32) return JG_ERR_BAD_ARG;
   const long Mpix = (long)a->B * a->Ho * a->Wo;
   if (Mpix <= 0 || Mpix > (1L << 30)) return JG_ERR_BAD_ARG;
@@ -818,7 +871,21 @@
   p.Cout_out = a->Cout_out > 0 ? a->Cout_out : a->Cout;
   p.lddy = a->lddy; p.ldx = a->ldx; p.lddw = a->lddw;
   p.nh = a->nh; p.splitk = a->splitk;
-  if (jg_tune(JG_TUNE_DETERMINISTIC) != 0 && a->out_mode == JG_OUT_ATOMIC_F32) p.splitk = 1;
+  const bool det = jg_tune(JG_TUNE_DETERMINISTIC) != 0 && a->out_mode == JG_OUT_ATOMIC_F32;
+  if (det) p.splitk = 1;
+  const int variant = jg_tune(JG_TUNE_WGRAD_VARIANT);
+  p.out_mode = a->out_mode;
+  const int mask = 2 | (variant != 3 ? 1 : 0) | (variant >= 2 && wg_big_ok(p) ? 4 : 0);
+  kind = jg_wgrad_old_kind(p.Cout, p.Ktot, p.Mpix, mask);
+  if (a->splitk == 0) {
+    if (a->out_mode != JG_OUT_ATOMIC_F32) p.splitk = 1;
+    else if (jg_tune(JG_TUNE_WGRAD_PICK) == 0) p.splitk = det ? 1 : jg_wgrad_old_split(p.Cout, p.Ktot, p.Mpix, a->nbatch);
+    else {
+      const JgWgPick c = wg_pick_cached(p.Cout, p.Ktot, p.Mpix, a->nbatch, det, mask, grouped);
+      kind = c.kind;
+      p.splitk = c.splitk;
+    }
+  }
   p.sdyb = a->sdyb; p.sdyh = a->sdyh; p.sxb = a->sxb; p.sxh = a->sxh; p.sdwb = a->sdwb; p.sdwh = a->sdwh;
   p.alpha = a->alpha; p.out_mode = a->out_mode; p.B = a->B;
   p.dbias_scale = a->dbias_scale != 0.f ? a->dbias_scale : 1.f;
@@ -834,10 +901,13 @@
   if (!a || n < 1 || n > 4096) return JG_ERR_BAD_ARG;
   const int variant = jg_tune(JG_TUNE_WGRAD_VARIANT);
   if (variant < 2) return JG_ERR_UNSUPPORTED;
+  const int bigmode = jg_tune(JG_TUNE_WGRAD_BIG);
+  if (bigmode > 2) return JG_ERR_UNSUPPORTED;
   std::vector<WgP> ps((size_t)n);
   std::vector<char> special((size_t)n, 0);
+  std::vector<int> kinds((size_t)n, 0);
   for (int i = 0; i < n; ++i) {
-    const int rc = make_wgp(a + i, ps[i]);
+    const int rc = make_wgp(a + i, ps[i], kinds[i], true);
     if (rc != JG_OK) return rc;
     if (a[i].nbatch != 1 || a[i].out_mode != JG_OUT_ATOMIC_F32 || ps[i].reflect || ps[i].x_up) return JG_ERR_UNSUPPORTED;
     special[i] = variant >= 4 && (a[i].R > 1 || a[i].S > 1) &&
@@ -866,7 +936,7 @@
       const dim3 grid(g.start[g.n]);
       const int deep = jg_tune(JG_TUNE_WGRAD_DEEP);
       if (wavesm == 3) {
-        if (jg_tune(JG_TUNE_WGRAD_BIG) == 2) { JG_DISPATCH_DTYPE(dtype, hipLaunchKernelGGL((wgrad_tn_big_group_kernel<T, false>), grid, dim3(512), 0, (hipStream_t)stream, g);); }
+        if (bigmode == 2) { JG_DISPATCH_DTYPE(dtype, hipLaunchKernelGGL((wgrad_tn_big_group_kernel<T, false>), grid, dim3(512), 0, (hipStream_t)stream, g);); }
         else { JG_DISPATCH_DTYPE(dtype, hipLaunchKernelGGL((wgrad_tn_big_group_kernel<T, true>), grid, dim3(512), 0, (hipStream_t)stream, g);); }
       } else if (wavesm == 1) {
         if (deep & 1) { JG_DISPATCH_DTYPE(dtype, hipLaunchKernelGGL((wgrad_tn_tr_group_kernel<T, 1, true>), grid, dim3(256), gpad, (hipStream_t)stream, g);); }
@@ -880,7 +950,7 @@
     };
     for (int i = 0; i < n; ++i) {
       const WgP& p = ps[i];
-      if (special[i] || (wg_big_ok(p) ? 3 : p.Cout <= 64 ? 1 : 2) != wavesm) continue;
+      if (special[i] || kinds[i] != wavesm) continue;
       const int tiles = wavesm == 3 ? ((p.Cout + 255) / 256) * ((p.Ktot + 255) / 256) : ((p.Cout + 64 * wavesm - 1) / (64 * wavesm)) * ((p.Ktot + 127) / 128);
       g.p[g.n] = p;
       g.tiles[g.n] = tiles;
@@ -900,8 +970,9 @@
 extern "C" int jg_conv2d_wgrad_tn(int dtype, const jg_wgrad_args* a, jg_stream_t stream) {
   jg_note_kernel("");
   WgP p;
+  int kind = 0;
   {
-    const int rc = make_wgp(a, p);
+    const int rc = make_wgp(a, p, kind);
     if (rc != JG_OK) return rc;
   }
   const int variant = jg_tune(JG_TUNE_WGRAD_VARIANT);
@@ -915,15 +986,24 @@
     return JG_OK;
   }
   if (p.reflect || p.x_up) return JG_ERR_UNSUPPORTED;
-  if (variant >= 2 && wg_big_ok(p)) {
+  if (kind == JG_WGK_BIG) {
     const int tiles = ((p.Cout + 255) / 256) * ((p.Ktot + 255) / 256);
     dim3 grid(tiles, 1, a->nbatch * p.splitk);
     jg_note_kernel("wgrad_tn_big_kernel");
     const int bigmode = jg_tune(JG_TUNE_WGRAD_BIG);
-    if (bigmode == 11) { JG_DISPATCH_DTYPE(dtype, hipLaunchKernelGGL((wgrad_tn_big_kernel<T, true, 1>), grid, dim3(512), 0, (hipStream_t)stream, p);); }
-    else if (bigmode == 12) { JG_DISPATCH_DTYPE(dtype, hipLaunchKernelGGL((wgrad_tn_big_kernel<T, true, 2>), grid, dim3(512), 0, (hipStream_t)stream, p);); }
-    else if (bigmode == 14) { JG_DISPATCH_DTYPE(dtype, hipLaunchKernelGGL((wgrad_tn_big_kernel<T, true, 4>), grid, dim3(512), 0, (hipStream_t)stream, p);); }
-    else if (bigmode == 13) { JG_DISPATCH_DTYPE(dtype, hipLaunchKernelGGL((wgrad_tn_big_kernel<T, true, 3>), grid, dim3(512), 0, (hipStream_t)stream, p);); }
+    if (bigmode > 2) {
+#ifdef JG_ABLATIONS
+      if (bigmode == 11) { JG_DISPATCH_DTYPE(dtype, hipLaunchKernelGGL((wgrad_tn_big_kernel<T, true, 1>), grid, dim3(512), 0, (hipStream_t)stream, p);); }
+      else if (bigmode == 12) { JG_DISPATCH_DTYPE(dtype, hipLaunchKernelGGL((wgrad_tn_big_kernel<T, true, 2>), grid, dim3(512), 0, (hipStream_t)stream, p);); }
+      else if (bigmode == 13) { JG_DISPATCH_DTYPE(dtype, hipLaunchKernelGGL((wgrad_tn_big_kernel<T, true, 3>), grid, dim3(512), 0, (hipStream_t)stream, p);); }
+      else if (bigmode == 14) { JG_DISPATCH_DTYPE(dtype, hipLaunchKernelGGL((wgrad_tn_big_kernel<T, true, 4>), grid, dim3(512), 0, (hipStream_t)stream, p);); }
+      else if (bigmode == 15) { JG_DISPATCH_DTYPE(dtype, hipLaunchKernelGGL((wgrad_tn_big_kernel<T, true, 5>), grid, dim3(512), 0, (hipStream_t)stream, p);); }
+      else if (bigmode == 16) { JG_DISPATCH_DTYPE(dtype, hipLaunchKernelGGL((wgrad_tn_big_kernel<T, true, 6>), grid, dim3(512), 0, (hipStream_t)stream, p);); }
+      else return JG_ERR_UNSUPPORTED;
+#else
+      return JG_ERR_UNSUPPORTED;
+#endif
+    }
     else if (bigmode == 2) { JG_DISPATCH_DTYPE(dtype, hipLaunchKernelGGL((wgrad_tn_big_kernel<T, false>), grid, dim3(512), 0, (hipStream_t)stream, p);); }
     else { JG_DISPATCH_DTYPE(dtype, hipLaunchKernelGGL((wgrad_tn_big_kernel<T, true>), grid, dim3(512), 0, (hipStream_t)stream, p);); }
     JG_CHECK_LAUNCH();
@@ -933,7 +1013,7 @@
   if (variant == 1) {
     dim3 grid(((p.Cout + 127) / 128) * tilesN, 1, a->nbatch * p.splitk);
     JG_DISPATCH_DTYPE(dtype, hipLaunchKernelGGL((wgrad_tn_kernel<T>), grid, dim3(256), 0, (hipStream_t)stream, p););
-  } else if (p.Cout <= 64 && variant != 3) {
+  } else if (kind == JG_WGK_TR64) {
     dim3 grid(tilesN, 1, a->nbatch * p.splitk);
     jg_note_kernel("wgrad_tn_tr_kernel<1>");
     if (jg_tune(JG_TUNE_WGRAD_DEEP) & 1) { JG_DISPATCH_DTYPE(dtype, hipLaunchKernelGGL((wgrad_tn_tr_kernel<T, 1, true>), grid, dim3(256), 0, (hipStream_t)stream, p);); }
diff --git a/joligen_amd/csrc/wgrad_pick.h b/joligen_amd/csrc/wgrad_pick.h
--- /dev/null
+++ b/joligen_amd/csrc/wgrad_pick.h
@@ -0,0 +1,87 @@
+#pragma once
+
+enum { JG_WGK_TR64 = 1, JG_WGK_TR128 = 2, JG_WGK_BIG = 3 };
+
+struct JgWgKind {
+  int bm, bn;
+  int per_cu;
+  double step_us[2];
+  double epi_us;
+};
+constexpr double JG_WGPICK_LAUNCH_US = 4.0;
+
+inline JgWgKind jg_wgrad_kind(int kind) {
+  switch (kind) {
+    case JG_WGK_TR64: return {64, 128, 2, {1.50, 2.03}, 64 * 128 * 4 / 1.2e6};
+    case JG_WGK_BIG: return {256, 256, 1, {2.19, 2.19}, 256 * 256 * 4 / 1.2e6};
+    default: return {128, 128, 2, {1.63, 1.70}, 128 * 128 * 4 / 1.2e6};
+  }
+}
+
+struct JgWgPick {
+  int kind, splitk;
+  long blocks, rounds;
+  int steps;
+  double cost_us;
+};
+
+inline JgWgPick jg_wgrad_cost(int kind, int split, int Cout, int Ktot, int Mpix, int nbatch, int cus) {
+  const JgWgKind k = jg_wgrad_kind(kind);
+  if (split < 1) split = 1;
+  long per = ((long)Mpix + split - 1) / split;
+  per = (per + 63) / 64 * 64;
+  const int ske = (int)(((long)Mpix + per - 1) / per);
+  JgWgPick r;
+  r.kind = kind;
+  r.splitk = ske;
+  r.steps = (int)(per / 64);
+  const long tiles = (long)((Cout + k.bm - 1) / k.bm) * ((Ktot + k.bn - 1) / k.bn);
+  r.blocks = tiles * ske * nbatch;
+  const long slots = (long)(cus > 0 ? cus : 1) * k.per_cu;
+  r.rounds = (r.blocks + slots - 1) / slots;
+  const long last = r.blocks - (r.rounds - 1) * slots;
+  const long res = (last + (cus > 0 ? cus : 1) - 1) / (cus > 0 ? cus : 1);
+  r.cost_us = JG_WGPICK_LAUNCH_US + r.steps * ((r.rounds - 1) * k.step_us[k.per_cu - 1] + k.step_us[res - 1]) + r.blocks * k.epi_us;
+  return r;
+}
+
+inline int jg_wgrad_old_split(int Cout, int Ktot, int Mpix, int nbatch) {
+  const long tiles = (long)((Cout + 127) / 128) * ((Ktot + 127) / 128);
+  long s = (1536 + tiles - 1) / tiles;
+  const long cap = Mpix / 256;
+  if (s > cap) s = cap;
+  if (s > 512) s = 512;
+  if (s > 65535 / (nbatch > 0 ? nbatch : 1)) s = 65535 / (nbatch > 0 ? nbatch : 1);
+  return s < 1 ? 1 : (int)s;
+}
+
+inline int jg_wgrad_old_kind(int Cout, int Ktot, int Mpix, int mask) {
+  if ((mask & 4) && Cout >= 256 && Ktot >= 256 && Mpix >= 8192) return JG_WGK_BIG;
+  if ((mask & 1) && Cout <= 64) return JG_WGK_TR64;
+  return JG_WGK_TR128;
+}
+
+inline JgWgPick jg_wgrad_pick(int Cout, int Ktot, int Mpix, int nbatch, int cus, int deterministic, int mask = 7, int keep_kind = 0) {
+  if (nbatch < 1) nbatch = 1;
+  const long ksteps = ((long)Mpix + 63) / 64;
+  const long zmax = 65535 / nbatch;
+  const int old_kind = jg_wgrad_old_kind(Cout, Ktot, Mpix, mask);
+  int old_split = deterministic ? 1 : jg_wgrad_old_split(Cout, Ktot, Mpix, nbatch);
+  if (old_split > zmax) old_split = (int)(zmax < 1 ? 1 : zmax);
+  JgWgPick best = jg_wgrad_cost(old_kind, old_split, Cout, Ktot, Mpix, nbatch, cus);
+  const int first = old_kind == JG_WGK_TR64 || keep_kind ? old_kind : JG_WGK_TR128;
+  for (int kind = first; kind <= old_kind; ++kind) {
+    const JgWgKind k = jg_wgrad_kind(kind);
+    const long tiles = (long)((Cout + k.bm - 1) / k.bm) * ((Ktot + k.bn - 1) / k.bn) * nbatch;
+    long smax = 8L * cus * k.per_cu / tiles + 1;
+    if (smax > ksteps) smax = ksteps;
+    if (smax > zmax) smax = zmax;
+    if (deterministic || smax < 1) smax = 1;
+    for (long s = 1; s <= smax; ++s) {
+      const JgWgPick c = jg_wgrad_cost(kind, (int)s, Cout, Ktot, Mpix, nbatch, cus);
+      if (c.splitk != s) continue;
+      if (c.cost_us < best.cost_us || (c.cost_us == best.cost_us && (c.blocks < best.blocks || (c.blocks == best.blocks && c.kind > best.kind)))) best = c;
+    }
+  }
+  return best;
+}
diff --git a/joligen_amd/modules/projected_d.py b/joligen_amd/modules/projected_d.py
--- a/joligen_amd/modules/projected_d.py
+++ b/joligen_amd/modules/projected_d.py
@@ -223,10 +223,8 @@
                 raise RuntimeError("spectral conv weight has no arena-backed .grad")
             K = m.R * m.S * m.Cin_real
             dwsn = ctx.sn[0].dwsn(ctx.sn[1]) if ctx.sn is not None else torch.zeros((m.Cout_real, K), device=dy.device, dtype=torch.float32)
-            ktot = m.R * m.S * Cin
-            splitk = ops._wgrad_splitk(((Cout + 127) // 128) * ((ktot + 127) // 128), B * Ho * Wo)
             wgrad_tn(dy, x, dwsn, B=B, H=H, W=W_, Cin=Cin, Cout=Cout, R=m.R, S=m.S, pad=m.pad, stride=m.stride, Ho=Ho, Wo=Wo, lddy=Cout, ldx=Cin,
-                     lddw=K, dbias=mod.bias.grad if mod.bias is not None else None, Cin_out=m.Cin_real, Cout_out=m.Cout_real, splitk=splitk,
+                     lddw=K, dbias=mod.bias.grad if mod.bias is not None else None, Cin_out=m.Cin_real, Cout_out=m.Cout_real, splitk=0,
                      defer=ctx.sn is not None)
             if ctx.sn is not None:
                 ctx.sn[0].delivered(ctx.sn[1])
diff --git a/joligen_amd/modules/unet_exec.py b/joligen_amd/modules/unet_exec.py
--- a/joligen_amd/modules/unet_exec.py
+++ b/joligen_amd/modules/unet_exec.py
@@ -185,12 +185,9 @@
     wg = m.weight.grad
     if wg is None:
         raise RuntimeError("conv weight has no arena-backed .grad")
-    ktot = m.R * m.S * Cin
-    tiles = ((Cout + 127) // 128) * ((ktot + 127) // 128)
-    splitk = ops._wgrad_splitk(tiles, B * Ho * Wo)
     wgrad_tn(dy, x, wg, B=B, H=H, W=W, Cin=Cin, Cout=Cout, R=m.R, S=m.S, pad=m.pad, stride=m.stride, Ho=Ho, Wo=Wo,
              lddy=_ld(dy), ldx=_ld(x), lddw=m.R * m.S * m.Cin_real, dbias=m.bias.grad if m.bias is not None else None,
-             Cin_out=m.Cin_real, Cout_out=m.Cout_real, splitk=splitk, alpha=alpha, dbias_scale=dbias_scale, x_mode=(2 if subpixel else 1) if x_up else 0)
+             Cin_out=m.Cin_real, Cout_out=m.Cout_real, splitk=0, alpha=alpha, dbias_scale=dbias_scale, x_mode=(2 if subpixel else 1) if x_up else 0)
 
 
 def gn_coef(st, hw, gamma, beta, film, G, eps):
diff --git a/joligen_amd/ops.py b/joligen_amd/ops.py
--- a/joligen_amd/ops.py
+++ b/joligen_amd/ops.py
@@ -325,13 +325,10 @@
     wg = m.weight.grad
     if wg is None:
         raise RuntimeError("conv weight has no arena-backed .grad (module not finalised by ParamArena)")
-    ktot = m.R * m.S * Cin
-    tiles = ((Cout + 127) // 128) * ((ktot + 127) // 128)
-    splitk = _wgrad_splitk(tiles, B * Ho * Wo)
     dbias = m.bias.grad if (want_b and m.bias is not None) else None
     wgrad_tn(dy, x, wg, B=B, H=H, W=W, Cin=Cin, Cout=Cout, R=m.R, S=m.S, pad=m.pad, stride=m.stride, Ho=Ho, Wo=Wo,
              lddy=Cout, ldx=Cin, lddw=m.R * m.S * m.Cin_real, dbias=dbias, Cin_out=m.Cin_real, Cout_out=m.Cout_real,
-             splitk=splitk, alpha=alpha)
+             splitk=0, alpha=alpha)
 
 
 HEAD7_PACKED = os.environ.get("JG_HEAD7_PACKED", "1") != "0"
@@ -535,7 +532,7 @@
             dbias = m.bias.grad if (ctx.needs_input_grad[2] and m.bias is not None) else None
             wgrad_tn(dy, x, wg, B=B, H=H, W=W, Cin=Cin, Cout=m.Cout, R=3, S=3, pad=1, stride=1, Ho=H, Wo=W, lddy=m.Cout, ldx=Cin,
                      lddw=9 * m.Cin_real, dbias=dbias, Cin_out=m.Cin_real, Cout_out=m.Cout_real,
-                     splitk=_wgrad_splitk(((m.Cout + 127) // 128) * ((9 * Cin + 127) // 128), B * H * W), pad_mode=1)
+                     splitk=0, pad_mode=1)
         if did is not None and dx is not None:
             dx = axpby(dx, 1.0, did.contiguous(), 1.0)
         elif did is not None:
@@ -798,9 +795,8 @@
             if wg is None:
                 raise RuntimeError("conv-transpose weight has no arena-backed .grad")
             ktot = m.R * m.S * Cout_t
-            tiles = ((Cin_t + 127) // 128) * ((ktot + 127) // 128)
             wgrad_tn(x, dy, wg, B=B, H=Ho, W=Wo, Cin=Cout_t, Cout=Cin_t, R=m.R, S=m.S, pad=m.pad, stride=m.stride, Ho=H, Wo=W,
-                     lddy=Cin_t, ldx=Cout_t, lddw=ktot, splitk=_wgrad_splitk(tiles, B * H * W))
+                     lddy=Cin_t, ldx=Cout_t, lddw=ktot, splitk=0)
         if ctx.needs_input_grad[2] and m.bias is not None:
             check(_lib.lib().jg_channel_sum(_dt(dy), dy.data_ptr(), Cout_t, m.bias.grad.data_ptr(), B * Ho * Wo, Cout_t, 1.0, _st()),
                   "jg_channel_sum")
@@ -2071,9 +2067,8 @@
     dw = torch.zeros((Cout, R, S, Cin), device=x.device, dtype=torch.float32)
     db = torch.zeros((Cout,), device=x.device, dtype=torch.float32)
     ktot = R * S * Cin
-    splitk = _wgrad_splitk(((Cout + 127) // 128) * ((ktot + 127) // 128), B * Ho * Wo)
     wgrad_tn(dy.contiguous(), x.contiguous(), dw, B=B, H=H, W=W, Cin=Cin, Cout=Cout, R=R, S=S, pad=pad, stride=stride, Ho=Ho, Wo=Wo,
-             lddy=Cout, ldx=Cin, lddw=ktot, dbias=db, splitk=splitk, alpha=alpha)
+             lddy=Cout, ldx=Cin, lddw=ktot, dbias=db, splitk=0, alpha=alpha)
     return dw, db
 
 
diff --git a/joligen_amd/ops_library_cut.py b/joligen_amd/ops_library_cut.py
--- a/joligen_amd/ops_library_cut.py
+++ b/joligen_amd/ops_library_cut.py
@@ -289,7 +289,7 @@
     dw = torch.zeros((Cout, 3, 3, Cin), device=x.device, dtype=torch.float32)
     db = torch.zeros((Cout,), device=x.device, dtype=torch.float32)
     wgrad_tn(dy, x, dw, B=B, H=H, W=W, Cin=Cin, Cout=Cout, R=3, S=3, pad=1, stride=1, Ho=H, Wo=W, lddy=Cout, ldx=Cin, lddw=9 * Cin, dbias=db,
-             splitk=ops._wgrad_splitk(((Cout + 127) // 128) * ((9 * Cin + 127) // 128), B * H * W), pad_mode=1)
+             splitk=0, pad_mode=1)
     return dw, db
 
 
diff --git a/joligen_amd/ops_segformer.py b/joligen_amd/ops_segformer.py
--- a/joligen_amd/ops_segformer.py
+++ b/joligen_amd/ops_segformer.py
@@ -412,7 +412,7 @@
     @staticmethod
     @torch.autograd.function.once_differentiable
     def backward(ctx, dy):
-        from .ops import _wgrad_splitk, conv_nt, wgrad_tn
+        from .ops import conv_nt, wgrad_tn
 
         (x,) = ctx.saved_tensors
         m, row0, n = ctx.cfg
@@ -428,9 +428,8 @@
             if wg is None:
                 raise RuntimeError("projection weight has no arena-backed .grad")
             dbias = m.bias.grad[row0:row0 + n] if (m.bias is not None and ctx.needs_input_grad[2]) else None
-            tiles = ((n + 127) // 128) * ((Cin + 127) // 128)
             wgrad_tn(dy, x, wg, B=B, H=1, W=N, Cin=Cin, Cout=n, R=1, S=1, pad=0, stride=1, Ho=1, Wo=N, lddy=n, ldx=Cin, lddw=Cin, dbias=dbias,
-                     Cin_out=Cin, Cout_out=n, splitk=_wgrad_splitk(tiles, B * N), dw_off=row0 * Cin)
+                     Cin_out=Cin, Cout_out=n, splitk=0, dw_off=row0 * Cin)
         return dx, None, None, None, None, None
 
 
@@ -454,7 +453,7 @@
     @staticmethod
     @torch.autograd.function.once_differentiable
     def backward(ctx, dy):
-        from .ops import _wgrad_splitk, conv_nt, wgrad_tn
+        from .ops import conv_nt, wgrad_tn
 
         (x,) = ctx.saved_tensors
         m, col0, with_bias = ctx.cfg
@@ -470,9 +469,8 @@
             if wg is None:
                 raise RuntimeError("convolution weight has no arena-backed .grad")
             dbias = m.bias.grad if (with_bias and m.bias is not None and ctx.needs_input_grad[2]) else None
-            tiles = ((m.Cout + 127) // 128) * ((k + 127) // 128)
             wgrad_tn(dy, x, wg, B=B, H=H, W=W, Cin=k, Cout=m.Cout, R=1, S=1, pad=0, stride=1, Ho=H, Wo=W, lddy=m.Cout, ldx=k, lddw=m.Cin_real,
-                     dbias=dbias, Cin_out=k, Cout_out=m.Cout_real, splitk=_wgrad_splitk(tiles, B * H * W), dw_off=col0)
+                     dbias=dbias, Cin_out=k, Cout_out=m.Cout_real, splitk=0, dw_off=col0)
         return dx, None, None, None, None, None
 
 
```

Measured after the change: 674.5 images/sec. Within noise of the previous version (-0.1%).
